# k-sheridan/ekf_vio

Measured on AMD Instinct MI355X. Metric: filter steps/sec (predict+update), higher is better.
Workload: dtype f32

## Files before the change

### ekf_vio_amd/capi.py

```python
import ctypes as C
import os

from . import _build

OK, EINVAL, ENUMERIC, ECAPACITY, EDEVICE, ESTATE, EABORTED = range(7)
_ERR = {EINVAL: "EKFVIO_EINVAL", ENUMERIC: "EKFVIO_ENUMERIC", ECAPACITY: "EKFVIO_ECAPACITY",
        EDEVICE: "EKFVIO_EDEVICE", ESTATE: "EKFVIO_ESTATE", EABORTED: "EKFVIO_EABORTED"}
PREDICT_STRUCTURED, PREDICT_DENSE = 0, 1


class Config(C.Structure):
    _fields_ = [("max_features", C.c_int32), ("default_point_depth", C.c_float),
                ("default_point_depth_variance", C.c_float), ("default_point_homogenous_variance", C.c_float),
                ("predict_mode", C.c_int32), ("klt_window_size", C.c_int32), ("klt_max_pyramid_level", C.c_int32),
                ("klt_max_iterations", C.c_int32), ("klt_epsilon", C.c_float), ("klt_min_eigen", C.c_float),
                ("kill_pad", C.c_int32), ("max_image_width", C.c_int32), ("max_image_height", C.c_int32),
                ("use_principal_point", C.c_int32), ("inverse_image_scale", C.c_int32), ("fast_threshold", C.c_int32),
                ("min_new_feature_dist", C.c_int32), ("fast_blur_sigma", C.c_float), ("replenish", C.c_int32),
                ("sample_based_uncertainty", C.c_int32), ("use_imu", C.c_int32), ("imu_gyro_variance", C.c_float),
                ("imu_accel_variance", C.c_float), ("gravity", C.c_float * 3),
                ("klt_fb_max_px", C.c_float), ("remove_lost", C.c_int32)]


class EkfvioError(RuntimeError):
    def __init__(self, code, msg=""):
        super().__init__("%s %s" % (_ERR.get(code, str(code)), msg))
        self.code = code


SYMBOLS = ["ekfvio_default_config", "ekfvio_create", "ekfvio_destroy", "ekfvio_reset", "ekfvio_last_error",
           "ekfvio_add_features", "ekfvio_process", "ekfvio_linearize", "ekfvio_update", "ekfvio_measurement_map",
           "ekfvio_num_features", "ekfvio_dim", "ekfvio_get_base_mu", "ekfvio_get_features", "ekfvio_get_sigma",
           "ekfvio_get_feature_cov", "ekfvio_get_depth_variance", "ekfvio_set_feature_cov", "ekfvio_metric2pixel_map",
           "ekfvio_pixel2metric_map", "ekfvio_get_odometry", "ekfvio_get_points", "ekfvio_check_sigma", "ekfvio_set_state",
           "ekfvio_remove_features", "ekfvio_klt_push_frame", "ekfvio_klt_track", "ekfvio_klt_track_points", "ekfvio_klt_get_level",
           "ekfvio_klt_uncertainty_points", "ekfvio_step_image", "ekfvio_replenish", "ekfvio_fast_detect", "ekfvio_imu", "ekfvio_imu_update",
           "ekfvio_upload_measurements", "ekfvio_run_uploaded", "ekfvio_synchronize", "ekfvio_profile_enable",
           "ekfvio_profile_reset", "ekfvio_profile_count", "ekfvio_profile_name", "ekfvio_profile_get",
           "ekfvio_profile_update_gemms", "ekfvio_get_counters", "ekfvio_set_gate", "ekfvio_get_gate",
           "ekfvio_set_klt_fb", "ekfvio_get_klt_fb", "ekfvio_klt_track_points_fb", "ekfvio_set_distortion", "ekfvio_rectify_map",
           "ekfvio_set_output_covariance", "ekfvio_get_odometry_covariance", "ekfvio_get_points_covariance", "ekfvio_rotation_error_jacobian",
           "ekfvio_set_mask", "ekfvio_get_mask", "ekfvio_get_mask_hits", "ekfvio_mask_blocked", "ekfvio_set_equalize", "ekfvio_equalize",
           "ekfvio_set_klt_photometric", "ekfvio_klt_project_gradients",
           "ekfvio_get_landmark_ids", "ekfvio_set_ended_export", "ekfvio_get_ended",
           "ekfvio_set_zupt", "ekfvio_zupt_update", "ekfvio_get_zupt", "ekfvio_zupt_decide"]
MASK_RECTIFY_BORDER = 1
HOOK_SYMBOLS = ["ekfvio_test_klt_padded_level", "ekfvio_test_blurred_level0", "ekfvio_test_gemm", "ekfvio_test_gemm_bench", "ekfvio_test_potrf_stamps",
                "ekfvio_test_sweep_stamps", "ekfvio_test_sweep_fault", "ekfvio_test_sweep_delay", "ekfvio_test_cholesky_solve", "ekfvio_test_plan", "ekfvio_test_persist_grid", "ekfvio_test_t2_pair",
                "ekfvio_test_gemm_plan", "ekfvio_test_predict_plan", "ekfvio_test_run_plan", "ekfvio_test_mem", "ekfvio_test_mem_fail",
                "ekfvio_test_fill_update_scratch", "ekfvio_test_zupt_decide"]

_libs = {}


def lib_path():
    return _build.LIB_PATH


def load(build_if_missing=True, hooks=False):
    if hooks in _libs:
        return _libs[hooks]
    path = _build.HOOKS_LIB_PATH if hooks else _build.LIB_PATH
    if build_if_missing:
        _build.build(hooks=hooks)
    elif not os.path.exists(path):
        raise FileNotFoundError(path + " not built; run python -m ekf_vio_amd._build")
    lib = C.CDLL(path)
    vp, i32, f32 = C.c_void_p, C.c_int32, C.c_float
    fp, u8p, ip = C.POINTER(C.c_float), C.POINTER(C.c_uint8), C.POINTER(C.c_int32)
    sig = {
        "ekfvio_default_config": [C.POINTER(Config)],
        "ekfvio_create": [C.POINTER(Config), C.c_int, vp, C.POINTER(vp)],
        "ekfvio_destroy": [vp], "ekfvio_reset": [vp],
        "ekfvio_add_features": [vp, fp, i32], "ekfvio_process": [vp, f32], "ekfvio_linearize": [vp, f32, fp],
        "ekfvio_update": [vp, fp, fp, u8p, i32], "ekfvio_measurement_map": [vp, u8p, i32, ip, ip],
        "ekfvio_num_features": [vp], "ekfvio_dim": [vp], "ekfvio_get_base_mu": [vp, fp],
        "ekfvio_get_features": [vp, fp, fp, u8p], "ekfvio_get_sigma": [vp, fp, i32],
        "ekfvio_get_feature_cov": [vp, i32, fp], "ekfvio_get_depth_variance": [vp, i32, fp],
        "ekfvio_set_feature_cov": [vp, i32, fp], "ekfvio_metric2pixel_map": [fp, fp], "ekfvio_pixel2metric_map": [fp, fp],
        "ekfvio_get_odometry": [vp, fp, fp, fp, fp], "ekfvio_get_points": [vp, fp, fp],
        "ekfvio_check_sigma": [vp, fp, fp], "ekfvio_set_state": [vp, i32, fp, fp, fp, u8p, fp, i32],
        "ekfvio_remove_features": [vp, u8p, i32, ip],
        "ekfvio_klt_push_frame": [vp, u8p, i32, i32, i32, fp], "ekfvio_klt_track": [vp, fp, fp, u8p],
        "ekfvio_klt_track_points": [vp, fp, fp, i32, fp, u8p],
        "ekfvio_klt_uncertainty_points": [vp, fp, fp, i32, fp],
        "ekfvio_klt_get_level": [vp, i32, ip, ip, u8p, C.POINTER(C.c_int16)],
        "ekfvio_step_image": [vp, C.c_double, u8p, i32, i32, i32, fp], "ekfvio_imu": [vp, C.c_double, fp, fp], "ekfvio_imu_update": [vp, fp, fp],
        "ekfvio_replenish": [vp, ip, ip], "ekfvio_fast_detect": [vp, i32, i32, i32, ip, ip, ip],
        "ekfvio_upload_measurements": [vp, i32, fp, fp, u8p], "ekfvio_run_uploaded": [vp, i32, i32, f32],
        "ekfvio_synchronize": [vp], "ekfvio_profile_enable": [vp, i32], "ekfvio_profile_reset": [vp],
        "ekfvio_profile_count": [], "ekfvio_profile_name": [i32],
        "ekfvio_profile_get": [vp, i32, C.POINTER(C.c_double), C.POINTER(C.c_int64), C.POINTER(C.c_double)],
        "ekfvio_profile_update_gemms": [vp, i32, C.POINTER(C.c_double), C.POINTER(C.c_double)],
        "ekfvio_get_counters": [vp, C.POINTER(C.c_int64)],
        "ekfvio_set_gate": [vp, f32], "ekfvio_get_gate": [vp, fp, u8p, ip, ip, C.POINTER(C.c_int64)],
        "ekfvio_set_klt_fb": [vp, f32], "ekfvio_get_klt_fb": [vp, fp, u8p, ip, ip, C.POINTER(C.c_int64)],
        "ekfvio_klt_track_points_fb": [vp, fp, fp, i32, fp, u8p, fp, fp, u8p],
        "ekfvio_set_distortion": [vp, C.POINTER(C.c_double), i32],
        "ekfvio_rectify_map": [fp, C.POINTER(C.c_double), i32, i32, i32, ip, ip],
        "ekfvio_set_output_covariance": [vp, i32], "ekfvio_get_odometry_covariance": [vp, fp, fp], "ekfvio_get_points_covariance": [vp, fp],
        "ekfvio_rotation_error_jacobian": [fp, fp],
        "ekfvio_set_mask": [vp, u8p, i32, i32, i32, i32], "ekfvio_get_mask": [vp, u8p, i32, ip, ip], "ekfvio_get_mask_hits": [vp, u8p, ip, ip],
        "ekfvio_mask_blocked": [fp, C.POINTER(C.c_double), i32, u8p, i32, i32, i32, i32, i32, i32, u8p],
        "ekfvio_set_equalize": [vp, f32, i32, i32],
        "ekfvio_equalize": [u8p, i32, i32, i32, f32, i32, i32, u8p],
        "ekfvio_set_klt_photometric": [vp, i32],
        "ekfvio_klt_project_gradients": [ip, ip, ip, i32, ip, ip],
        "ekfvio_get_landmark_ids": [vp, C.POINTER(C.c_int64), C.POINTER(C.c_double)],
        "ekfvio_set_ended_export": [vp, i32],
        "ekfvio_get_ended": [vp, C.POINTER(C.c_int64), C.POINTER(C.c_double), ip, fp, fp, i32, ip, C.POINTER(C.c_int64)],
        "ekfvio_set_zupt": [vp, f32, i32, f32, f32, f32], "ekfvio_zupt_update": [vp, f32, f32],
        "ekfvio_get_zupt": [vp, fp, ip, ip, ip, ip, C.POINTER(C.c_int64)],
        "ekfvio_zupt_decide": [fp, fp, u8p, i32, f32, i32, f32, fp, ip, ip, ip],
    }
    if hooks:
        sig.update({
            "ekfvio_test_klt_padded_level": [vp, i32, ip, u8p, C.POINTER(C.c_int16)],
            "ekfvio_test_blurred_level0": [vp, u8p],
            "ekfvio_test_gemm": [vp, i32, i32, i32, i32, f32, fp, i32, fp, i32, f32, fp, i32, i32],
            "ekfvio_test_cholesky_solve": [vp, i32, i32, fp, fp, fp, fp, ip],
            "ekfvio_test_potrf_stamps": [vp, C.POINTER(C.c_int64)],
            "ekfvio_test_sweep_stamps": [vp, C.c_int, C.POINTER(C.c_int64)],
            "ekfvio_test_sweep_fault": [vp, i32, i32],
            "ekfvio_test_sweep_delay": [vp, i32, i32, i32],
            "ekfvio_test_gemm_bench": [vp, i32, i32, i32, i32, i32, i32, i32, C.POINTER(C.c_double)],
            "ekfvio_test_plan": [i32] * 8 + [f32, ip],
            "ekfvio_test_persist_grid": [i32] * 8 + [f32, ip, i32, ip],
            "ekfvio_test_t2_pair": [i32, ip],
            "ekfvio_test_gemm_plan": [i32] * 11 + [ip],
            "ekfvio_test_predict_plan": [i32] * 5 + [ip],
            "ekfvio_test_run_plan": [i32] * 4 + [ip, i32, ip],
            "ekfvio_test_mem": [vp, C.POINTER(C.c_int64)],
            "ekfvio_test_mem_fail": [vp, i32],
            "ekfvio_test_fill_update_scratch": [vp, C.c_uint32],
            "ekfvio_test_zupt_decide": [vp, fp, fp, u8p, i32, f32, i32, f32, fp, ip, ip, ip],
        })
    for name, args in sig.items():
        fn = getattr(lib, name)
        fn.argtypes = args
        fn.restype = C.c_int
    lib.ekfvio_last_error.argtypes = [vp]
    lib.ekfvio_last_error.restype = C.c_char_p
    lib.ekfvio_profile_name.restype = C.c_char_p
    _libs[hooks] = lib
    return lib
```

### ekf_vio_amd/csrc/api.hip

```cpp
#include <math.h>
#include <stdio.h>
#include <string.h>

#include <algorithm>
#include <atomic>
#include <chrono>

#include <unistd.h>

#include "common.h"

static_assert((int)hipErrorOutOfMemory == MEM_ERR_OUT_OF_MEMORY && (int)hipSuccess == MEM_OK, "mem.h's codes are the runtime's");
namespace {
struct MemTotal {
    std::atomic<int64_t> live{0}, live_bytes{0}, acquired{0}, released{0};
} g_mem_total[MEM_KINDS];
int hip_mem_allocate(MemKind kind, size_t bytes, void** out) {
    static const unsigned host_flags[MEM_KINDS] = {0, hipHostMallocDefault, hipHostMallocMapped, hipHostMallocMapped | hipHostMallocCoherent};
    void* p = nullptr;
    const hipError_t e = kind == MEM_DEVICE ? hipMalloc(&p, bytes) : hipHostMalloc(&p, bytes, host_flags[kind]);
    if (e != hipSuccess) return (int)e;
    g_mem_total[kind].live++, g_mem_total[kind].live_bytes += (int64_t)bytes, g_mem_total[kind].acquired++;
    *out = p;
    return MEM_OK;
// ... 117 lines not shown
    return EKFVIO_OK;
}

extern "C" {

int ekfvio_default_config(ekfvio_config* c) {
    if (!c) return EKFVIO_EINVAL;
    c->max_features = 100;
    c->default_point_depth = 0.5f;
    c->default_point_depth_variance = 100.f;
    c->default_point_homogenous_variance = 1e-5f;
    c->predict_mode = EKFVIO_PREDICT_STRUCTURED;
    c->klt_window_size = 21;
    c->klt_max_pyramid_level = 3;
    c->klt_max_iterations = 30;
    c->klt_epsilon = 0.01f;
    c->klt_min_eigen = 1e-4f;
    c->kill_pad = 11;
    c->max_image_width = 640;
    c->max_image_height = 480;
    c->use_principal_point = 0;
    c->inverse_image_scale = 1;
    c->fast_threshold = 50;
    c->min_new_feature_dist = 30;
    c->fast_blur_sigma = 0.f;
    c->replenish = 0;
    c->sample_based_uncertainty = 0;
    c->use_imu = 0;
    c->imu_gyro_variance = 1e-4f;
    c->imu_accel_variance = 1e-2f;
    c->gravity[0] = 0.f;
    c->gravity[1] = 9.81f;
    c->gravity[2] = 0.f;
    c->klt_fb_max_px = 0.f;
    c->remove_lost = 0;
    return EKFVIO_OK;
}

static int create_body(ekfvio_filter* f, const ekfvio_config* cfg, int device, void* stream) {
    HIP_TRY(f, hipSetDevice(device));
    if (stream) {
        f->stream = (hipStream_t)stream;
    } else {
        HIP_TRY(f, hipStreamCreateWithFlags(&f->stream, hipStreamNonBlocking));
        f->own_stream = true;
    }
    const int maxf = cfg->max_features;
    const FilterDims dims = filter_dims(maxf);
    f->n_cap = dims.n_cap, f->ldp = dims.ldp, f->m_cap = dims.m_cap, f->ld_aug = dims.ld_aug, f->sweep_sync_words = dims.sweep_sync_words;
    f->tune = tuning_from_env();
    const size_t pp = (size_t)f->ldp * f->ldp, pm = (size_t)f->ldp * f->m_cap;
    HIP_TRY(f, dev_alloc(f, &f->mu, f->ldp));
    HIP_TRY(f, dev_alloc(f, &f->mu_next, f->ldp));
    HIP_TRY(f, dev_alloc(f, &f->last_klt, 2 * (size_t)maxf));
    HIP_TRY(f, dev_alloc(f, &f->del_flag, (size_t)maxf));
    HIP_TRY(f, dev_alloc(f, &f->lm_id, (size_t)maxf));
    HIP_TRY(f, dev_alloc(f, &f->lm_born, (size_t)maxf));
    HIP_TRY(f, dev_alloc(f, &f->P, pp));
    HIP_TRY(f, dev_alloc(f, &f->P2, pp));
    HIP_TRY(f, dev_alloc(f, &f->FA, EKF_BASE * EKF_BASE));
    HIP_TRY(f, dev_alloc(f, &f->FB, 27 * (size_t)maxf));
    HIP_TRY(f, dev_alloc(f, &f->FD, 9 * (size_t)maxf));
    HIP_TRY(f, dev_alloc(f, &f->Fdense, pp));
    HIP_TRY(f, dev_alloc(f, &f->idx, (size_t)f->m_cap));
    HIP_TRY(f, dev_alloc(f, &f->inv_idx, (size_t)f->ldp));
    HIP_TRY(f, dev_alloc(f, &f->zmeas, 2 * (size_t)maxf));
    HIP_TRY(f, dev_alloc(f, &f->Rmeas, 4 * (size_t)maxf));
    HIP_TRY(f, dev_alloc(f, &f->pass, (size_t)maxf));
    HIP_TRY(f, dev_alloc(f, &f->yres, (size_t)f->m_cap));
    HIP_TRY(f, dev_alloc(f, &f->Rm, 2 * (size_t)f->m_cap));
    HIP_TRY(f, dev_alloc(f, &f->Saug, (size_t)f->ld_aug * f->m_cap));
    HIP_TRY(f, dev_alloc(f, &f->Laug, (size_t)f->ld_aug * f->m_cap));
    HIP_TRY(f, dev_alloc(f, &f->Linv, 64 * (size_t)f->m_cap));
    HIP_TRY(f, dev_alloc(f, &f->Lsign, (size_t)(f->m_cap / 64 > 256 ? f->m_cap / 64 : 256)));
    HIP_TRY(f, dev_alloc(f, &f->sweep_sync, f->sweep_sync_words));
    {
        hipDeviceProp_t prop;
        HIP_TRY(f, hipGetDeviceProperties(&prop, device));
        f->num_cus = prop.multiProcessorCount;
    }
    HIP_TRY(f, dev_alloc(f, &f->Km, pm));
    HIP_TRY(f, dev_alloc(f, &f->Wt, pm));
    HIP_TRY(f, dev_alloc(f, &f->Gm, pm));
    HIP_TRY(f, dev_alloc(f, &f->info, 4));
    HIP_TRY(f, dev_alloc(f, &f->remove_words, 4));
    HIP_TRY(f, host_alloc(f, &f->h_info, 16 * sizeof(int), MEM_PINNED_COHERENT));
    memset(f->h_info, 0, 16 * sizeof(int));
    HIP_TRY(f, hipHostGetDevicePointer((void**)&f->d_hinfo, f->h_info, 0));
    {
        const size_t words = out_words(f);
        HIP_TRY(f, host_alloc(f, &f->h_out, words * sizeof(float), MEM_PINNED_COHERENT));
        HIP_TRY(f, hipHostGetDevicePointer((void**)&f->d_out, f->h_out, 0));
    }
    {
        const size_t cap = (size_t)(f->cfg.max_features > 0 ? f->cfg.max_features : 1);
        HIP_TRY(f, host_alloc(f, &f->h_meas, 25 * cap, MEM_PINNED));
        HIP_TRY(f, dev_alloc_bare(f, &f->d_meas, 25 * cap));
    }
    HIP_TRY(f, hipEventCreate(&f->ev0));
    HIP_TRY(f, hipEventCreate(&f->ev1));
    int rc = klt_alloc(f);
    if (rc != EKFVIO_OK) return rc;
    rc = fast_alloc(f);
    if (rc != EKFVIO_OK) return rc;
    return ekfvio_reset(f);
}

}

static std::atomic<int>* live_registry() {
    static std::atomic<int>* reg = [] {
        char name[64], val[32];
        snprintf(name, sizeof(name), "EKFVIO_LIVE_HANDLES_%ld", (long)getpid());
        if (const char* e = getenv(name)) {
            void* p = nullptr;
            if (sscanf(e, "%p", &p) == 1 && p) return static_cast<std::atomic<int>*>(p);
        }
        auto* a = new std::atomic<int>[64];
        for (int i = 0; i < 64; i++) a[i].store(0, std::memory_order_relaxed);
        snprintf(val, sizeof(val), "%p", static_cast<void*>(a));
        setenv(name, val, 1);
        return a;
    }();
    return reg;
}
int live_handles_on(int device) { return (device >= 0 && device < 64) ? live_registry()[device].load(std::memory_order_relaxed) : 2; }

void drop_graph(ekfvio_filter* f) {
    for (GraphCache::Entry& e : f->graphs.g) {
        if (e.exec) (void)hipGraphExecDestroy(e.exec);
        e = GraphCache::Entry();
    }
}
template <class Body>
static int capture_graph(ekfvio_filter* f, hipGraphExec_t* out, Body body) {
    hipGraph_t g = nullptr;
    HIP_TRY(f, hipStreamSynchronize(f->stream));
    HIP_TRY(f, hipStreamBeginCapture(f->stream, hipStreamCaptureModeThreadLocal));
    body();
    const hipError_t ce = hipStreamEndCapture(f->stream, &g);
    if (ce != hipSuccess || !g) {
        f->last_error = std::string("graph capture: ") + hipGetErrorString(ce);
        return EKFVIO_EDEVICE;
    }
    HIP_TRY(f, hipGraphInstantiate(out, g, nullptr, nullptr, 0));
    (void)hipGraphDestroy(g);
    return EKFVIO_OK;
}

extern "C" {

int ekfvio_create(const ekfvio_config* cfg, int device, void* stream, ekfvio_filter** out) {
    if (!out) return EKFVIO_EINVAL;
    *out = nullptr;
    if (!cfg || cfg->max_features < 0) return EKFVIO_EINVAL;
    if (cfg->remove_lost != 0 && cfg->remove_lost != 1) return EKFVIO_EINVAL;
    if (cfg->remove_lost && (size_t)cfg->max_features * 17 > 64 * 1024) return EKFVIO_ECAPACITY;
    if (!(cfg->klt_fb_max_px >= 0.f)) return EKFVIO_EINVAL;
    int ndev = 0;
    if (hipGetDeviceCount(&ndev) != hipSuccess || device < 0 || device >= ndev) return EKFVIO_EDEVICE;
    ekfvio_filter* f = new ekfvio_filter();
#ifdef EKFVIO_TEST_HOOKS
    f->mem.fail_nth(g_next_create_fail.exchange(0));
#endif
    f->cfg = *cfg;
    f->device = device;
// ... 817 lines not shown
    return EKFVIO_OK;
}

int ekfvio_test_plan(int32_t num_cus, int32_t max_features, int32_t N, int32_t m, int32_t m_on_device, int32_t sole_handle,
                     int32_t latched_off, int32_t dense_predict, float next_dt, int32_t plan[12]) {
    if (!plan || max_features < 0 || N < 0 || N > max_features) return EKFVIO_EINVAL;
    const FilterDims d = filter_dims(max_features);
    PlanShape s;
    s.num_cus = num_cus, s.ldp = d.ldp, s.sweep_sync_words = d.sweep_sync_words, s.N = N, s.n = EKF_BASE + 3 * N;
    s.dense_predict = dense_predict != 0, s.sole_handle = sole_handle != 0, s.latched_off = latched_off != 0;
    const UpdatePlan p = plan_update(tuning_from_env(), s, m, m_on_device != 0, next_dt);
    const int32_t out[12] = {p.m, p.m_pad, p.n_pad, p.sweep, p.fused_gather, p.with_wt, p.gain, p.tail, p.t2_skip, p.t2_by_sweep, p.compact, p.lin_blocks};
    std::copy(out, out + 12, plan);
    return EKFVIO_OK;
}

int ekfvio_test_gemm_plan(int32_t num_cus, int32_t M, int32_t N, int32_t K, int32_t transB, int32_t lowerB, int32_t epi, int32_t mean,
                          int32_t lin_blocks, int32_t sym, int32_t variant, int32_t plan[18]) {
    if (!plan || M <= 0 || N <= 0 || K <= 0 || epi < EPI_NONE || epi > EPI_MEAN_PARTIAL) return EKFVIO_EINVAL;
    GemmShape s;
    s.M = M, s.N = N, s.K = K, s.transB = transB != 0, s.lowerB = lowerB != 0, s.epi = epi, s.mean = mean != 0;
    s.lin_blocks = lin_blocks, s.sym = sym != 0, s.variant = variant;
    const GemmPlan p = plan_gemm(tuning_from_env(), num_cus, s);
    const int32_t out[18] = {p.k16, p.bm, p.wps, p.groups, p.threads(), p.tiles_x, p.tiles_y, p.tiles, p.grid_x, p.grid_y, p.mean_wg, p.lin_blocks,
                             p.mean_keep, p.sym, p.sym_w, p.order2d, gemm_throughput_regime(num_cus, M, N, K), gemm_tile_height(num_cus, M, N, K, s.transB)};
    std::copy(out, out + 18, plan);
    return EKFVIO_OK;
}
int ekfvio_test_predict_plan(int32_t num_cus, int32_t N, int32_t dense_predict, int32_t prelinearized, int32_t bookkeeping, int32_t plan[8]) {
    if (!plan || N < 0) return EKFVIO_EINVAL;
    PlanShape s;
    s.num_cus = num_cus, s.N = N, s.n = EKF_BASE + 3 * N, s.dense_predict = dense_predict != 0;
    const PredictPlan p = plan_predict(tuning_from_env(), s, prelinearized != 0);
    const int32_t out[8] = {p.dense, p.pre, p.lin_inside, p.lin_in_front, p.ts, p.chunks, p.book_rides(), p.grid(bookkeeping != 0)};
    std::copy(out, out + 8, plan);
    return EKFVIO_OK;
}
int ekfvio_test_run_plan(int32_t N, int32_t gated, int32_t profiling, int32_t frames, const int32_t* rows, int32_t count, int32_t out[6]) {
    if (!out || !rows || N < 0 || frames <= 0 || count < 0) return EKFVIO_EINVAL;
    const RunPlan p = plan_run(rows, frames, N, gated != 0, profiling != 0, count);
    const int32_t res[6] = {p.graphs, p.m, p.replays[0], p.replays[1], p.replays[2], p.eager};
    std::copy(res, res + 6, out);
    return EKFVIO_OK;
}

int ekfvio_test_persist_grid(int32_t num_cus, int32_t max_features, int32_t N, int32_t m, int32_t m_on_device, int32_t sole_handle,
                             int32_t latched_off, int32_t dense_predict, float next_dt, int32_t* roles, int32_t max_blocks, int32_t out[10]) {
    if (!out || max_features < 0 || N < 0 || N > max_features) return EKFVIO_EINVAL;
    const FilterDims d = filter_dims(max_features);
    PlanShape s;
    s.num_cus = num_cus, s.ldp = d.ldp, s.sweep_sync_words = d.sweep_sync_words, s.N = N, s.n = EKF_BASE + 3 * N;
    s.dense_predict = dense_predict != 0, s.sole_handle = sole_handle != 0, s.latched_off = latched_off != 0;
    const UpdatePlan p = plan_update(tuning_from_env(), s, m, m_on_device != 0, next_dt);
    std::fill(out, out + 10, 0);
    if (!p.persistent()) return EKFVIO_OK;
    const PersistGrid g = persist_grid(p, d.ldp);
    const PersistFlags fl(p.m_pad, p.n_pad);
    const int32_t res[10] = {g.total(), g.kind, g.owners(), fl.ready(), fl.fin(), fl.pan(), fl.abort_word(), (int32_t)fl.words(), fl.zero_words(),
                             (int32_t)d.sweep_sync_words};
    std::copy(res, res + 10, out);
    if (!roles) return EKFVIO_OK;
    if (max_blocks < g.total()) return EKFVIO_ECAPACITY;
    for (int b = 0; b < g.total(); b++) {
        const PersistRole r = g.role(b);
        roles[4 * b] = r.kind, roles[4 * b + 1] = r.a, roles[4 * b + 2] = r.b;
        roles[4 * b + 3] = r.kind == ROLE_OWNER ? g.owner_block(r.n) : -1;
    }
    return EKFVIO_OK;
}
int ekfvio_test_t2_pair(int32_t p, int32_t pair[2]) {
    if (p < 0 || !pair) return EKFVIO_EINVAL;
    int ta, tb;
    t2_pair(p, ta, tb);
    pair[0] = ta, pair[1] = tb;
    return EKFVIO_OK;
}

int ekfvio_test_fill_update_scratch(ekfvio_filter* f, uint32_t word) {
    if (!f) return EKFVIO_EINVAL;
    HIP_TRY(f, hipSetDevice(f->device));
    const size_t maxf = (size_t)(f->cfg.max_features > 0 ? f->cfg.max_features : 0);
    const size_t aug = (size_t)f->ld_aug * f->m_cap, pm = (size_t)f->ldp * f->m_cap;
    const struct { float* p; size_t count; } regions[] = {
        {f->Saug, aug}, {f->Laug, aug}, {f->Linv, 64 * (size_t)f->m_cap}, {f->Km, pm}, {f->Wt, pm}, {f->Gm, pm},
        {f->yres, (size_t)f->m_cap}, {f->Rm, 2 * (size_t)f->m_cap}, {f->Fdense, (size_t)f->ldp * f->ldp},
        {f->FA, (size_t)EKF_BASE * EKF_BASE}, {f->FB, 27 * maxf}, {f->FD, 9 * maxf}, {f->mu_next, (size_t)f->ldp},
    };
    for (const auto& r : regions)
        if (r.p && r.count) HIP_TRY(f, hipMemsetD32Async((hipDeviceptr_t)r.p, (int)word, r.count, f->stream));
    return EKFVIO_OK;
}
#endif

}
```

### ekf_vio_amd/csrc/chol_persist.inc

```

#ifndef PERSIST_POLL_SLEEP_LAZY
#define PERSIST_POLL_SLEEP_LAZY 12
#endif
#ifndef PERSIST_POLL_SLEEP
#define PERSIST_POLL_SLEEP 2
#endif

struct PollBound {
    int spin_limit, wait_ticks;
};
struct PersistArgs {
    float* S;
    int lds;
    float* L;
    int ldl;
    float* Linv;
    int mb, idb0;
    int* info;
    unsigned long long* Lsign;
    int* ready;
    int* fin;
    int* abort_flag;
    long long* dbg;
    PersistGrid grid;
// ... 144 lines not shown
}
__device__ __forceinline__ void persist_publish(int* flag, int tid) {
    wait_vm0();
    __syncthreads();
    if (tid == 0) __hip_atomic_store(flag, 1, __ATOMIC_RELAXED, __HIP_MEMORY_SCOPE_AGENT);
}
__device__ __forceinline__ void persist_publish_wave(int* flag, int lane) {
    wait_vm0();
    if (lane == 0) __hip_atomic_fetch_add(flag, 1, __ATOMIC_RELAXED, __HIP_MEMORY_SCOPE_AGENT);
}
#ifdef EKFVIO_TEST_HOOKS
#define PERSIST_TEST_DELAY(a, point)                                                                                        \
    do {                                                                                                                    \
        if ((int)blockIdx.x == (a).delay_wg && (a).delay_point == (point)) {                                                \
            const unsigned long long t0_ = __builtin_amdgcn_s_memrealtime();                                                \
            while (__builtin_amdgcn_s_memrealtime() - t0_ < (unsigned long long)(unsigned)(a).delay_ticks) __builtin_amdgcn_s_sleep(8); \
        }                                                                                                                   \
    } while (0)
#else
#define PERSIST_TEST_DELAY(a, point) do { } while (0)
#endif
__device__ __forceinline__ unsigned long long ld_sign_sc1(const unsigned long long* p) {
    return __hip_atomic_load(p, __ATOMIC_RELAXED, __HIP_MEMORY_SCOPE_AGENT);
}

__device__ __forceinline__ void gain_tile(const PersistArgs& a, float* Ti, float* Tj, float* Tl, float* Tinv, int ib, int cb, int tid) {
    const int lane = tid & 63, wave = tid >> 6, wr = wave & 1, wc = wave >> 1;
    const int r = wr * 32 + (lane & 31);
    const int mb = a.mb, ldl = a.ldl;
    const __amdgpu_buffer_rsrc_t bL = persist_rsrc(a.L, (unsigned)ldl * (unsigned)(mb * PB));
    float kv[16];
#pragma unroll
    for (int q = 0; q < 16; q++) kv[q] = 0.f;
    const int iy = mb + ib, iz = a.idb0 + cb;
    for (int kb = cb; kb < mb; kb++) {
        bool signed_last = false;
        unsigned long long negl = 0ull;
        if (kb == mb - 1) {
            const __amdgpu_buffer_rsrc_t bS = persist_rsrc(a.S, (unsigned)a.lds * (unsigned)(mb * PB));
            const __amdgpu_buffer_rsrc_t bI = persist_rsrc(a.Linv, (unsigned)(mb * PB * PB));
            const bool zi = a.grid.compact() && cb == kb;
            persist_wait(a, nullptr, a.fin + iy * mb + kb, zi ? nullptr : a.fin + iz * mb + kb, tid, 1, true);
            load_tile_sc1(Ti, bS, (unsigned)(kb * PB) * (unsigned)a.lds + (unsigned)(iy * PB), a.lds, tid);
            if (zi) identity_tile(Tj, tid);
            else load_tile_sc1(Tj, bS, (unsigned)(kb * PB) * (unsigned)a.lds + (unsigned)(iz * PB), a.lds, tid);
            persist_wait(a, a.ready + kb, nullptr, nullptr, tid, 4, false);
            load_tile_sc1(Tl, bL, (unsigned)(kb * PB) * (unsigned)ldl + (unsigned)(kb * PB), ldl, tid);
            load_inv_sc1(Tinv, bI, (unsigned)(kb * PB * PB), tid);
            negl = ld_sign_sc1(a.Lsign + kb);
            __syncthreads();
            tri_solve_fwd2(Ti, Tj, Tl, Tinv, wave, lane);
            if (a.dbg && tid == 0 && ib * mb + cb < 104) a.dbg[400 + ib * mb + cb] = (long long)__builtin_amdgcn_s_memrealtime();
            signed_last = negl != 0ull;
        } else {
            persist_wait(a, nullptr, a.pan + iy * mb + kb, a.pan + iz * mb + kb, tid, 1, true);
            load_tile_sc1(Ti, bL, (unsigned)(kb * PB) * (unsigned)ldl + (unsigned)(iy * PB), ldl, tid);
            load_tile_sc1(Tj, bL, (unsigned)(kb * PB) * (unsigned)ldl + (unsigned)(iz * PB), ldl, tid);
        }
        __syncthreads();
        const f32x16 up = signed_last ? mma64_signed(Ti, 1, PLD, Tj, 1, PLD, wr, wc, lane, negl) : mma64(Ti, 1, PLD, Tj, 1, PLD, wr, wc, lane);
#pragma unroll
        for (int q = 0; q < 16; q++) kv[q] = kv[q] + up[q];
    }
    float* Kt = a.K + (size_t)(cb * PB) * a.ldk + (size_t)ib * PB;
#pragma unroll
    for (int q = 0; q < 16; q++) {
        const int c = mma64_col(wc, lane, q);
        Kt[(size_t)c * a.ldk + r] = (fabsf(kv[q]) > EKF_FLUSH_THRESH) ? kv[q] : 0.f;
    }
}

__device__ __forceinline__ void sign_cols(float* dst, const float* src, unsigned long long neg, int tid) {
#pragma unroll
    for (int it = 0; it < 4; it++) {
        const int e = tid + it * 256;
        const int c = e >> 4, r4 = (e & 15) * 4;
        const float sg = ((neg >> c) & 1ull) ? -1.f : 1.f;
        const float4 v = *reinterpret_cast<const float4*>(src + c * PLD + r4);
        *reinterpret_cast<float4*>(dst + c * PLD + r4) = make_float4(sg * v.x, sg * v.y, sg * v.z, sg * v.w);
    }
}

template <bool WAIT>
__device__ __forceinline__ void gain_tile2(const PersistArgs& a, const GatherArgs& ga, float* Ti, float* Tj, float* Tl, float* Tinv, float* Th, float* tab,
                                           int ib, int cb, int tid) {
    const int lane = tid & 63, wave = tid >> 6, wr = wave & 1, wc = wave >> 1;
    const int r = wr * 32 + (lane & 31);
    const int mb = a.mb, ldl = a.ldl;
    const int m = ga.m_dev ? *ga.m_dev : ga.m;
    const __amdgpu_buffer_rsrc_t bL = persist_rsrc(a.L, (unsigned)ldl * (unsigned)(mb * PB));
    const __amdgpu_buffer_rsrc_t bS = persist_rsrc(a.S, (unsigned)a.lds * (unsigned)(mb * PB));
    const int iy = mb + ib, iz = a.idb0 + cb;
    const int cq = cb * PB + lane;
    const int sq = (cq < m) ? ga.idx[cq] : -1;
    const unsigned sqc = (unsigned)max(sq, 0);
    int alo = 0, ahi = -1;
    if (cb * PB < m) {
        alo = ga.idx[cb * PB] / PB;
        ahi = ga.idx[min(cb * PB + PB - 1, m - 1)] / PB;
    }
    if (tid < 64) {
        float yq = 0.f, rd = 0.f, ro = 0.f;
        if (sq >= 0) {
            yq = ga.zrow[cq] - ga.mu[sq];
            rd = ga.Rm[2 * cq];
            ro = ga.Rm[2 * (cq ^ 1) + 1];
        }
        tab[tid] = yq, tab[64 + tid] = rd, tab[128 + tid] = ro;
    }
    auto column_flags = [&](int kb, const int* zflag) -> PollLane {
        const int ax = alo + tid - 2;
        return {tid == 0 ? a.pan + iy * mb + kb : tid == 1 ? zflag : (tid >= 2 && ax <= ahi) ? a.pan + (mb + ax) * mb + kb : nullptr, 1};
    };
    float kv[16], w2[16];
    {
        float wv[16];
        const int scl = max(sq, 0);
#pragma unroll
        for (int ps = 0; ps < 16; ps++) wv[ps] = ga.P[(size_t)min(ib * PB + wave + 4 * ps, ga.n - 1) * ga.ld + scl];
#pragma unroll
        for (int ps = 0; ps < 16; ps++) asm volatile("" : "+v"(wv[ps]));
#pragma unroll
        for (int ps = 0; ps < 16; ps++) Th[(wave + 4 * ps) * 65 + lane] = (sq >= 0 && ib * PB + wave + 4 * ps < ga.n) ? wv[ps] : 0.f;
        __syncthreads();
#pragma unroll
        for (int q = 0; q < 16; q++) {
            kv[q] = 0.f;
            w2[q] = Th[r * 65 + mma64_col(wc, lane, q)];
        }
    }
    auto fetch = [&](int kb) -> unsigned long long {
        const bool gk = kb >= cb;
        float hv[16];
        unsigned long long neg;
        if constexpr (WAIT) {
            persist_wait(a, column_flags(kb, gk ? a.pan + iz * mb + kb : nullptr), tid, kb < mb - 2);
            load_tile_sc1(Ti, bL, (unsigned)(kb * PB) * (unsigned)ldl + (unsigned)(iy * PB), ldl, tid);
            if (gk) load_tile_sc1(Tj, bL, (unsigned)(kb * PB) * (unsigned)ldl + (unsigned)(iz * PB), ldl, tid);
#pragma unroll
            for (int ps = 0; ps < 16; ps++)
                hv[ps] = __builtin_bit_cast(float, __builtin_amdgcn_raw_buffer_load_b32(bL, ((unsigned)(kb * PB + wave + 4 * ps) * (unsigned)ldl + (unsigned)(mb * PB) + sqc) * 4u, 0, 16));
#pragma unroll
            for (int ps = 0; ps < 16; ps++) hv[ps] = (sq >= 0) ? hv[ps] : 0.f;
#pragma unroll
            for (int ps = 0; ps < 16; ps++) Th[(wave + 4 * ps) * PLD + lane] = hv[ps];
            neg = ld_sign_sc1(a.Lsign + kb);
        } else {
            load_tile(Ti, a.L + (size_t)kb * PB * ldl + (size_t)iy * PB, ldl, tid);
            if (gk) load_tile(Tj, a.L + (size_t)kb * PB * ldl + (size_t)iz * PB, ldl, tid);
#pragma unroll
            for (int ps = 0; ps < 16; ps++) hv[ps] = a.L[(size_t)(kb * PB + wave + 4 * ps) * ldl + (size_t)(mb * PB) + sqc];
#pragma unroll
            for (int ps = 0; ps < 16; ps++) hv[ps] = (sq >= 0) ? hv[ps] : 0.f;
#pragma unroll
            for (int ps = 0; ps < 16; ps++) Th[(wave + 4 * ps) * PLD + lane] = hv[ps];
            neg = a.Lsign[kb];
        }
        return neg;
    };
    auto products = [&](int kb, unsigned long long neg, bool z_unsigned) {
        if (kb >= cb) {
            const f32x16 up = (z_unsigned && neg != 0ull) ? mma64_signed(Ti, 1, PLD, Tj, 1, PLD, wr, wc, lane, neg) : mma64(Ti, 1, PLD, Tj, 1, PLD, wr, wc, lane);
#pragma unroll
            for (int q = 0; q < 16; q++) kv[q] = kv[q] + up[q];
        }
        if (alo <= ahi) {
            f32x16 up;
            if constexpr (WAIT) {
                up = (neg == 0ull) ? mma64(Ti, 1, PLD, Th, 1, PLD, wr, wc, lane) : mma64_signed(Ti, 1, PLD, Th, 1, PLD, wr, wc, lane, neg);
            } else {
                if (__builtin_amdgcn_readfirstlane((int)(neg != 0ull))) {
                    __syncthreads();
                    sign_cols(Ti, Ti, neg, tid);
                    __syncthreads();
                }
                up = mma64(Ti, 1, PLD, Th, 1, PLD, wr, wc, lane);
            }
#pragma unroll
            for (int q = 0; q < 16; q++) w2[q] = w2[q] - up[q];
        }
        if (WAIT && a.dbg && tid == 0 && mb <= 8 && (ib == 0 || ib == 6) && (cb == 0 || cb == 3 || cb == 7))
            a.dbg[100 + 8 * ((ib ? 3 : 0) + (cb == 0 ? 0 : cb == 3 ? 1 : 2)) + kb] = (long long)__builtin_amdgcn_s_memrealtime();
    };
    if constexpr (WAIT) {
        for (int kb = 0; kb < mb - 2; kb++) {
            __syncthreads();
            const unsigned long long neg = fetch(kb);
            __syncthreads();
            products(kb, neg, false);
        }
    } else {
        for (int kb = 0; kb < mb; kb++) {
            __syncthreads();
            const unsigned long long neg = fetch(kb);
            __syncthreads();
            products(kb, neg, false);
        }
    }
    if constexpr (WAIT) {
        const int kl = mb - 1, k6 = mb - 2;
        const bool gk6 = k6 >= cb;
        const __amdgpu_buffer_rsrc_t bI = persist_rsrc(a.Linv, (unsigned)(mb * PB * PB));
        const bool zi = a.grid.compact() && cb == kl;
        __syncthreads();
        persist_wait(a, column_flags(k6, gk6 ? a.pan + iz * mb + k6 : (zi ? nullptr : a.fin + iz * mb + kl)), tid, false);
        RegTile ql, qi, qj;
        float hq[16];
        unsigned long long neg6;
        {
            RegTile pi6, pj6;
            float h6[16];
            pi6.request(bL, (unsigned)(k6 * PB) * (unsigned)ldl + (unsigned)(iy * PB), ldl, tid);
            if (gk6) pj6.request(bL, (unsigned)(k6 * PB) * (unsigned)ldl + (unsigned)(iz * PB), ldl, tid);
#pragma unroll
            for (int ps = 0; ps < 16; ps++)
                h6[ps] = __builtin_bit_cast(float, __builtin_amdgcn_raw_buffer_load_b32(bL, ((unsigned)(k6 * PB + wave + 4 * ps) * (unsigned)ldl + (unsigned)(mb * PB) + sqc) * 4u, 0, 16));
            neg6 = ld_sign_sc1(a.Lsign + k6);
            pi6.put(Ti, tid);
            if (gk6) pj6.put(Tj, tid);
#pragma unroll
            for (int ps = 0; ps < 16; ps++) Th[(wave + 4 * ps) * PLD + lane] = (sq >= 0) ? h6[ps] : 0.f;
        }
        persist_wait(a, a.ready + kl, nullptr, nullptr, tid, 4, false);
        ql.request(bL, (unsigned)(kl * PB) * (unsigned)ldl + (unsigned)(kl * PB), ldl, tid);
        qi.request(bS, (unsigned)(kl * PB) * (unsigned)a.lds + (unsigned)(iy * PB), a.lds, tid);
        if (!zi) qj.request(bS, (unsigned)(kl * PB) * (unsigned)a.lds + (unsigned)(iz * PB), a.lds, tid);
        const float4 qv = ld_sc1(bI, (unsigned)(kl * PB * PB) + tid * 4);
        const unsigned long long neg7 = ld_sign_sc1(a.Lsign + kl);
#pragma unroll
        for (int ps = 0; ps < 16; ps++)
            hq[ps] = __builtin_bit_cast(float, __builtin_amdgcn_raw_buffer_load_b32(bS, ((unsigned)(kl * PB + wave + 4 * ps) * (unsigned)a.lds + (unsigned)(mb * PB) + sqc) * 4u, 0, 16));
        products(mb - 2, neg6, false);
        __syncthreads();
        ql.put(Tl, tid);
        qi.put(Ti, tid);
        if (zi) identity_tile(Tj, tid);
        else qj.put(Tj, tid);
        inv_put(qv, Tinv, tid);
#pragma unroll
        for (int ps = 0; ps < 16; ps++) Th[(wave + 4 * ps) * PLD + lane] = (sq >= 0) ? hq[ps] : 0.f;
        __syncthreads();
        float* const t3[3] = {Ti, Tj, Th};
        tri_solve_fwd_n<3>(t3, Tl, Tinv, wave, lane);
        __syncthreads();
        products(kl, neg7, true);
    }
#pragma unroll
    for (int q = 0; q < 16; q++) kv[q] = (fabsf(kv[q]) > EKF_FLUSH_THRESH) ? kv[q] : 0.f;
    float* Kt = a.K + (size_t)(cb * PB) * a.ldk + (size_t)ib * PB;
    float* Gt = ga.G + (size_t)(cb * PB) * ga.ld + (size_t)ib * PB;
    float acc = 0.f;
#pragma unroll
    for (int q = 0; q < 16; q++) {
        const int c = mma64_col(wc, lane, q), cg = cb * PB + c;
        Kt[(size_t)c * a.ldk + r] = kv[q];
        float g = 0.f;
        if (cg < m) {
            const float x = kv[q] * tab[64 + c], y = kv[q ^ 1] * tab[128 + c];
            const float kr = ((cg ^ 1) < cg) ? (y + x) : (x + y);
            g = kr - w2[q];
            acc = acc + kv[q] * tab[c];
        }
        Gt[(size_t)c * ga.ld + r] = g;
    }
    __syncthreads();
    float* part = Th;
    part[(wc * 2 + (lane >> 5)) * 64 + r] = acc;
    __syncthreads();
    if (tid < 64) ga.Wt[(size_t)cb * ga.ld + (size_t)ib * PB + tid] = ((part[tid] + part[64 + tid]) + part[128 + tid]) + part[192 + tid];
}

template <bool WAIT>
__device__ __forceinline__ void t2_tile(const PersistArgs& a, float* Ti, float* Tj, float* Tl, float* Tinv, int ta, int tb, int tid, long long* dbg = nullptr) {
    const int lane = tid & 63, wave = tid >> 6, wr = wave & 1, wc = wave >> 1;
    const int r = wr * 32 + (lane & 31);
    const int mb = a.mb, ldl = a.ldl;
    const bool diag = ta == tb;
    const __amdgpu_buffer_rsrc_t bL = persist_rsrc(a.L, (unsigned)ldl * (unsigned)(mb * PB));
    float tab[16], tba[16];
    {
        const float* sab = a.Sg + (size_t)tb * PB * a.ldsg + (size_t)ta * PB;
        const float* sba = a.Sg + (size_t)ta * PB * a.ldsg + (size_t)tb * PB;
#pragma unroll
        for (int q = 0; q < 16; q++) {
            const int c = mma64_col(wc, lane, q);
            tab[q] = sab[(size_t)c * a.ldsg + r];
            tba[q] = diag ? 0.f : sba[(size_t)c * a.ldsg + r];
        }
    }
    const int ia = mb + ta, ib = mb + tb;
    auto apply = [&](int kb, unsigned long long neg) {
        const float* Bj = diag ? Ti : Tj;
        f32x16 up;
        if constexpr (WAIT) {
            up = (neg == 0ull) ? mma64(Ti, 1, PLD, Bj, 1, PLD, wr, wc, lane) : mma64_signed(Ti, 1, PLD, Bj, 1, PLD, wr, wc, lane, neg);
        } else if (__builtin_amdgcn_readfirstlane((int)(neg != 0ull))) {
            sign_cols(Tl, Ti, neg, tid);
            __syncthreads();
            up = mma64(Tl, 1, PLD, Bj, 1, PLD, wr, wc, lane);
            __syncthreads();
        } else {
            up = mma64(Ti, 1, PLD, Bj, 1, PLD, wr, wc, lane);
        }
#pragma unroll
        for (int q = 0; q < 16; q++) tab[q] = tab[q] - up[q];
        if (!diag) {
#pragma unroll
            for (int q = 0; q < 16; q++) Tl[r * PLD + mma64_col(wc, lane, q)] = up[q];
            __syncthreads();
#pragma unroll
            for (int q = 0; q < 16; q++) tba[q] = tba[q] - Tl[mma64_col(wc, lane, q) * PLD + r];
        }
        if (dbg && tid == 0) dbg[kb] = (long long)__builtin_amdgcn_s_memrealtime();
    };
    if constexpr (WAIT) {
        for (int kb = 0; kb < mb - 2; kb++) {
            __syncthreads();
            persist_wait(a, nullptr, a.pan + ia * mb + kb, diag ? nullptr : a.pan + ib * mb + kb, tid, 1, true);
            load_tile_sc1(Ti, bL, (unsigned)(kb * PB) * (unsigned)ldl + (unsigned)(ia * PB), ldl, tid);
            if (!diag) load_tile_sc1(Tj, bL, (unsigned)(kb * PB) * (unsigned)ldl + (unsigned)(ib * PB), ldl, tid);
            const unsigned long long neg = ld_sign_sc1(a.Lsign + kb);
            __syncthreads();
            apply(kb, neg);
        }
    } else {
        for (int kb = 0; kb < mb; kb++) {
            __syncthreads();
            load_tile(Ti, a.L + (size_t)kb * PB * ldl + (size_t)ia * PB, ldl, tid);
            if (!diag) load_tile(Tj, a.L + (size_t)kb * PB * ldl + (size_t)ib * PB, ldl, tid);
            const unsigned long long neg = a.Lsign[kb];
            __syncthreads();
            apply(kb, neg);
        }
    }
    if constexpr (WAIT) {
        const int kl = mb - 1, k6 = mb - 2;
        const __amdgpu_buffer_rsrc_t bS = persist_rsrc(a.S, (unsigned)a.lds * (unsigned)(mb * PB));
        const __amdgpu_buffer_rsrc_t bI = persist_rsrc(a.Linv, (unsigned)(mb * PB * PB));
        __syncthreads();
        persist_wait(a, a.ready + kl, a.pan + ia * mb + k6, diag ? nullptr : a.pan + ib * mb + k6, tid, 4, false);
        RegTile pi6, pj6, ql, qi, qj;
        pi6.request(bL, (unsigned)(k6 * PB) * (unsigned)ldl + (unsigned)(ia * PB), ldl, tid);
        if (!diag) pj6.request(bL, (unsigned)(k6 * PB) * (unsigned)ldl + (unsigned)(ib * PB), ldl, tid);
        const unsigned long long neg6 = ld_sign_sc1(a.Lsign + k6);
        ql.request(bL, (unsigned)(kl * PB) * (unsigned)ldl + (unsigned)(kl * PB), ldl, tid);
        qi.request(bS, (unsigned)(kl * PB) * (unsigned)a.lds + (unsigned)(ia * PB), a.lds, tid);
        if (!diag) qj.request(bS, (unsigned)(kl * PB) * (unsigned)a.lds + (unsigned)(ib * PB), a.lds, tid);
        const float4 qv = ld_sc1(bI, (unsigned)(kl * PB * PB) + tid * 4);
        const unsigned long long neg7 = ld_sign_sc1(a.Lsign + kl);
        pi6.put(Ti, tid);
        if (!diag) pj6.put(Tj, tid);
        __syncthreads();
        apply(k6, neg6);
        __syncthreads();
        ql.put(Tl, tid);
        qi.put(Ti, tid);
        if (!diag) qj.put(Tj, tid);
        inv_put(qv, Tinv, tid);
        __syncthreads();
        if (diag) tri_solve_fwd(Ti, Tl, Tinv, wave, lane);
        else tri_solve_fwd2(Ti, Tj, Tl, Tinv, wave, lane);
        __syncthreads();
        apply(kl, neg7);
    }
    __syncthreads();
#pragma unroll
    for (int q = 0; q < 16; q++) {
        const int c = mma64_col(wc, lane, q);
        Ti[c * PLD + r] = (ta * PB + r < a.nstate && tb * PB + c < a.nstate) ? tab[q] : 0.f;
        if (!diag) Tj[c * PLD + r] = (tb * PB + r < a.nstate && ta * PB + c < a.nstate) ? tba[q] : 0.f;
    }
    __syncthreads();
    store_tile(Ti, a.T2 + (size_t)tb * PB * a.ldt + (size_t)ta * PB, a.ldt, tid);
    if (!diag) store_tile(Tj, a.T2 + (size_t)ta * PB * a.ldt + (size_t)tb * PB, a.ldt, tid);
    if (dbg && tid == 0) dbg[15] = (long long)__builtin_amdgcn_s_memrealtime();
}

template <bool SC1>
__device__ __forceinline__ float persist_ldf(const float* p) {
    if constexpr (SC1) return __hip_atomic_load(p, __ATOMIC_RELAXED, __HIP_MEMORY_SCOPE_AGENT);
    else return *p;
}
template <bool SC1>
__device__ __forceinline__ void persist_tile_x(f32x4 (&x)[4], const float* G, int ld, int wave, int lane) {
    const int li = lane & 15, g = lane >> 4;
#pragma unroll
    for (int b = 0; b < 4; b++)
#pragma unroll
        for (int v = 0; v < 4; v++) x[b][v] = persist_ldf<SC1>(G + (size_t)(16 * b + 4 * g + v) * ld + 16 * wave + li);
}
__device__ __forceinline__ void persist_diag_block(float* D, const float* P, int tr, int tc, int lane, unsigned long long neg) {
    const int li = lane & 15, lk = lane >> 4;
    const int rb = 16 * tr, cb = 16 * tc;
    const float* ap = P + rb + li + lk * PLD;
    const float* bp = P + cb + li + lk * PLD;
    f32x4 u = {0.f, 0.f, 0.f, 0.f};
    if (neg == 0ull) {
#pragma unroll
        for (int q = 0; q < PB; q += 4) u = __builtin_amdgcn_mfma_f32_16x16x4f32(bp[q * PLD], ap[q * PLD], u, 0, 0, 0);
    } else {
#pragma unroll 4
        for (int q = 0; q < PB; q += 4) {
            float av = ap[q * PLD];
            if ((neg >> (q + lk)) & 1ull) av = -av;
            u = __builtin_amdgcn_mfma_f32_16x16x4f32(bp[q * PLD], av, u, 0, 0, 0);
        }
    }
    float t[4];
#pragma unroll
    for (int gq = 0; gq < 4; gq++) t[gq] = D[(cb + 4 * lk + gq) * PLD + rb + li];
#pragma unroll
    for (int gq = 0; gq < 4; gq++) D[(cb + 4 * lk + gq) * PLD + rb + li] = t[gq] - u[gq];
}


struct GTile {
    int ia[16];
    int ib;
    float v[16], rd[16], ro[16];
};
__device__ __forceinline__ void gtile_idx(GTile& t, const GatherArgs& ga, int m, int rb, int cb, int mb, int idb0, int tid) {
    if (rb < mb) {
        const int c = cb * PB + (tid & 63);
        t.ib = (c < m) ? ga.idx[c] : 0;
#pragma unroll
        for (int ps = 0; ps < 16; ps++) {
            const int rc = max(min(rb * PB + (tid >> 6) + 4 * ps, m - 1), 0);
            t.ia[ps] = max(ga.idx[rc], 0);
            t.rd[ps] = ga.Rm[2 * rc];
            t.ro[ps] = ga.Rm[2 * rc + 1];
        }
    } else if (rb < idb0) {
#pragma unroll
        for (int ps = 0; ps < 16; ps++) {
            const int c = cb * PB + (tid >> 6) + 4 * ps;
            t.ia[ps] = (c < m) ? ga.idx[c] : 0;
        }
    }
}
__device__ __forceinline__ void gtile_val(GTile& t, const GatherArgs& ga, int m, int rb, int cb, int mb, int idb0, int tid) {
    if (rb < mb) {
#pragma unroll
        for (int ps = 0; ps < 16; ps++) t.v[ps] = ga.P[(size_t)t.ia[ps] * ga.ld + t.ib];
    } else if (rb < idb0) {
        const int x = min((rb - mb) * PB + (tid & 63), ga.ld - 1);
#pragma unroll
        for (int ps = 0; ps < 16; ps++) t.v[ps] = ga.P[(size_t)t.ia[ps] * ga.ld + x];
    }
}
__device__ __forceinline__ void gtile_put(const GTile& t, float* T, const GatherArgs& ga, int m, int rb, int cb, int mb, int idb0, int tid) {
    if (rb < mb) {
        const int cl = tid & 63, c = cb * PB + cl;
#pragma unroll
        for (int ps = 0; ps < 16; ps++) {
            const int rl = (tid >> 6) + 4 * ps;
            T[cl * PLD + rl] = gather_a_elem(t.v[ps], rb * PB + rl, c, m, t.rd[ps], t.ro[ps]);
        }
// ... 193 lines not shown
#pragma unroll
                    for (int v = 0; v < 4; v++) Pdst[(size_t)(16 * bq + 4 * g + v) * ldl] = x[0][bq][v];
            }
            __syncthreads();
            PSTAMP(32 + 8 * k + 3);
            persist_diag_block(Dn, Ti, wave, 0, lane, neg);
            __syncthreads();
            PSTAMP(32 + 8 * k + 4);
            float* Dn_c = Dn;
            const float* Ti_c = Ti;
            const unsigned long long neg_c = neg;
            auto idle = [&](auto pc, int wv) {
                constexpr int p = decltype(pc)::value;
                if constexpr (p == 0) {
                    if (wv == 1) {
                        persist_diag_block(Dn_c, Ti_c, 1, 1, lane, neg_c);
                        persist_diag_block(Dn_c, Ti_c, 2, 1, lane, neg_c);
                    } else if (wv == 2) {
                        persist_diag_block(Dn_c, Ti_c, 3, 1, lane, neg_c);
                        persist_diag_block(Dn_c, Ti_c, 2, 2, lane, neg_c);
                    } else {
                        persist_diag_block(Dn_c, Ti_c, 3, 2, lane, neg_c);
                        persist_diag_block(Dn_c, Ti_c, 3, 3, lane, neg_c);
                    }
                }
            };
            const bool bad = potrf64_lds<EKF_POTRF_FV>(Dn, Tinv, tid, nullptr, idle);
            unsigned long long neg1 = 0ull;
            PSTAMP(32 + 8 * k + 5);
            if (a.dbg && tid == 0) a.dbg[700 + k] = (long long)__builtin_amdgcn_s_memrealtime();
            seen = 1;
            if (k + 2 < mb && lane < 2)
                seen = __hip_atomic_load(lane == 0 ? a.fin + (i + 1) * mb + i : a.fin + (i + 1) * mb + (i + 1), __ATOMIC_RELAXED, __HIP_MEMORY_SCOPE_AGENT);
            if (bad) {
                __syncthreads();
                if (k >= kf) load_tile_sc1(Dn, bS, oii, lds, tid);
                else load_tile(Dn, S + oii, lds, tid);
                __syncthreads();
                const f32x16 up = (neg == 0ull) ? mma64(Ti, 1, PLD, Ti, 1, PLD, wr, wc, lane) : mma64_signed(Ti, 1, PLD, Ti, 1, PLD, wr, wc, lane, neg);
#pragma unroll
                for (int q = 0; q < 16; q++) {
                    const int c = mma64_col(wc, lane, q);
                    Dn[c * PLD + r] = Dn[c * PLD + r] - up[q];
                }
                neg1 = potrf64_signed(Dn, Tinv, tid);
            }
            store_tile_sc1<true>(Dn, bL, (unsigned)(i * PB) * (unsigned)ldl + (unsigned)(i * PB), ldl, tid);
            store_inv_sc1(Tinv, bI, (unsigned)(i * PB * PB), tid);
            if (tid == 0) {
                __hip_atomic_store(a.Lsign + i, neg1, __ATOMIC_RELAXED, __HIP_MEMORY_SCOPE_AGENT);
                if (bad) atomicOr(a.info, 1);
            }
            asm volatile("" ::: "memory");
            neg = neg1;
            float* t = Lk;
            Lk = Dn;
            Dn = t;
        }
        persist_publish_wave(a.ready + (mb - 1), lane);
        PSTAMP(32 + 8 * (mb - 1));
        if (a.dbg && tid == 0) a.dbg[897] = (long long)__builtin_amdgcn_s_memrealtime();
        PEXIT();
    }

    if (role.kind == ROLE_LEAD || role.kind == ROLE_LEAD_GATHER0) {
        if (!compact) gather_body<false>(ga, ga.nb1 + role.n, persist_dyn_lds);
        else if (role.kind == ROLE_LEAD_GATHER0) {
            const int cb = role.a;
            const int m = ga.m_dev ? *ga.m_dev : ga.m;
            GTile t;
            gtile_idx(t, ga, m, 1, cb, mb, a.idb0, tid);
            gtile_pin(t);
            gtile_val(t, ga, m, 1, cb, mb, a.idb0, tid);
            gtile_pinv(t);
            gtile_put(t, Tl, ga, m, 1, cb, mb, a.idb0, tid);
            __syncthreads();
            store_tile_sc1<false>(Tl, bS, (unsigned)(cb * PB) * (unsigned)lds + (unsigned)PB, lds, tid);
            persist_publish(a.fin + 1 * mb + cb, tid);
        }
        if (a.gain) {
            const int tb = role.n;
            __syncthreads();
            if (role.a < a.idb0 - mb) {
                if (a.t2) gain_tile2<true>(a, ga, Ti, Tj, Tl, Tinv, persist_dyn_lds, persist_dyn_lds + PB * PLD, role.a, role.b, tid);
                else gain_tile(a, Ti, Tj, Tl, Tinv, role.a, role.b, tid);
                if (a.dbg && tid == 0 && tb < 104) a.dbg[200 + tb] = (long long)__builtin_amdgcn_s_memrealtime();
            }
        }
        PEXIT();
    }
    const int idb0 = a.idb0;
    if (role.kind == ROLE_GATHER0) {
        const int cb = role.a;
        const int m = ga.m_dev ? *ga.m_dev : ga.m;
        GTile t;
        gtile_idx(t, ga, m, 1, cb, mb, idb0, tid);
        gtile_pin(t);
        gtile_val(t, ga, m, 1, cb, mb, idb0, tid);
        gtile_pinv(t);
        gtile_put(t, Tl, ga, m, 1, cb, mb, idb0, tid);
        __syncthreads();
        store_tile_sc1<false>(Tl, bS, (unsigned)(cb * PB) * (unsigned)lds + (unsigned)PB, lds, tid);
        persist_publish(a.fin + 1 * mb + cb, tid);
        PEXIT();
    }
    const int i = role.a, j = role.b, hidx = role.n;
    const int k0 = (i >= idb0) ? (i - idb0) : 0;
    const int klast = (i == j) ? j - 2 : j - 1;
    const unsigned oij = (unsigned)(j * PB) * (unsigned)lds + (unsigned)(i * PB);
    float tv[16];
    if (fused) {
        const int m = ga.m_dev ? *ga.m_dev : ga.m;
        const bool step0 = k0 == 0 && klast >= 0;
        GTile tn, ti_, tj_;
        gtile_idx(tn, ga, m, i, j, mb, idb0, tid);
        if (step0) {
            gtile_idx(ti_, ga, m, i, 0, mb, idb0, tid);
            if (i != j) gtile_idx(tj_, ga, m, j, 0, mb, idb0, tid);
        }
        gtile_pin(tn);
        if (step0) gtile_pin(ti_);
        gtile_val(tn, ga, m, i, j, mb, idb0, tid);
        if (step0) {
            gtile_val(ti_, ga, m, i, 0, mb, idb0, tid);
            if (i != j) gtile_val(tj_, ga, m, j, 0, mb, idb0, tid);
        }
        gtile_pinv(tn);
        gtile_put(tn, Tl, ga, m, i, j, mb, idb0, tid);
        if (step0) {
            gtile_put(ti_, Ti, ga, m, i, 0, mb, idb0, tid);
            if (i != j) gtile_put(tj_, Tj, ga, m, j, 0, mb, idb0, tid);
        }
        __syncthreads();
#pragma unroll
        for (int q = 0; q < 16; q++) tv[q] = Tl[mma64_col(wc, lane, q) * PLD + r];
        __syncthreads();
    } else {
#pragma unroll
        for (int q = 0; q < 16; q++) tv[q] = S[oij + (size_t)mma64_col(wc, lane, q) * lds + r];
    }
#define HSTAMP(n)                                                                                                       \
    do {                                                                                                                \
        if (a.dbg && i == j + 1 && i < mb && k == klast && tid == 0) a.dbg[600 + 8 * j + (n)] = (long long)__builtin_amdgcn_s_memtime(); \
    } while (0)
    unsigned long long neg = 0ull;
    int k = k0;
    for (; k <= klast; k++) {
        HSTAMP(0);
        const bool lazy = !(k == klast && i <= j + 1);
        const bool early = a.early_sources && k >= 1;
        const bool src_ident = compact && k >= 1 && i >= idb0 && i - idb0 == k;
        const int* fin_ik = src_ident ? nullptr : a.fin + i * mb + k;
        if (early) {
            persist_wait(a, nullptr, fin_ik, (i != j) ? a.fin + j * mb + k : nullptr, tid, 1, lazy);
            if (src_ident) identity_tile(Ti, tid);
            else load_tile_sc1(Ti, bS, (unsigned)(k * PB) * (unsigned)lds + (unsigned)(i * PB), lds, tid);
            if (i != j) load_tile_sc1(Tj, bS, (unsigned)(k * PB) * (unsigned)lds + (unsigned)(j * PB), lds, tid);
            persist_wait(a, a.ready + k, nullptr, nullptr, tid, 4, lazy);
        } else if (k >= 1) persist_wait(a, a.ready + k, fin_ik, (i != j) ? a.fin + j * mb + k : nullptr, tid, 4, lazy);
        else if (fused) persist_wait(a, a.ready, nullptr, nullptr, tid, 4, lazy);
        else __syncthreads();
        HSTAMP(1);
        if (k >= 1 || fused) {
            load_tile_sc1(Tl, bL, (unsigned)(k * PB) * (unsigned)ldl + (unsigned)(k * PB), ldl, tid);
            load_inv_sc1(Tinv, bI, (unsigned)(k * PB * PB), tid);
            if (k >= 1 && !early) {
                if (src_ident) identity_tile(Ti, tid);
                else load_tile_sc1(Ti, bS, (unsigned)(k * PB) * (unsigned)lds + (unsigned)(i * PB), lds, tid);
                if (i != j) load_tile_sc1(Tj, bS, (unsigned)(k * PB) * (unsigned)lds + (unsigned)(j * PB), lds, tid);
            }
            neg = ld_sign_sc1(a.Lsign + k);
        } else {
            load_tile(Tl, L, ldl, tid);
            load_inv(Tinv, a.Linv, tid);
            load_tile(Ti, S + (size_t)i * PB, lds, tid);
            if (i != j) load_tile(Tj, S + (size_t)j * PB, lds, tid);
            neg = a.Lsign[0];
        }
        __syncthreads();
        HSTAMP(2);
        if (i != j)
            tri_solve_fwd2(Ti, Tj, Tl, Tinv, wave, lane);
        else
            tri_solve_fwd(Ti, Tl, Tinv, wave, lane);
        __syncthreads();
        HSTAMP(3);
        const float* Bj = (i != j) ? Tj : Ti;
        const f32x16 up = (neg == 0ull) ? mma64(Ti, 1, PLD, Bj, 1, PLD, wr, wc, lane) : mma64_signed(Ti, 1, PLD, Bj, 1, PLD, wr, wc, lane, neg);
#pragma unroll
        for (int q = 0; q < 16; q++) tv[q] = tv[q] - up[q];
        HSTAMP(4);
    }
    k = klast;
    if (klast >= k0 || fused) {
        if (klast < k0) __syncthreads();
#pragma unroll
        for (int q = 0; q < 16; q++) Tl[mma64_col(wc, lane, q) * PLD + r] = tv[q];
        __syncthreads();
        PERSIST_TEST_DELAY(a, 0);
        store_tile_sc1<false>(Tl, bS, oij, lds, tid);
    }
    if ((int)blockIdx.x != a.stall_wg) persist_publish(a.fin + i * mb + j, tid);
    else __syncthreads();
    HSTAMP(5);
    if (a.dbg && tid == 0 && i < mb && (i == j + 1 || i == j)) a.dbg[(i == j ? 740 : 720) + j] = (long long)__builtin_amdgcn_s_memrealtime();
    if (klast >= k0 && i != j) {
        if (a.gain && i >= mb) {
            const unsigned od = (unsigned)(klast * PB) * (unsigned)ldl + (unsigned)(i * PB);
            PERSIST_TEST_DELAY(a, 1);
            if (neg != 0ull && i >= idb0) store_tile_signed_sc1(Ti, bL, od, ldl, tid, neg);
            else store_tile_sc1<false>(Ti, bL, od, ldl, tid);
            persist_publish(a.pan + i * mb + klast, tid);
        } else {
            float* dst = L + (size_t)klast * PB * ldl + (size_t)i * PB;
            if (neg != 0ull && i >= idb0) store_tile_signed(Ti, dst, ldl, tid, neg);
            else store_tile(Ti, dst, ldl, tid);
        }
    }
    if (a.t2) {
        const int p = a.grid.t2_pair_of(hidx);
        if (a.dbg && tid == 0 && hidx < 8) {
            a.dbg[192 + hidx] = (long long)__builtin_amdgcn_s_memrealtime();
        }
        if (p >= 0) {
            int ta, tb;
            t2_pair(p, ta, tb);
            long long* td = nullptr;
            const int np_ = t2_pairs(a.grid.nX);
            if (a.dbg && (p == 0 || p == np_ / 2 || p == np_ - 1)) {
                td = a.dbg + 840 + 16 * (p == 0 ? 0 : p == np_ - 1 ? 2 : 1);
                if (tid == 0) td[14] = (long long)__builtin_amdgcn_s_memrealtime();
            }
            t2_tile<true>(a, Ti, Tj, Tl, Tinv, ta, tb, tid, td);
            if (a.dbg && tid == 0 && p < 91) a.dbg[304 + p] = (long long)__builtin_amdgcn_s_memrealtime();
        }
        PEXIT();
    }
    if (j == mb - 1 && i >= mb) {
        if (i >= idb0 && i - idb0 > j) PEXIT();
        if (a.gain) PEXIT();
        persist_wait(a, a.ready + j, nullptr, nullptr, tid, 4, false);
        load_tile_sc1(Tj, bL, (unsigned)(j * PB) * (unsigned)ldl + (unsigned)(j * PB), ldl, tid);
        load_inv_sc1(Tinv, bI, (unsigned)(j * PB * PB), tid);
        const unsigned long long negl = ld_sign_sc1(a.Lsign + j);
        if (klast < k0) {
#pragma unroll
            for (int q = 0; q < 16; q++) Tl[mma64_col(wc, lane, q) * PLD + r] = tv[q];
        }
        __syncthreads();
        tri_solve_fwd(Tl, Tj, Tinv, wave, lane);
        __syncthreads();
        if (a.gain) {
            const unsigned od = (unsigned)(j * PB) * (unsigned)ldl + (unsigned)(i * PB);
            if (negl != 0ull && i >= idb0) store_tile_signed_sc1(Tl, bL, od, ldl, tid, negl);
            else store_tile_sc1<false>(Tl, bL, od, ldl, tid);
            persist_publish(a.pan + i * mb + j, tid);
        } else {
            float* dst = L + (size_t)j * PB * ldl + (size_t)i * PB;
            if (negl != 0ull && i >= idb0) store_tile_signed(Tl, dst, ldl, tid, negl);
            else store_tile(Tl, dst, ldl, tid);
        }
    }
    PEXIT();
#undef PEXIT
#undef HSTAMP
#undef PSTAMP
}

__global__ __launch_bounds__(256) void gain_tiles_kernel(PersistArgs a) {
    __shared__ __attribute__((aligned(16))) float Ti[PB * PLD];
    __shared__ __attribute__((aligned(16))) float Tj[PB * PLD];
    const int tid = threadIdx.x, lane = tid & 63, wave = tid >> 6, wr = wave & 1, wc = wave >> 1;
    const int r = wr * 32 + (lane & 31);
    const int mb = a.mb, ldl = a.ldl;
    const int ib = (int)blockIdx.x / mb, cb = (int)blockIdx.x % mb;
    const int iy = mb + ib, iz = a.idb0 + cb;
    float kv[16];
#pragma unroll
    for (int q = 0; q < 16; q++) kv[q] = 0.f;
#define GT_DECL(S) float4 ya##S##0, ya##S##1, ya##S##2, ya##S##3, za##S##0, za##S##1, za##S##2, za##S##3;
#define GT_REQ1(S, IT, KB)                                                                                                                    \
    ya##S##IT = *reinterpret_cast<const float4*>(a.L + (size_t)(KB) * PB * ldl + (size_t)iy * PB + (size_t)((tid + IT * 256) >> 4) * ldl + ((tid + IT * 256) & 15) * 4); \
    za##S##IT = *reinterpret_cast<const float4*>(a.L + (size_t)(KB) * PB * ldl + (size_t)iz * PB + (size_t)((tid + IT * 256) >> 4) * ldl + ((tid + IT * 256) & 15) * 4);
#define GT_REQ(S, KB) GT_REQ1(S, 0, KB) GT_REQ1(S, 1, KB) GT_REQ1(S, 2, KB) GT_REQ1(S, 3, KB)
#define GT_PUT1(S, IT)                                                                                        \
    *reinterpret_cast<float4*>(Ti + ((tid + IT * 256) >> 4) * PLD + ((tid + IT * 256) & 15) * 4) = ya##S##IT; \
    *reinterpret_cast<float4*>(Tj + ((tid + IT * 256) >> 4) * PLD + ((tid + IT * 256) & 15) * 4) = za##S##IT;
#define GT_STEP(S, KB)                                                      \
    do {                                                                    \
        __syncthreads();                                                    \
        GT_PUT1(S, 0) GT_PUT1(S, 1) GT_PUT1(S, 2) GT_PUT1(S, 3)             \
        __syncthreads();                                                    \
        if ((KB) + 2 < mb) { GT_REQ(S, (KB) + 2) }                          \
        const f32x16 up = mma64(Ti, 1, PLD, Tj, 1, PLD, wr, wc, lane);      \
        _Pragma("unroll") for (int q = 0; q < 16; q++) kv[q] = kv[q] + up[q]; \
    } while (0)
    GT_DECL(0)
    GT_DECL(1)
    GT_REQ(0, cb)
    if (cb + 1 < mb) { GT_REQ(1, cb + 1) }
    else { ya10 = ya11 = ya12 = ya13 = za10 = za11 = za12 = za13 = make_float4(0.f, 0.f, 0.f, 0.f); }
    for (int kb = cb; kb < mb; kb += 2) {
        GT_STEP(0, kb);
        if (kb + 1 < mb) GT_STEP(1, kb + 1);
    }
#undef GT_DECL
#undef GT_REQ1
#undef GT_REQ
#undef GT_PUT1
#undef GT_STEP
    float* Kt = a.K + (size_t)(cb * PB) * a.ldk + (size_t)ib * PB;
#pragma unroll
    for (int q = 0; q < 16; q++) {
        const int c = mma64_col(wc, lane, q);
        Kt[(size_t)c * a.ldk + r] = (fabsf(kv[q]) > EKF_FLUSH_THRESH) ? kv[q] : 0.f;
    }
}

__global__ __launch_bounds__(256) void gain2_t2_tiles_kernel(PersistArgs a, GatherArgs ga, int gain_wgs) {
    extern __shared__ float g2_dyn_lds[];
    __shared__ __attribute__((aligned(16))) float Ti[PB * PLD];
    __shared__ __attribute__((aligned(16))) float Tj[PB * PLD];
    __shared__ __attribute__((aligned(16))) float Th[PB * PLD];
    __shared__ float tab[192];
    if ((int)blockIdx.x < gain_wgs) {
        gain_tile2<false>(a, ga, Ti, Tj, nullptr, nullptr, Th, tab, (int)blockIdx.x / a.mb, (int)blockIdx.x % a.mb, threadIdx.x);
    } else {
        int ta, tb;
        t2_pair((int)blockIdx.x - gain_wgs, ta, tb);
        t2_tile<false>(a, Ti, Tj, Th, nullptr, ta, tb, threadIdx.x);
    }
}
```

### ekf_vio_amd/csrc/common.h

```cpp
#pragma once
#include <hip/hip_runtime.h>
#include <stdint.h>

#include <chrono>
#include <string>
#include <vector>

#include "../../include/ekfvio.h"
#include "mem.h"
#include "plan.h"
#ifdef EKFVIO_TEST_HOOKS
#include "../../include/ekfvio_test_hooks.h"
#endif

#ifndef EKF_POTRF_FV
#define EKF_POTRF_FV 12
#endif
#define EKF_FLUSH_THRESH (1e-8f * 1e-5f)

#define HIP_TRY(f, expr)                                                           \
    do {                                                                           \
        hipError_t e__ = (expr);                                                   \
        if (e__ != hipSuccess) {                                                   \
            (f)->last_error = std::string(#expr) + ": " + hipGetErrorString(e__);  \
// ... 67 lines not shown
    }
};
struct GraphCache {
    struct Entry {
        hipGraphExec_t exec = nullptr;
        int steps = 0;
        int pre = 0;
    };
    GraphKey key;
    Entry g[RUN_GRAPHS];
    bool leaves_flags_clean = false;
};

const MemBackend& hip_mem_backend();

struct ekfvio_filter {
    ekfvio_config cfg;
    int device = 0;
    hipStream_t stream = nullptr;
    bool own_stream = false;
    std::string last_error;
    MemLedger mem{hip_mem_backend()};

    int N = 0;
    int n = EKF_BASE;
    int n_cap = 0, ldp = 0, m_cap = 0;
    Tuning tune;

    float* mu = nullptr;
    float* mu_next = nullptr;
    float* last_klt = nullptr;
    uint8_t* del_flag = nullptr;
    int64_t* lm_id = nullptr;
    double* lm_born = nullptr;
    int64_t next_id = 0;
    float* P = nullptr;
    float* P2 = nullptr;
    float* FA = nullptr;
    float* FB = nullptr;
    float* FD = nullptr;
    float* Fdense = nullptr;
    int* idx = nullptr;
    int* inv_idx = nullptr;
    float* zmeas = nullptr;
    float* Rmeas = nullptr;
    uint8_t* pass = nullptr;
    float* yres = nullptr;
    float* Rm = nullptr;
    float* Saug = nullptr;
    float* Laug = nullptr;
    int ld_aug = 0;
    float* Linv = nullptr;
    unsigned long long* Lsign = nullptr;
    int* sweep_sync = nullptr;
    size_t sweep_sync_words = 0;
    bool sweep_latched_off = false;
    long long persistent_sweeps = 0;
    long long schur_sweeps = 0;
    long long sweep_recoveries = 0;
    long long early_output_frames = 0;
    int sweep_spin_limit = 0;
    int sweep_stall_wg = -1;
#ifdef EKFVIO_TEST_HOOKS
    int sweep_delay_wg = -1, sweep_delay_point = 0, sweep_delay_ticks = 0;
#endif
    bool sweep_retry_armed = false;
    double sweep_retry_pause_s = 0.0;
    int sweep_probation = 0;
    std::chrono::steady_clock::time_point sweep_retry_at;
    bool sweep_flags_clean = false;
    bool persist_attr_set = false;
    bool gain2_attr_set = false;
    bool gather_attr_set = false;
    long long t2_updates = 0;
    long long graph_steps = 0;
    long long prelinearized_steps = 0;
    int num_cus = 0;
    int last_m = 0;
    long long* sweep_dbg = nullptr;
    long long* gemm_stamps = nullptr;
    float* Km = nullptr;
    float* Wt = nullptr;
    float* Gm = nullptr;
    int* info = nullptr;
    float gate_chi2 = 0.f;
    float* gate_d2 = nullptr;
    uint8_t* gate_flag = nullptr;
    uint8_t* gate_pass = nullptr;
    int* gate_words = nullptr;
    int* fb_words = nullptr;
    float* fb_err2 = nullptr;
    uint8_t* fb_flag = nullptr;
    float* fb_pt_err2 = nullptr;
    float* fb_pt_back = nullptr;
    uint8_t* fb_pt_flag = nullptr;
    bool ended_on = false;
    unsigned char* h_ended = nullptr;
    int64_t* ended_id = nullptr;
    double* ended_born = nullptr;
    float* ended_xyz = nullptr;
    float* ended_cov = nullptr;
    int* ended_index = nullptr;
    int ended_count = 0;
    int64_t ended_total = 0;
    float zupt_max_flow_px = 0.f;
    int zupt_min_tracks = 0;
    float zupt_min_ratio = 0.f, zupt_vel_var = 0.f, zupt_omega_var = 0.f;
    int* zupt_words = nullptr;
    int* h_zupt = nullptr;
    int* d_hzupt = nullptr;
    int zupt_n = 0, zupt_pass = 0, zupt_still = 0, zupt_applied_last = 0;
    int64_t zupt_applied_total = 0;
    int* remove_words = nullptr;
    int* h_info = nullptr;
    int* d_hinfo = nullptr;
    int status_seq = 0;
    float* h_out = nullptr;
    float* d_out = nullptr;
    bool out_fresh = false;
    bool output_cov = false;
    bool out_cov_fresh = false;
    unsigned char* h_meas = nullptr;
    unsigned char* d_meas = nullptr;
    float* seq_z = nullptr;
    float* seq_R = nullptr;
    uint8_t* seq_pass = nullptr;
    int seq_frames = 0;
    int seq_N = 0;
    std::vector<int> seq_m;
    std::vector<std::vector<uint8_t>> seq_pass_host;

    KltFrame frames[2];
    int cur = 0;
    int klt_border = 0;
    float* klt_prev_px = nullptr;
    float* klt_next_px = nullptr;
    uint8_t* klt_status = nullptr;
    float* klt_cov_px = nullptr;
    bool klt_photo = false;
    uint8_t* staging = nullptr;
    uint8_t* h_image = nullptr;
    size_t src_cap = 0;
    double dist[5] = {0, 0, 0, 0, 0};
    bool rect_on = false;
    int* rect_sx = nullptr;
    int* rect_sy = nullptr;
    uint8_t* rect_img = nullptr;
    size_t rect_cap = 0;
    RectifyKey rect_key;
    bool rect_key_valid = false;
    bool mask_on = false;
    int mask_flags = 0;
    uint8_t* mask_user = nullptr;
    int mask_uw = 0, mask_uh = 0;
    unsigned mask_user_gen = 0;
    unsigned* mask_nodata = nullptr;
    unsigned* mask_blocked = nullptr;
    size_t mask_cap_words = 0;
    MaskKey mask_key;
    bool mask_key_valid = false;
    int mask_bw = 0, mask_bh = 0;
    uint8_t* mask_hit = nullptr;
    int mask_hits_n = 0;
    bool eq_on = false;
    float eq_clip = 0.f;
    int eq_tx = 0, eq_ty = 0;
    uint8_t* eq_lut = nullptr;
    size_t eq_lut_cap = 0;
    uint8_t* blurred = nullptr;
    unsigned* fast_row_kp = nullptr;
    int* fast_kp_xy = nullptr;
    short* fast_kp_score = nullptr;
    int fast_kp_cap = 0;
    uint8_t* occ_mask = nullptr;
    int* fast_row_cnt = nullptr;
    int* new_xy = nullptr;
    int* fast_counts = nullptr;
    int fast_cap_w = 0, fast_cap_h = 0;
    double t_stamp = 0;
    bool have_stamp = false;

    GraphCache graphs;

    bool prof_on = false;
    float prof_overhead_ms = 0.f;
    ProfSlot prof[PC_COUNT];
    hipEvent_t ev0 = nullptr, ev1 = nullptr;
};

inline hipError_t mem_error(int rc) { return rc == MEM_ERR_FOREIGN ? hipErrorInvalidDevicePointer : (hipError_t)rc; }
template <class T>
hipError_t dev_alloc(MemLedger& mem, hipStream_t s, T** p, size_t count) {
    const size_t bytes = sizeof(T) * (count ? count : 1);
    hipError_t e = mem_error(mem.acquire(p, bytes, MEM_DEVICE));
    if (e == hipSuccess) e = hipMemsetAsync(*p, 0, bytes, s);
    return e;
}
template <class T>
hipError_t dev_alloc(ekfvio_filter* f, T** p, size_t count) { return dev_alloc(f->mem, f->stream, p, count); }
template <class T>
hipError_t dev_alloc_bare(ekfvio_filter* f, T** p, size_t bytes) { return mem_error(f->mem.acquire(p, bytes, MEM_DEVICE)); }
template <class T>
hipError_t host_alloc(ekfvio_filter* f, T** p, size_t bytes, MemKind kind) { return mem_error(f->mem.acquire(p, bytes, kind)); }

struct GemmEpi {
    int mode = 0;
    const int* inv_idx = nullptr;
    const float* Rm = nullptr;
    float* G = nullptr;
    int ldg = 0;
    float* mu = nullptr;
    float* Pcol = nullptr;
    const float* Kyp = nullptr;
    int kyp_blocks = 0, kyp_ld = 0;
    int n = 0;
    int* frame_counter = nullptr;
    int frames = 0;
    long long* stamps = nullptr;
    int* zero_words = nullptr;
    int n_zero = 0;
    int order2d = 0;
    int lin_blocks = 0;
    int lin_N = 0;
    float lin_dt = 0.f;
    float* lin_FA = nullptr;
    float* lin_FB = nullptr;
    float* lin_FD = nullptr;
    float* lin_mu_next = nullptr;
    int mean_keep = 0;
    int sym_w = 1;
    int sym = 0;
    const int* abort = nullptr;
};
struct GemmCall {
    int M = 0, N = 0, K = 0;
    bool transB = false;
    bool flush = false, lowerB = false;
    float alpha = 1.f, beta = 0.f;
    const float *A = nullptr, *B = nullptr, *Cin = nullptr;
    float* C = nullptr;
    int lda = 0, ldb = 0, ldcin = 0, ldc = 0;
    GemmEpi epi;
    int variant = 0;
};
inline GemmShape gemm_shape(const GemmCall& c) {
    GemmShape s;
    s.M = c.M, s.N = c.N, s.K = c.K, s.transB = c.transB, s.lowerB = c.lowerB;
    s.epi = c.epi.mode, s.mean = c.epi.n > 0, s.lin_blocks = c.epi.lin_blocks, s.sym = c.epi.sym != 0, s.variant = c.variant;
    return s;
}
void launch_gemm(ekfvio_filter* f, const GemmCall& c);

struct BookArgs {
    int enabled = 0;
    int N = 0, m_pad = 0;
    const float* z = nullptr;
    const float* R = nullptr;
    const uint8_t* pass = nullptr;
    float* last_klt = nullptr;
    uint8_t* del_flag = nullptr;
    int* idx = nullptr;
    int* inv_idx = nullptr;
    float* zrow = nullptr;
    float* Rm = nullptr;
    const int* frame_counter = nullptr;
    int* m_out = nullptr;
    uint8_t* pass_eff = nullptr;
    const float* mu = nullptr;
    const float* P = nullptr;
    int ldp = 0;
    float chi2 = 0.f;
    float* d2 = nullptr;
    uint8_t* gated = nullptr;
    int* gate_words = nullptr;
    int count_total = 0;
};
BookArgs make_book_args(ekfvio_filter* f, int m, const float* d_z, const float* d_R, const uint8_t* d_pass, const int* d_frame_counter);
void launch_linearize(ekfvio_filter* f, float dt, const BookArgs* book = nullptr);
void launch_build_dense_F(ekfvio_filter* f, float* Fdense);
bool launch_predict(ekfvio_filter* f, float dt, const BookArgs* book = nullptr, bool prelinearized = false);
struct UpdateInputs {
    int m = 0;
    const float *z = nullptr, *R = nullptr;
    const uint8_t* pass = nullptr;
    int* frame_counter = nullptr;
    int frames = 0;
    bool bookkeeping_done = false;
    bool m_on_device = false;
    bool gate_counted = false;
    float next_dt = -1.f;
    int publish_seq = 0;
    int (*between)(ekfvio_filter*, int kyp_blocks) = nullptr;
    bool recoverable = true;
};
struct UpdateResult {
    bool published = false;
    int between_seq = 0;
    bool linearised_next = false;
};
UpdateResult launch_update(ekfvio_filter* f, const UpdateInputs& in);
void launch_check_sigma(ekfvio_filter* f, float* d_out);
int klt_level_pitch(int w);
int klt_border();
void klt_intrinsics(const ekfvio_filter* f, const float* K, float* fx, float* fy, float* cx, float* cy);
struct Level0View {
    const uint8_t* img = nullptr;
    int pitch = 0, w = 0, h = 0;
    float fx = 0.f, fy = 0.f, cx = 0.f, cy = 0.f;
};
Level0View klt_level0(const ekfvio_filter* f);
inline size_t out_cov_offset(const ekfvio_filter* f) { return EKF_BASE + 4 * (size_t)(f->cfg.max_features > 0 ? f->cfg.max_features : 1); }
inline size_t out_ids_offset(const ekfvio_filter* f) {
    return (out_cov_offset(f) + 72 + 9 * (size_t)(f->cfg.max_features > 0 ? f->cfg.max_features : 1) + 1) & ~(size_t)1;
}
// ... 86 lines not shown
```

### ekf_vio_amd/csrc/ekf_kernels.hip

```cpp
#include <algorithm>
#include <utility>

#include "common.h"

namespace {

#include "motion_model.inc"

template <int NT, bool EFF = false>
__device__ __forceinline__ void bookkeeping_body(const BookArgs& a) {
    __shared__ int s_cnt[32];
    __shared__ int s_total;
    const int tid = threadIdx.x;
    const int N = a.N, m_pad = a.m_pad;
    const float* z = a.z;
    const float* R = a.R;
    const uint8_t* pass = a.pass;
    if (a.frame_counter) {
        const int fi = *a.frame_counter;
        z += (size_t)fi * 2 * N;
        R += (size_t)fi * 4 * N;
        pass += (size_t)fi * N;
    }
    if (EFF) pass = a.pass_eff;
// ... 667 lines not shown
};
static TailGemms update_tail_gemms(ekfvio_filter* f, const UpdatePlan& p, const float* from, float* to) {
    const int n = f->n, ld = f->ldp;
    TailGemms t;
    GemmCall c;
    c.M = c.N = n, c.K = p.m_pad, c.transB = true, c.lda = c.ldb = c.ldcin = c.ldc = ld, c.beta = 1.f, c.Cin = from, c.C = to;
    t.g[0] = t.g[1] = c;
    GemmCall& g2 = t.g[1];
    if (p.tail != TAIL_JOSEPH) {
        t.count = 1;
        GemmCall& g = t.g[0];
        g.A = f->Km, g.B = f->Gm, g.flush = true, g.epi.mode = EPI_MEAN;
        return t;
    }
    t.count = 2;
    GemmCall& g1 = t.g[0];
    g1.N = n + 1, g1.alpha = -1.f, g1.A = f->Km, g1.B = f->Wt;
    g1.epi.mode = EPI_JOSEPH1, g1.epi.inv_idx = f->inv_idx, g1.epi.Rm = f->Rm, g1.epi.G = f->Gm, g1.epi.ldg = ld;
    g2.A = f->Gm, g2.B = f->Km, g2.Cin = to, g2.flush = true, g2.epi.mode = EPI_MEAN, g2.epi.sym = 1;
    return t;
}

UpdateResult launch_update(ekfvio_filter* f, const UpdateInputs& in) {
    const bool gate = f->gate_chi2 > 0.f && f->N > 0;
    const UpdatePlan p = plan_update(f, in.m, in.m_on_device || (gate && in.m > 0), in.next_dt, in.recoverable);
    const int m = p.m, m_pad = p.m_pad, n_pad = p.n_pad, n = f->n, ld = f->ldp;
    UpdateResult out;
    f->last_m = m;
    {
        ProfScope ps(f, PC_GATHER);
        if (!in.bookkeeping_done) {
            BookArgs bk = make_book_args(f, m, in.z, in.R, in.pass, in.frame_counter);
            if (p.m_on_device) bk.m_out = f->info + 2;
            if (gate) {
                bk.pass_eff = f->gate_pass, bk.mu = f->mu, bk.P = f->P, bk.ldp = ld, bk.chi2 = f->gate_chi2;
                bk.d2 = f->gate_d2, bk.gated = f->gate_flag, bk.gate_words = f->gate_words, bk.count_total = in.gate_counted ? 0 : 1;
                hipLaunchKernelGGL(gate_bookkeeping_kernel, dim3(1), dim3(1024), 0, f->stream, bk);
            } else
                hipLaunchKernelGGL(update_bookkeeping_kernel, dim3(1), dim3(1024), 0, f->stream, bk);
        }
        if (p.fused_gather) {
            launch_gather_potrf(f, p);
        } else if (m > 0 && p.sweep != SWEEP_PERSIST_FUSED) {
            const GatherArgs ga = make_gather_args(f, p);
            const int nb2 = p.with_wt ? (m_pad / 64) * (ld / 64) : 0;
            hipLaunchKernelGGL(gather_kernel, dim3(ga.nb1 + nb2), dim3(256), 0, f->stream, ga);
        }
    }
    if (m <= 0) {
        ProfScope ps(f, PC_UPDATE_MISC);
        hipLaunchKernelGGL(mean_update_kernel, dim3((n + 63) / 64), dim3(256), 0, f->stream, f->Km, ld, n, 0, f->yres, f->mu,
                           in.frame_counter, in.frames);
        return out;
    }
    const bool zero_flags = p.persistent() && !p.fused_gather && !f->sweep_flags_clean;
    const int* abort = p.sweep == SWEEP_PERSIST_FUSED ? launch_persist_fused(f, p, zero_flags)
                                                      : launch_chol_sweep(f, p, f->Saug, f->Laug, f->Linv, f->ld_aug, zero_flags);
    if (in.publish_seq) launch_publish_status(f, in.publish_seq), out.published = true;
    TailGemms tail = update_tail_gemms(f, p, p.tail == TAIL_T2 ? t2_buffer(f) : f->P, f->P);
    GemmEpi& e2 = tail.last().epi;
    e2.mu = f->mu, e2.Pcol = f->P + (size_t)n * ld, e2.n = n;
    e2.frame_counter = in.frame_counter, e2.frames = in.frames;
    e2.abort = abort;
    if (p.persistent()) {
        e2.zero_words = f->sweep_sync, e2.n_zero = persist_zero_words(m_pad, n_pad);
        f->sweep_flags_clean = true;
    }
    if (p.tail == TAIL_T2) f->t2_updates++;
    if (p.gain == GAIN_SCHUR) launch_joseph_g(f, m, m_pad, n_pad, p.m_on_device);
    else if (p.gain == GAIN2_T2_TILES) launch_gain2_tiles(f, p);
    else if (p.gain != GAIN_SWEEP) launch_gain_from_sweep(f, p, f->Laug, f->ld_aug, n, f->Km, f->Gm, ld, 0);
    if (p.tail == TAIL_JOSEPH) {
        tail.g[0].epi.abort = abort;
        ProfScope ps(f, PC_GEMM_UPDATE, 2.0 * n * (double)(n + 1) * m_pad + 2.0 * n * (double)n * m_pad, 2);
        launch_gemm(f, tail.g[0]);
        if (in.between) out.between_seq = in.between(f, 0);
        launch_gemm(f, tail.g[1]);
        return out;
    }
    if (p.tail == TAIL_T2 && in.between) out.between_seq = in.between(f, m_pad / 64);
    ProfScope ps(f, PC_GEMM_UPDATE, 2.0 * n * (double)n * m_pad, 1);
    e2.mode = EPI_MEAN_PARTIAL;
    e2.Kyp = f->Wt, e2.kyp_blocks = m_pad / 64, e2.kyp_ld = ld;
    if (p.lin_blocks) {
        e2.lin_blocks = p.lin_blocks, e2.lin_N = f->N, e2.lin_dt = in.next_dt;
        e2.lin_FA = f->FA, e2.lin_FB = f->FB, e2.lin_FD = f->FD, e2.lin_mu_next = f->mu_next;
        out.linearised_next = true;
    }
    launch_gemm(f, tail.last());
    return out;
}

int launch_update_gemms_scratch(ekfvio_filter* f, const UpdatePlan& p, int reps, double* last_flops) {
    TailGemms tail = update_tail_gemms(f, p, f->P, f->P2);
    for (int r = 0; r < reps; r++)
        for (int k = 0; k < tail.count; k++) launch_gemm(f, tail.g[k]);
    const GemmShape sh = gemm_shape(tail.last());
    *last_flops = gemm_executed_flops(sh, plan_gemm(f->tune, f->num_cus, sh));
    return tail.count;
}

void launch_check_sigma(ekfvio_filter* f, float* d_out) {
    hipLaunchKernelGGL(check_sigma_kernel, dim3(1), dim3(256), 0, f->stream, f->P, f->ldp, f->n, d_out);
}
```

### ekf_vio_amd/csrc/gather_body.inc

```
struct GatherArgs {
    const float* P;
    int ld, n;
    const int* idx;
    const float* Rm;
    int m, m_pad, n_pad;
    const int* m_dev;
    float* Saug;
    int lda;
    float* Wt;
    const float* zrow;
    const float* mu;
    float* G;
    int gx, nb1;
    int* zero_words;
    int n_zero;
};

__device__ __forceinline__ float gather_a_elem(float sigma_cr, int r, int c, int m, float rd, float ro) {
    if (r < m && c < m) {
        float v = sigma_cr;
        if (r == c)
            v = v + rd;
        else if ((r ^ 1) == c)
            v = v + ro;
        return v;
    }
    return (r == c) ? 1.f : 0.f;
}

template <bool WT>
__device__ __forceinline__ void gather_st(float* p, float v) {
    if constexpr (WT) __hip_atomic_store(p, v, __ATOMIC_RELAXED, __HIP_MEMORY_SCOPE_AGENT);
    else *p = v;
}
template <bool WT = false>
__device__ __forceinline__ void gather_body(const GatherArgs& a, int block, float* tile ) {
    const float* __restrict__ P = a.P;
    const int* __restrict__ idx = a.idx;
    const int ld = a.ld, n = a.n, m = a.m_dev ? *a.m_dev : a.m, m_pad = a.m_pad, n_pad = a.n_pad, lda = a.lda;
    float* Saug = a.Saug;
    if (block >= a.nb1) {
        const int tb = block - a.nb1, tiles_c = m_pad / 64;
        const int c0 = (tb % tiles_c) * 64, i0 = (tb / tiles_c) * 64;
        const int l64 = threadIdx.x & 63, q4 = threadIdx.x >> 6;
        const int c = c0 + l64;
        const int sc = (c < m) ? idx[c] : -1;
        float wv[16];
        const int scl = max(sc, 0);
#pragma unroll
        for (int ps = 0; ps < 16; ps++) {
            const int i = min(i0 + q4 + 4 * ps, n - 1);
            wv[ps] = P[(size_t)i * ld + scl];
        }
#pragma unroll
        for (int ps = 0; ps < 16; ps++) asm volatile("" : "+v"(wv[ps]));
        const bool has_n = (n >= i0 && n < i0 + 64);
        const float ny = (has_n && sc >= 0) ? -(a.zrow[c] - a.mu[sc]) : 0.f;
#pragma unroll
        for (int ps = 0; ps < 16; ps++) {
            const int ii = q4 + 4 * ps;
            float w = (sc >= 0 && i0 + ii < n) ? wv[ps] : 0.f;
            if (i0 + ii == n) w = ny;
            tile[ii * 65 + l64] = w;
        }
        __syncthreads();
        const int i = i0 + l64;
#pragma unroll
        for (int ps = 0; ps < 16; ps++) {
            const int cc = q4 + 4 * ps, cw = c0 + cc;
            if (i < ld) {
                a.Wt[(size_t)cw * ld + i] = tile[l64 * 65 + cc];
                if (cw >= m) a.G[(size_t)cw * ld + i] = 0.f;
            }
        }
        return;
    }
    const int x = (block % a.gx) * blockDim.x + threadIdx.x;
    const int r = x;
    const int ir = (r < m) ? idx[r] : 0;
    const float rd = (r < m) ? a.Rm[2 * r] : 0.f, ro = (r < m) ? a.Rm[2 * r + 1] : 0.f;
    constexpr int GCT = GC * GCI;
    const int cbase = (block / a.gx) * GCT;
    int scv[GCT];
    float sv[GCT], cv[GCT];
#pragma unroll
    for (int q = 0; q < GCT; q++) scv[q] = (cbase + q < m) ? idx[cbase + q] : 0;
#pragma unroll
    for (int q = 0; q < GCT; q++) {
        const int c = cbase + q;
        sv[q] = (x < m_pad && r < m && c < m) ? P[(size_t)ir * ld + scv[q]] : 0.f;
        cv[q] = (x < ld && c < m && x < n) ? P[(size_t)scv[q] * ld + x] : 0.f;
    }
#pragma unroll
    for (int q = 0; q < GCT; q++) {
        asm volatile("" : "+v"(sv[q]));
        asm volatile("" : "+v"(cv[q]));
    }
#pragma unroll
    for (int q = 0; q < GCT; q++) {
        const int c = cbase + q;
        if (x < m_pad) {
            gather_st<WT>(Saug + (size_t)c * lda + r, gather_a_elem(sv[q], r, c, m, rd, ro));
            gather_st<WT>(Saug + (size_t)c * lda + m_pad + n_pad + r, (r == c) ? 1.f : 0.f);
        }
        if (x < ld) {
            if (x < n_pad) gather_st<WT>(Saug + (size_t)c * lda + m_pad + x, cv[q]);
            if (c >= m) a.G[(size_t)c * ld + x] = 0.f;
        }
    }
}

static GatherArgs make_gather_args(ekfvio_filter* f, const UpdatePlan& p) {
    const int m_pad = p.m_pad;
    GatherArgs a;
    a.P = f->P;
    a.ld = f->ldp;
    a.n = f->n;
    a.idx = f->idx;
    a.Rm = f->Rm;
    a.m = p.m;
    a.m_dev = p.m_on_device ? f->info + 2 : nullptr;
    a.m_pad = m_pad;
    a.n_pad = p.n_pad;
    a.Saug = f->Saug;
    a.lda = f->ld_aug;
    a.Wt = f->Wt;
    a.zrow = f->yres;
    a.mu = f->mu;
    a.G = f->Gm;
    a.gx = gather_gx(f->ldp, m_pad);
    a.nb1 = gather_element_wgs(f->ldp, m_pad);
    a.zero_words = nullptr;
    a.n_zero = 0;
    return a;
}
```

### ekf_vio_amd/csrc/gemm.hip

```cpp
#include "common.h"

#include <algorithm>

typedef float f32x16 __attribute__((ext_vector_type(16)));
typedef float f32x4 __attribute__((ext_vector_type(4)));

namespace {
#include "motion_model.inc"
}

#ifdef EKF_GEMM_STAMPS
#define GSTAMP(i)                                                                                  \
    do {                                                                                           \
        if (stamps_ && (i) < 40) stamps_[i] = (long long)__builtin_amdgcn_s_memtime();             \
    } while (0)
#else
#define GSTAMP(i) do { } while (0)
#endif

#define BM 64
#define BN 64
#define BK 32
#define LDS_A (BM)
#define LDS_BT (BN)
#define LDS_BN (BN + 1)

template <bool TRANSB, int GROUPS, int EPI>
__global__ __launch_bounds__(256 * GROUPS) void gemm_f32_mfma_kernel(int M, int N, int K, float alpha, const float* __restrict__ A,
                                                            int lda, const float* __restrict__ B, int ldb, float beta,
                                                            const float* Cin, int ldcin, float* C, int ldc, int flush,
                                                            int lowerB, GemmEpi epi) {
    __shared__ __attribute__((aligned(16))) float AsG[GROUPS][2][BK * LDS_A];
    __shared__ __attribute__((aligned(16))) float BsG[GROUPS][2][BK * LDS_BN];
    constexpr int LDB_S = TRANSB ? LDS_BT : LDS_BN;

#ifdef EKF_GEMM_STAMPS
    long long* stamps_ = (blockIdx.x == 1 && blockIdx.y == 1 && threadIdx.x == 0) ? epi.stamps : nullptr;
#endif
    GSTAMP(0);
    const int grp = (GROUPS > 1) ? (threadIdx.x >> 8) : 0;
    float (*As)[BK * LDS_A] = AsG[grp];
    float (*Bs)[BK * LDS_BN] = BsG[grp];
    const int tid = threadIdx.x & 255;
    const int lane = tid & 63;
    const int wave = tid >> 6;
    const int wr = wave & 1;
    const int wc = wave >> 1;
    int bx = blockIdx.x, by = blockIdx.y;
    if (EPI == 2 && epi.sym) {
        const int T = gridDim.x, L = (int)blockIdx.x;
        const int bq = T >> 3, br = T & 7, xcd = L & 7;
        int t = xcd * bq + min(xcd, br) + (L >> 3);
        const int tn = (N + BN - 1) / BN;
        int c0 = 0, w = 1;
        for (;;) {
            w = min(epi.sym_w, tn - c0);
            const int cnt = w * (w - 1) / 2 + w * (tn - c0 - (w - 1));
            if (t < cnt || c0 + w >= tn) break;
            t -= cnt;
            c0 += w;
        }
        const int head = w * (w - 1) / 2;
        if (t < head) {
            int r = 0;
            while (t >= r + 1) {
                t -= r + 1;
                r++;
            }
            bx = c0 + r;
            by = c0 + t;
        } else {
            t -= head;
            const int r = t / w;
            bx = c0 + (w - 1) + r;
            by = c0 + (t - r * w);
        }
    } else if (epi.order2d) {
        const int tm = gridDim.x, tn = gridDim.y, T = tm * tn;
        const int L = (int)blockIdx.x + (int)blockIdx.y * tm;
        const int bq = T >> 3, br = T & 7, xcd = L & 7;
        const int swz = xcd * bq + min(xcd, br) + (L >> 3);
        const int W = (tn + 7) >> 3, per = tm * W;
        const int st = swz / per, within = swz - st * per;
        const int wcs = min(W, tn - st * W);
        bx = within / wcs;
        by = st * W + within - bx * wcs;
    }
    const int i0 = bx * BM;
    const int j0 = by * BN;

    const int a_k = tid >> 4;
    const int a_i = (tid & 15) * 4;
    const int b_j = tid >> 2;
    const int b_k = (tid & 3) * 4;

    const int kbeg0 = lowerB ? min(j0, K) : 0;
    const int KTall = (K - kbeg0) / BK;
    const int KTm = (KTall + GROUPS - 1) / GROUPS;
    const int KT = max(0, min(KTm, KTall - grp * KTm));
    const int kbeg = kbeg0 + grp * KTm * BK;
    const float* Ap = A + (size_t)(kbeg + a_k) * lda + i0 + a_i;
    const float* Bp = TRANSB ? (B + (size_t)(kbeg + a_k) * ldb + j0 + a_i) : (B + (size_t)(j0 + b_j) * ldb + kbeg + b_k);
    const size_t a_step = (size_t)BK * lda, b_step = TRANSB ? (size_t)BK * ldb : (size_t)BK;
    const size_t a_half = (size_t)16 * lda, b_half = TRANSB ? (size_t)16 * ldb : (size_t)16;

    f32x16 acc;
#pragma unroll
    for (int r = 0; r < 16; r++) acc[r] = 0.f;
    const int li = lane & 31;
    const int lk = lane >> 5;
    int sweep_aborted = 0;
    if (EPI != 0 && epi.abort) sweep_aborted = *epi.abort;

    float4 xa0, xa1, xb0, xb1;
    xa0 = xa1 = xb0 = xb1 = make_float4(0.f, 0.f, 0.f, 0.f);
    float Fa[BK / 2], Fb[BK / 2], Ga[BK / 2], Gb[BK / 2];
#pragma unroll
    for (int kk = 0; kk < BK / 2; kk++) Fa[kk] = Fb[kk] = Ga[kk] = Gb[kk] = 0.f;

#define GEMM_LOAD(kt)                                                      \
    do {                                                                   \
        const float* ap_ = Ap + (size_t)(kt) * a_step;                     \
        const float* bp_ = Bp + (size_t)(kt) * b_step;                     \
        xa0 = *reinterpret_cast<const float4*>(ap_);                       \
        xa1 = *reinterpret_cast<const float4*>(ap_ + a_half);              \
        xb0 = *reinterpret_cast<const float4*>(bp_);                       \
        xb1 = *reinterpret_cast<const float4*>(bp_ + b_half);              \
    } while (0)
#define GEMM_STAGE_A0(buf) *reinterpret_cast<float4*>(&As[buf][a_k * LDS_A + a_i]) = xa0
#define GEMM_STAGE_A1(buf) *reinterpret_cast<float4*>(&As[buf][(a_k + 16) * LDS_A + a_i]) = xa1
#define GEMM_STAGE_B0(buf)                                                                          \
    do {                                                                                            \
        if (TRANSB) {                                                                               \
            *reinterpret_cast<float4*>(&Bs[buf][a_k * LDS_BT + a_i]) = xb0;                         \
        } else {                                                                                    \
            float* b_ = &Bs[buf][b_k * LDS_BN + b_j];                                               \
            b_[0] = xb0.x; b_[LDS_BN] = xb0.y; b_[2 * LDS_BN] = xb0.z; b_[3 * LDS_BN] = xb0.w;      \
        }                                                                                           \
    } while (0)
#define GEMM_STAGE_B1(buf)                                                                          \
    do {                                                                                            \
        if (TRANSB) {                                                                               \
            *reinterpret_cast<float4*>(&Bs[buf][(a_k + 16) * LDS_BT + a_i]) = xb1;                  \
        } else {                                                                                    \
            float* b_ = &Bs[buf][(b_k + 16) * LDS_BN + b_j];                                        \
            b_[0] = xb1.x; b_[LDS_BN] = xb1.y; b_[2 * LDS_BN] = xb1.z; b_[3 * LDS_BN] = xb1.w;      \
        }                                                                                           \
    } while (0)
#define GEMM_STAGE(buf)    \
    do {                   \
        GEMM_STAGE_A0(buf); \
        GEMM_STAGE_A1(buf); \
        GEMM_STAGE_B0(buf); \
        GEMM_STAGE_B1(buf); \
    } while (0)
#define GEMM_FRAGS(S, buf)                                                         \
    do {                                                                           \
        const float* as_ = &As[buf][lk * LDS_A + wr * 32 + li];                    \
        const float* bs_ = &Bs[buf][lk * LDB_S + wc * 32 + li];                    \
        _Pragma("unroll") for (int kk = 0; kk < BK / 2; kk++) {                    \
            S##a[kk] = as_[2 * kk * LDS_A];                                        \
            S##b[kk] = bs_[2 * kk * LDB_S];                                        \
        }                                                                          \
    } while (0)
#define GEMM_MFMA1(S, kk) acc = __builtin_amdgcn_mfma_f32_32x32x2f32(S##b[kk], S##a[kk], acc, 0, 0, 0)
#define GEMM_TILE(C, Nx, nb, sb, act, fr, stg, ld, lt)                                         \
    do {                                                                                       \
        const float* as_ = &As[nb][lk * LDS_A + wr * 32 + li];                                 \
        const float* bs_ = &Bs[nb][lk * LDB_S + wc * 32 + li];                                 \
        const float* ap_ = Ap + (size_t)(lt) * a_step;                                         \
        const float* bp_ = Bp + (size_t)(lt) * b_step;                                         \
        _Pragma("unroll") for (int sl = 0; sl < 16; sl++) {                                    \
            if (act) GEMM_MFMA1(C, sl);                                                        \
            if (sl < 8 && (fr)) {                                                              \
                Nx##a[2 * sl] = as_[(4 * sl) * LDS_A];                                         \
                Nx##a[2 * sl + 1] = as_[(4 * sl + 2) * LDS_A];                                 \
                Nx##b[2 * sl] = bs_[(4 * sl) * LDB_S];                                         \
                Nx##b[2 * sl + 1] = bs_[(4 * sl + 2) * LDB_S];                                 \
            }                                                                                  \
            if (stg) {                                                                         \
                if (sl == 8) GEMM_STAGE_A0(sb);                                                \
                if (sl == 9) GEMM_STAGE_A1(sb);                                                \
                if (sl == 10) GEMM_STAGE_B0(sb);                                               \
                if (sl == 11) GEMM_STAGE_B1(sb);                                               \
            }                                                                                  \
            if (ld) {                                                                          \
                if (sl == 12) xa0 = *reinterpret_cast<const float4*>(ap_);                     \
                if (sl == 13) xa1 = *reinterpret_cast<const float4*>(ap_ + a_half);            \
                if (sl == 14) xb0 = *reinterpret_cast<const float4*>(bp_);                     \
                if (sl == 15) xb1 = *reinterpret_cast<const float4*>(bp_ + b_half);            \
            }                                                                                  \
            __builtin_amdgcn_sched_barrier(0);                                                 \
        }                                                                                      \
    } while (0)

    const int ci_ = i0 + wr * 32 + li;
    float cpre[16];
#pragma unroll
    for (int r = 0; r < 16; r++) {
        const int j = j0 + wc * 32 + (r & 3) + 8 * (r >> 2) + 4 * lk;
        cpre[r] = (beta != 0.f && ci_ < M && j < N) ? Cin[(size_t)j * ldcin + ci_] : 0.f;
    }
    {
        float4 ya0, ya1, yb0, yb1;
        ya0 = ya1 = yb0 = yb1 = make_float4(0.f, 0.f, 0.f, 0.f);
        if (KT > 0) GEMM_LOAD(0);
        if (KT > 1) {
            const float* ap_ = Ap + a_step;
            const float* bp_ = Bp + b_step;
            ya0 = *reinterpret_cast<const float4*>(ap_);
            ya1 = *reinterpret_cast<const float4*>(ap_ + a_half);
            yb0 = *reinterpret_cast<const float4*>(bp_);
            yb1 = *reinterpret_cast<const float4*>(bp_ + b_half);
        }
        if (KT > 0) GEMM_STAGE(0);
        __syncthreads();
        if (KT > 0) GEMM_FRAGS(F, 0);
        xa0 = ya0; xa1 = ya1; xb0 = yb0; xb1 = yb1;
        if (KT > 1) GEMM_STAGE(1);
        if (KT > 2) GEMM_LOAD(2);
        __syncthreads();
    }
    GSTAMP(1);
    const int klast = KT > 0 ? KT - 1 : 0;
    const bool any = KT > 0;
    int kt = 0;
    for (; kt + 1 < KTm; kt += 2) {
        GEMM_TILE(F, G, 1, 0, kt < KT, any, any, any, min(kt + 3, klast));
        __syncthreads();
        GSTAMP(2 + kt);
        GEMM_TILE(G, F, 0, 1, kt + 1 < KT, any, any, any, min(kt + 4, klast));
        __syncthreads();
        GSTAMP(3 + kt);
    }
    if (kt < KTm) {
        GEMM_TILE(F, G, 1, 0, kt < KT, false, false, false, klast);
        __syncthreads();
    }
    GSTAMP(36);
    if (GROUPS > 1) {
        float* red = &AsG[0][0][0];
        if (grp == 1) {
#pragma unroll
            for (int r = 0; r < 16; r++) red[r * 256 + tid] = acc[r];
        }
        __syncthreads();
        if (grp == 1) return;
#pragma unroll
        for (int r = 0; r < 16; r++) acc[r] += red[r * 256 + tid];
    }
#undef GEMM_LOAD
#undef GEMM_STAGE
#undef GEMM_STAGE_A0
#undef GEMM_STAGE_A1
#undef GEMM_STAGE_B0
#undef GEMM_STAGE_B1
#undef GEMM_FRAGS
#undef GEMM_MFMA1
#undef GEMM_TILE

    GSTAMP(37);
    if (EPI != 0 && sweep_aborted) return;
    const int i = i0 + wr * 32 + li;
    float vout[16];
#pragma unroll
    for (int r = 0; r < 16; r++) {
        float v = alpha * acc[r];
        v = v + beta * cpre[r];
        if (flush) v = (fabsf(v) > EKF_FLUSH_THRESH) ? v : 0.f;
        vout[r] = v;
    }
    if (EPI == 1) {
        const int ic = min(i, M - 1);
        int qv[16];
#pragma unroll
        for (int r = 0; r < 16; r++) {
            const int j = j0 + wc * 32 + 4 * lk + (r & 3) + 8 * (r >> 2);
            qv[r] = epi.inv_idx[min(j, N - 1)];
        }
        float kq[16], kp[16];
#pragma unroll
        for (int r = 0; r < 16; r++) {
            const int q = max(qv[r], 0);
            kq[r] = A[(size_t)q * lda + ic] * epi.Rm[2 * q];
            kp[r] = A[(size_t)(q ^ 1) * lda + ic] * epi.Rm[2 * q + 1];
        }
#pragma unroll
        for (int r = 0; r < 16; r++) {
            const int j = j0 + wc * 32 + 4 * lk + (r & 3) + 8 * (r >> 2);
            const int q = qv[r];
            const float kr = ((q ^ 1) < q) ? (kp[r] + kq[r]) : (kq[r] + kp[r]);
            if (q >= 0 && j < N && i < M) epi.G[(size_t)q * epi.ldg + i] = kr - vout[r];
        }
    }
    if ((EPI == 2 || EPI == 3) && bx == 0 && by == 0 && epi.n > 0) {
        __shared__ float s_q[4];
        for (int e = threadIdx.x; e < epi.n; e += 256 * GROUPS) {
            float v;
            if (EPI == 3) {
                float ky = epi.Kyp[e];
                for (int cb = 1; cb < epi.kyp_blocks; cb++) ky = ky + epi.Kyp[(size_t)cb * epi.kyp_ld + e];
                v = epi.mu[e] + ky;
            } else {
                v = epi.mu[e] + epi.Pcol[e];
                epi.Pcol[e] = 0.f;
            }
            if (e >= 3 && e <= 6) s_q[e - 3] = v;
            else epi.mu[e] = v;
        }
        __syncthreads();
        if (threadIdx.x < 4) {
            const float qn = sqrtf(s_q[0] * s_q[0] + s_q[1] * s_q[1] + s_q[2] * s_q[2] + s_q[3] * s_q[3]);
            epi.mu[3 + threadIdx.x] = s_q[threadIdx.x] / qn;
        }
        if (threadIdx.x == 0 && epi.frame_counter) {
            const int fi = *epi.frame_counter + 1;
            *epi.frame_counter = (fi >= epi.frames) ? 0 : fi;
        }
        for (int e = threadIdx.x; e < epi.n_zero; e += 256 * GROUPS) epi.zero_words[e] = 0;
    }
    float* cp = C + (size_t)(j0 + wc * 32 + 4 * lk) * ldc + i;
    if (i0 + BM <= M && j0 + BN <= N) {
#pragma unroll
        for (int r = 0; r < 16; r++) cp[(size_t)((r & 3) + 8 * (r >> 2)) * ldc] = vout[r];
    } else if (i < M) {
#pragma unroll
        for (int r = 0; r < 16; r++) {
            const int jo = (r & 3) + 8 * (r >> 2);
            if (j0 + wc * 32 + 4 * lk + jo < N) cp[(size_t)jo * ldc] = vout[r];
        }
    }
    if (EPI == 2 && epi.sym && bx != by) {
        static_assert(!TRANSB || 2 * BK * LDS_BN >= 64 * 65, "turning tile");
        float* tr = &BsG[0][0][0];
        __syncthreads();
        const int il = wr * 32 + li;
#pragma unroll
        for (int r = 0; r < 16; r++) tr[il * 65 + wc * 32 + 4 * lk + (r & 3) + 8 * (r >> 2)] = vout[r];
        __syncthreads();
        const int jm = j0 + il;
#pragma unroll
        for (int r = 0; r < 16; r++) {
            const int io = wc * 32 + 4 * lk + (r & 3) + 8 * (r >> 2);
            if (jm < N && i0 + io < M) C[(size_t)(i0 + io) * ldc + jm] = tr[io * 65 + il];
        }
    }
    GSTAMP(38);
}


template <int EPI>
__device__ __forceinline__ void gemm16_finish_mean(const GemmEpi& epi) {
    __shared__ float s_q[4];
    int aborted = 0;
    if (epi.abort) aborted = *epi.abort;
    const bool keep = EPI == 3 && epi.mean_keep;
    float v4[4] = {0.f, 0.f, 0.f, 0.f};
#pragma unroll
    for (int u = 0; u < 4; u++) {
        if (keep) break;
        const int e = min((int)threadIdx.x + 256 * u, epi.n - 1);
        if (EPI == 3) {
            float pk[16];
#pragma unroll
            for (int cb = 0; cb < 16; cb++) pk[cb] = epi.Kyp[(size_t)min(cb, epi.kyp_blocks - 1) * epi.kyp_ld + e];
            const float m0 = epi.mu[e];
            float ky = pk[0];
#pragma unroll
            for (int cb = 1; cb < 16; cb++) ky = (cb < epi.kyp_blocks) ? ky + pk[cb] : ky;
            for (int cb = 16; cb < epi.kyp_blocks; cb++) ky = ky + epi.Kyp[(size_t)cb * epi.kyp_ld + e];
            v4[u] = m0 + ky;
        } else {
            v4[u] = epi.mu[e] + epi.Pcol[e];
        }
    }
    if (aborted) return;
#pragma unroll
    for (int u = 0; u < 4; u++) {
        const int e = (int)threadIdx.x + 256 * u;
        if (e < epi.n && !keep) {
            if (EPI != 3) epi.Pcol[e] = 0.f;
            if (e >= 3 && e <= 6) s_q[e - 3] = v4[u];
            else epi.mu[e] = v4[u];
        }
    }
    for (int e = threadIdx.x + 1024; e < (keep ? 0 : epi.n); e += 256) {
        float v;
        if (EPI == 3) {
            float ky = epi.Kyp[e];
            for (int cb = 1; cb < epi.kyp_blocks; cb++) ky = ky + epi.Kyp[(size_t)cb * epi.kyp_ld + e];
            v = epi.mu[e] + ky;
        } else {
            v = epi.mu[e] + epi.Pcol[e];
            epi.Pcol[e] = 0.f;
        }
        epi.mu[e] = v;
    }
    __builtin_amdgcn_s_waitcnt(0xc07f);
    __builtin_amdgcn_s_barrier();
    if (threadIdx.x < 4 && !keep) {
        const float qn = sqrtf(s_q[0] * s_q[0] + s_q[1] * s_q[1] + s_q[2] * s_q[2] + s_q[3] * s_q[3]);
        epi.mu[3 + threadIdx.x] = s_q[threadIdx.x] / qn;
    }
    if (threadIdx.x == 0 && epi.frame_counter) {
        const int fi = *epi.frame_counter + 1;
        *epi.frame_counter = (fi >= epi.frames) ? 0 : fi;
    }
    for (int e = threadIdx.x; e < epi.n_zero; e += 256) epi.zero_words[e] = 0;
}

template <int BMt, int WPS, int EPI>
__global__ __launch_bounds__(256 * WPS) void gemm16_kernel(int M, int N, int K, float alpha, const float* __restrict__ A, int lda,
                                                     const float* __restrict__ B, int ldb, float beta, const float* Cin,
                                                     int ldcin, float* C, int ldc, int flush, int lowerB, GemmEpi epi,
                                                     int tiles_x, int tiles_y) {
    constexpr int RB = BMt / 16;
    constexpr int SA = (BMt % 32 == 16) ? BMt : BMt + 16;
    constexpr int SB = 80;
    constexpr int BKK = 64;
    constexpr int NT = 256 * WPS;
    constexpr int AVT = BKK * BMt / 4;
    constexpr int AV = (AVT + NT - 1) / NT;
    constexpr int BV = BKK * 64 / 4 / NT;
    constexpr int BKS = NT / 16;
    constexpr int NS = BKK / 4 / WPS;
    __shared__ __attribute__((aligned(16))) float As[3][BKK * SA];
    __shared__ __attribute__((aligned(16))) float Bs[3][BKK * SB];

    if ((EPI == 2 || EPI == 3) && (int)blockIdx.x == tiles_x * tiles_y) {
        if (threadIdx.x >= 256) return;
        if (epi.n > 0) gemm16_finish_mean<EPI>(epi);
        return;
    }
    if (EPI == 3 && (int)blockIdx.x > tiles_x * tiles_y) {
        if (threadIdx.x >= 256) return;
        const int tid = threadIdx.x;
        const int lb = (int)blockIdx.x - tiles_x * tiles_y - 1;
        LinLds& l = *reinterpret_cast<LinLds*>(&As[0][0]);
        static_assert(sizeof(LinLds) <= sizeof(As), "linearisation scratch");
        float* s_mu = &Bs[0][0];
        int aborted = 0;
        if (epi.abort) aborted = *epi.abort;
        constexpr int NE = EKF_BASE + 3 * LIN_LM;
        if (tid < NE) {
            const int e = (tid < EKF_BASE) ? tid : min(EKF_BASE + 3 * LIN_LM * lb + (tid - EKF_BASE), epi.n - 1);
            float pk[16];
#pragma unroll
            for (int cb = 0; cb < 16; cb++) pk[cb] = epi.Kyp[(size_t)min(cb, epi.kyp_blocks - 1) * epi.kyp_ld + e];
            const float m0 = epi.mu[e];
            float ky = pk[0];
#pragma unroll
            for (int cb = 1; cb < 16; cb++) ky = (cb < epi.kyp_blocks) ? ky + pk[cb] : ky;
            for (int cb = 16; cb < epi.kyp_blocks; cb++) ky = ky + epi.Kyp[(size_t)cb * epi.kyp_ld + e];
            s_mu[tid] = aborted ? m0 : m0 + ky;
        }
        __syncthreads();
        if (tid < 4 && !aborted) {
            const float qn = sqrtf(s_mu[3] * s_mu[3] + s_mu[4] * s_mu[4] + s_mu[5] * s_mu[5] + s_mu[6] * s_mu[6]);
            const float qv = s_mu[3 + tid] / qn;
            s_mu[3 + tid] = qv;
        }
        __syncthreads();
        const int e0 = EKF_BASE + 3 * LIN_LM * lb;
        auto mean = [s_mu, e0](int e) { return (e < EKF_BASE) ? s_mu[e] : s_mu[EKF_BASE + (e - e0)]; };
        linearize_block(mean, epi.lin_N, epi.lin_dt, epi.lin_FA, epi.lin_FB, epi.lin_FD, epi.lin_mu_next, lb, epi.lin_blocks - 1, l, tid);
        return;
    }
    const int nwg = tiles_x * tiles_y;
    const int bq = nwg >> 3, br = nwg & 7, xcd = blockIdx.x & 7;
    const int swz = xcd * bq + min(xcd, br) + (blockIdx.x >> 3);
    const int ti = swz % tiles_x, tj = swz / tiles_x;
    const int i0 = ti * BMt;
    const int j0 = tj * 64;

#ifdef EKF_GEMM_STAMPS
    long long* stamps_ = (blockIdx.x == 9 && threadIdx.x == 0) ? epi.stamps : nullptr;
#endif
    GSTAMP(0);
    const int tid = threadIdx.x, lane = tid & 63;
    const int wave = (tid >> 6) & 3;
    const int kg = tid >> 8;
    const int li = lane & 15, g = lane >> 4;
    const int Mread = (M + 63) & ~63;

    const int kbeg = lowerB ? min(j0, K) : 0;
    const int KT = (K - kbeg) / BKK;

#define G16_ACOORD(u)                                                                       \
    const int ea##u = min(tid + NT * u, AVT - 1);                                           \
    const int ao##u = ((ea##u / (BMt / 4)) * lda + min(i0 + (ea##u % (BMt / 4)) * 4, Mread - 4)) * 4;  \
    const int al##u = (ea##u / (BMt / 4)) * SA + (ea##u % (BMt / 4)) * 4;
    G16_ACOORD(0) G16_ACOORD(1) G16_ACOORD(2) G16_ACOORD(3)
#undef G16_ACOORD
    const __amdgpu_buffer_rsrc_t rsA = __builtin_amdgcn_make_buffer_rsrc(const_cast<float*>(A), 0, K * lda * 4, 0x00020000);
    const __amdgpu_buffer_rsrc_t rsB = __builtin_amdgcn_make_buffer_rsrc(const_cast<float*>(B), 0, K * ldb * 4, 0x00020000);
    const int bo = ((tid >> 4) * ldb + j0 + (tid & 15) * 4) * 4;
    const int bl = (tid >> 4) * SB + (tid & 15) * 4;
    const int a_step = BKK * lda * 4, b_step = BKK * ldb * 4, b_rows = BKS * ldb * 4;
    const int a_base = kbeg * lda * 4, b_base = kbeg * ldb * 4;
    static_assert((BV == 4 || BV == 2) && AV >= 1 && AV <= 4, "staging is written for 1..4 float4 of A and 2 or 4 of B per thread");

    f32x4 acc[RB];
#pragma unroll
    for (int a = 0; a < RB; a++) acc[a] = f32x4{0.f, 0.f, 0.f, 0.f};
    int sweep_aborted = 0;
    if (EPI != 0 && epi.abort) sweep_aborted = *epi.abort;

    float cpre[RB][4];
#pragma unroll
    for (int a = 0; a < RB; a++)
#pragma unroll
        for (int v = 0; v < 4; v++) {
            const int i = i0 + 16 * a + li, j = j0 + 16 * wave + 4 * g + v;
            cpre[a][v] = (beta != 0.f && i < M && j < N) ? Cin[(size_t)j * ldcin + i] : 0.f;
        }

    int qv[4] = {-1, -1, -1, -1};
    float kq[RB][4], kp[RB][4];
    if (EPI == 1 && kg == 0) {
        const int jbq = j0 + 16 * wave + 4 * g;
#pragma unroll
        for (int v = 0; v < 4; v++) qv[v] = epi.inv_idx[min(jbq + v, N - 1)];
#pragma unroll
        for (int a = 0; a < RB; a++) {
            const int ic = min(i0 + 16 * a + li, M - 1);
#pragma unroll
            for (int v = 0; v < 4; v++) {
                const int q = max(qv[v], 0);
                kq[a][v] = A[(size_t)q * lda + ic] * epi.Rm[2 * q];
                kp[a][v] = A[(size_t)(q ^ 1) * lda + ic] * epi.Rm[2 * q + 1];
            }
        }
    }
    float4 Xa0, Xa1, Xa2, Xa3, Xb0, Xb1, Xb2, Xb3, Ya0, Ya1, Ya2, Ya3, Yb0, Yb1, Yb2, Yb3;
    float4 Za0, Za1, Za2, Za3, Zb0, Zb1, Zb2, Zb3;
    Xa0 = Xa1 = Xa2 = Xa3 = Xb0 = Xb1 = Xb2 = Xb3 = make_float4(0.f, 0.f, 0.f, 0.f);
    Ya0 = Ya1 = Ya2 = Ya3 = Yb0 = Yb1 = Yb2 = Yb3 = make_float4(0.f, 0.f, 0.f, 0.f);
    Za0 = Za1 = Za2 = Za3 = Zb0 = Zb1 = Zb2 = Zb3 = make_float4(0.f, 0.f, 0.f, 0.f);
#define G16_LOAD(S, kt)                                                                                \
    do {                                                                                               \
        const int sa_ = a_base + (kt) * a_step, sb_ = b_base + (kt) * b_step;                          \
        S##a0 = __builtin_bit_cast(float4, __builtin_amdgcn_raw_buffer_load_b128(rsA, ao0, sa_, 0));                                                               \
        if constexpr (AV > 1) S##a1 = __builtin_bit_cast(float4, __builtin_amdgcn_raw_buffer_load_b128(rsA, ao1, sa_, 0));                                         \
        if constexpr (AV > 2) S##a2 = __builtin_bit_cast(float4, __builtin_amdgcn_raw_buffer_load_b128(rsA, ao2, sa_, 0));                                         \
        if constexpr (AV > 3) S##a3 = __builtin_bit_cast(float4, __builtin_amdgcn_raw_buffer_load_b128(rsA, ao3, sa_, 0));                                         \
        S##b0 = __builtin_bit_cast(float4, __builtin_amdgcn_raw_buffer_load_b128(rsB, bo, sb_, 0));                                                                \
        S##b1 = __builtin_bit_cast(float4, __builtin_amdgcn_raw_buffer_load_b128(rsB, bo + b_rows, sb_, 0));                                                       \
        if constexpr (BV > 2) S##b2 = __builtin_bit_cast(float4, __builtin_amdgcn_raw_buffer_load_b128(rsB, bo + 2 * b_rows, sb_, 0));                             \
        if constexpr (BV > 2) S##b3 = __builtin_bit_cast(float4, __builtin_amdgcn_raw_buffer_load_b128(rsB, bo + 3 * b_rows, sb_, 0));                             \
    } while (0)
#define G16_LOADI(S, j, kt)                                                                            \
    do {                                                                                               \
        const int sa_ = a_base + (kt) * a_step, sb_ = b_base + (kt) * b_step;                          \
        if ((j) == 0) S##a0 = __builtin_bit_cast(float4, __builtin_amdgcn_raw_buffer_load_b128(rsA, ao0, sa_, 0));                                                 \
        if ((j) == 1 && AV > 1) S##a1 = __builtin_bit_cast(float4, __builtin_amdgcn_raw_buffer_load_b128(rsA, ao1, sa_, 0));                                       \
        if ((j) == 2 && AV > 2) S##a2 = __builtin_bit_cast(float4, __builtin_amdgcn_raw_buffer_load_b128(rsA, ao2, sa_, 0));                                       \
        if ((j) == 3 && AV > 3) S##a3 = __builtin_bit_cast(float4, __builtin_amdgcn_raw_buffer_load_b128(rsA, ao3, sa_, 0));                                       \
        if ((j) == AV) S##b0 = __builtin_bit_cast(float4, __builtin_amdgcn_raw_buffer_load_b128(rsB, bo, sb_, 0));                                                 \
        if ((j) == AV + 1) S##b1 = __builtin_bit_cast(float4, __builtin_amdgcn_raw_buffer_load_b128(rsB, bo + b_rows, sb_, 0));                                    \
        if ((j) == AV + 2 && BV > 2) S##b2 = __builtin_bit_cast(float4, __builtin_amdgcn_raw_buffer_load_b128(rsB, bo + 2 * b_rows, sb_, 0));                      \
        if ((j) == AV + 3 && BV > 2) S##b3 = __builtin_bit_cast(float4, __builtin_amdgcn_raw_buffer_load_b128(rsB, bo + 3 * b_rows, sb_, 0));                      \
    } while (0)
#define G16_STAGEI(S, j, buf)                                                                          \
    do {                                                                                               \
        if ((j) == 0) *reinterpret_cast<float4*>(&As[buf][al0]) = S##a0;                               \
        if ((j) == 1 && AV > 1) *reinterpret_cast<float4*>(&As[buf][al1]) = S##a1;                     \
        if ((j) == 2 && AV > 2) *reinterpret_cast<float4*>(&As[buf][al2]) = S##a2;                     \
        if ((j) == 3 && AV > 3) *reinterpret_cast<float4*>(&As[buf][al3]) = S##a3;                     \
        if ((j) == AV) *reinterpret_cast<float4*>(&Bs[buf][bl]) = S##b0;                               \
        if ((j) == AV + 1) *reinterpret_cast<float4*>(&Bs[buf][bl + BKS * SB]) = S##b1;                \
        if ((j) == AV + 2 && BV > 2) *reinterpret_cast<float4*>(&Bs[buf][bl + 2 * BKS * SB]) = S##b2;  \
        if ((j) == AV + 3 && BV > 2) *reinterpret_cast<float4*>(&Bs[buf][bl + 3 * BKS * SB]) = S##b3;  \
    } while (0)
#define G16_STAGE_A(S, buf)                                                                            \
    do {                                                                                               \
        *reinterpret_cast<float4*>(&As[buf][al0]) = S##a0;  \
        if constexpr (AV > 1) *reinterpret_cast<float4*>(&As[buf][al1]) = S##a1;                       \
        if constexpr (AV > 2) *reinterpret_cast<float4*>(&As[buf][al2]) = S##a2;                       \
        if constexpr (AV > 3) *reinterpret_cast<float4*>(&As[buf][al3]) = S##a3;                       \
    } while (0)
#define G16_STAGE_B(S, buf)                                                                            \
    do {                                                                                               \
        *reinterpret_cast<float4*>(&Bs[buf][bl]) = S##b0;                                              \
        *reinterpret_cast<float4*>(&Bs[buf][bl + BKS * SB]) = S##b1;                                   \
        if constexpr (BV > 2) *reinterpret_cast<float4*>(&Bs[buf][bl + 2 * BKS * SB]) = S##b2;         \
        if constexpr (BV > 2) *reinterpret_cast<float4*>(&Bs[buf][bl + 3 * BKS * SB]) = S##b3;         \
    } while (0)
#define G16_MFMA(c, b, a) c = __builtin_amdgcn_mfma_f32_16x16x4f32(b, a, c, 0, 0, 0)
#ifndef G16X_NOLOAD
#define G16X_NOLOAD 0
#endif
#ifndef G16X_NOSTAGE
#define G16X_NOSTAGE 0
#endif
#ifndef G16X_NOBAR
#define G16X_NOBAR 0
#endif
#ifndef G16X_NOFR
#define G16X_NOFR 0
#endif
#define G16_FR(P, st, slot)                                                               \
    do {                                                                                  \
        if (G16X_NOFR) break;                                                             \
        fb[slot] = P##b[(4 * WPS * (st)) * SB];                                           \
        _Pragma("unroll") for (int a = 0; a < RB; a++) fa[slot][a] = P##a[(4 * WPS * (st)) * SA + 16 * a]; \
    } while (0)
#define G16_TILE(S1, S2, tcur)                                                            \
    do {                                                                                  \
        const int nxt = (cb == 2) ? 0 : cb + 1;                                           \
        na = &As[nxt][(g + 4 * kg) * SA + li];                                            \
        nb = &Bs[nxt][(g + 4 * kg) * SB + 16 * wave + li];                                \
        _Pragma("unroll") for (int st = 0; st < NS; st++) {                               \
            if (st + 2 < NS) G16_FR(p, st + 2, (st + 2) % 4);                             \
            _Pragma("unroll") for (int a = 0; a < RB; a++)                                \
                G16_MFMA(acc[a], fb[st % 4], fa[st % 4][a]);                              \
               \
                   \
            if (!G16X_NOLOAD) G16_LOADI(S2, st, (tcur) + 3);                              \
            if (!G16X_NOSTAGE) G16_STAGEI(S1, st, nxt);                                   \
            if (st == BAR && !G16X_NOBAR) __syncthreads();                                \
            if (st == NS - 2) G16_FR(n, 0, 0);                                            \
            if (st == NS - 1) G16_FR(n, 1, 1);                                            \
            __builtin_amdgcn_sched_barrier(0);                                            \
        }                                                                                 \
        cb = nxt;                                                                         \
        pa = na;                                                                          \
        pb = nb;                                                                          \
    } while (0)

    if (KT > 0) {
        constexpr int BAR = AV + BV;
        static_assert(BAR <= NS - 3 && NS % 4 == 0, "step schedule");
        G16_LOAD(Z, 0);
        G16_LOAD(X, 1);
        G16_LOAD(Y, 2);
        G16_STAGE_A(Z, 0);
        G16_STAGE_B(Z, 0);
        __syncthreads();
        float fa[4][RB], fb[4];
        int cb = 0;
        const float* pa = &As[0][(g + 4 * kg) * SA + li];
        const float* pb = &Bs[0][(g + 4 * kg) * SB + 16 * wave + li];
        const float* na = pa;
        const float* nb = pb;
        G16_FR(n, 0, 0);
        G16_FR(n, 1, 1);
        GSTAMP(1);
        int t = 0;
        for (; t + 2 < KT; t += 3) {
            G16_TILE(X, Z, t);
            GSTAMP(2 + t);
            G16_TILE(Y, X, t + 1);
            GSTAMP(3 + t);
            G16_TILE(Z, Y, t + 2);
            GSTAMP(4 + t);
        }
        if (t < KT) {
            G16_TILE(X, Z, t);
            t++;
        }
        if (t < KT) G16_TILE(Y, X, t);
        GSTAMP(36);
        __syncthreads();
    }
#undef G16_TILE
#undef G16_FR
#undef G16_LOAD
#undef G16_LOADI
#undef G16_STAGEI
#undef G16_STAGE_A
#undef G16_STAGE_B
    if constexpr (WPS > 1) {
        float* red = &As[0][0];
        static_assert(3 * BKK * SA >= RB * 4 * 256, "reduction scratch");
        if (kg == 1) {
#pragma unroll
            for (int a = 0; a < RB; a++)
#pragma unroll
                for (int v = 0; v < 4; v++) red[(a * 4 + v) * 256 + (tid & 255)] = acc[a][v];
        }
        __syncthreads();
        if (kg == 1) return;
#pragma unroll
        for (int a = 0; a < RB; a++)
#pragma unroll
            for (int v = 0; v < 4; v++) acc[a][v] += red[(a * 4 + v) * 256 + tid];
    }

    GSTAMP(37);
    if (EPI != 0 && sweep_aborted) return;
    float vout[RB][4];
#pragma unroll
    for (int a = 0; a < RB; a++)
#pragma unroll
        for (int v = 0; v < 4; v++) {
            float x = alpha * acc[a][v];
            x = x + beta * cpre[a][v];
            if (flush) x = (fabsf(x) > EKF_FLUSH_THRESH) ? x : 0.f;
            vout[a][v] = x;
        }
    const int jb = j0 + 16 * wave + 4 * g;
    if (EPI == 1) {
#pragma unroll
        for (int a = 0; a < RB; a++) {
            const int i = i0 + 16 * a + li;
#pragma unroll
            for (int v = 0; v < 4; v++) {
                const int q = qv[v];
                const float kr = ((q ^ 1) < q) ? (kp[a][v] + kq[a][v]) : (kq[a][v] + kp[a][v]);
                if (q >= 0 && jb + v < N && i < M) epi.G[(size_t)q * epi.ldg + i] = kr - vout[a][v];
            }
        }
    }
    float* cp = C + (size_t)jb * ldc + i0 + li;
    if (i0 + BMt <= M && j0 + 64 <= N) {
#pragma unroll
        for (int a = 0; a < RB; a++)
#pragma unroll
            for (int v = 0; v < 4; v++) cp[(size_t)v * ldc + 16 * a] = vout[a][v];
    } else {
#pragma unroll
        for (int a = 0; a < RB; a++) {
            if (i0 + 16 * a + li < M) {
#pragma unroll
                for (int v = 0; v < 4; v++)
                    if (jb + v < N) cp[(size_t)v * ldc + 16 * a] = vout[a][v];
            }
        }
    }
    GSTAMP(38);
}

void launch_gemm(ekfvio_filter* f, const GemmCall& c) {
    const int M = c.M, N = c.N, K = c.K;
    if (M <= 0 || N <= 0 || K <= 0) return;
    GemmEpi e = c.epi;
    const GemmPlan p = plan_gemm(f->tune, f->num_cus, gemm_shape(c));
    hipStream_t s = f->stream;
    e.stamps = f->gemm_stamps;
    e.lin_blocks = p.lin_blocks, e.mean_keep = p.mean_keep;
    const dim3 grid(p.grid_x, p.grid_y), block(p.threads());
    const int flush = c.flush, lowerB = c.lowerB;
    if (p.k16) {
#define GEMM16_GO(BMv, W, EP)                                                                                                     \
    hipLaunchKernelGGL((gemm16_kernel<BMv, W, EP>), grid, block, 0, s, M, N, K, c.alpha, c.A, c.lda, c.B, c.ldb, c.beta, c.Cin, c.ldcin, \
                       c.C, c.ldc, flush, lowerB, e, p.tiles_x, p.tiles_y)
#define GEMM16_BM(W, EP)                            \
    do {                                            \
        if (p.bm == 32) GEMM16_GO(32, W, EP);       \
        else if (p.bm == 48) GEMM16_GO(48, W, EP);  \
        else GEMM16_GO(64, W, EP);                  \
    } while (0)
        if (e.mode == EPI_JOSEPH1) GEMM16_BM(2, 1);
        else if (e.mode == EPI_MEAN) GEMM16_BM(2, 2);
        else if (e.mode == EPI_MEAN_PARTIAL) GEMM16_BM(2, 3);
        else if (p.wps == 2) GEMM16_BM(2, 0);
        else GEMM16_BM(1, 0);
#undef GEMM16_BM
#undef GEMM16_GO
        return;
    }
    e.sym = p.sym, e.sym_w = p.sym_w, e.order2d = p.order2d;
#define GEMM_GO(TB, G, EP)                                                                                                        \
    hipLaunchKernelGGL((gemm_f32_mfma_kernel<TB, G, EP>), grid, block, 0, s, M, N, K, c.alpha, c.A, c.lda, c.B, c.ldb, c.beta, c.Cin, \
                       c.ldcin, c.C, c.ldc, flush, lowerB, e)
    if (e.mode == EPI_JOSEPH1) {
        GEMM_GO(true, 1, 1);
    } else if (e.mode == EPI_MEAN) {
        GEMM_GO(true, 1, 2);
    } else if (e.mode == EPI_MEAN_PARTIAL) {
        GEMM_GO(true, 1, 3);
    } else if (p.groups == 2) {
        if (c.transB) GEMM_GO(true, 2, 0);
        else GEMM_GO(false, 2, 0);
    } else {
        if (c.transB) GEMM_GO(true, 1, 0);
        else GEMM_GO(false, 1, 0);
    }
#undef GEMM_GO
}
```

### ekf_vio_amd/filter.py

```python
import ctypes as C

import numpy as np

from . import capi

BASE_STATE_SIZE = 22


def _fp(a):
    return a.ctypes.data_as(C.POINTER(C.c_float))


def _u8(a):
    return a.ctypes.data_as(C.POINTER(C.c_uint8))


class TightlyCoupledEKF:
    def __init__(self, max_features=100, device=0, stream=None, predict_mode=capi.PREDICT_STRUCTURED,
                 default_point_depth=0.5, default_point_depth_variance=100.0,
                 default_point_homogenous_variance=1e-5, hooks=False, gate_chi2=0.0, klt_fb_max_px=0.0, distortion=None, output_covariance=False,
                 mask=None, mask_rectify_border=False, equalize=None, klt_photometric=False, ended_export=False, zupt=None,
                 **cfg_overrides):
        self.hooks = bool(hooks)
        self.lib = capi.load(hooks=self.hooks)
# ... 267 lines not shown

    def set_state(self, st):
        base = np.ascontiguousarray(st["base_mu"], dtype=np.float32)
        feat = np.ascontiguousarray(st["feat_mu"], dtype=np.float32).reshape(-1, 3)
        N = feat.shape[0]
        klt = np.ascontiguousarray(st["last_klt"], dtype=np.float32).reshape(N, 2)
        dele = np.ascontiguousarray(st["del_flag"], dtype=np.uint8).reshape(N)
        sig = np.ascontiguousarray(np.asarray(st["Sigma"], dtype=np.float32).T)
        n = BASE_STATE_SIZE + 3 * N
        self._chk(self.lib.ekfvio_set_state(self.h, N, _fp(base), _fp(feat), _fp(klt), _u8(dele), _fp(sig), n))

    def upload_measurements(self, z, R, passed):
        z = np.ascontiguousarray(z, dtype=np.float32)
        R = np.ascontiguousarray(R, dtype=np.float32)
        p = np.ascontiguousarray(passed, dtype=np.uint8)
        frames = p.shape[0]
        self._chk(self.lib.ekfvio_upload_measurements(self.h, frames, _fp(z), _fp(R), _u8(p)))

    def run_uploaded(self, first, count, dt):
        self._chk(self.lib.ekfvio_run_uploaded(self.h, first, count, float(dt)))

    def synchronize(self):
        return self._chk(self.lib.ekfvio_synchronize(self.h), allow=(capi.ENUMERIC,))

    def profile(self, on):
        self._chk(self.lib.ekfvio_profile_enable(self.h, int(on)))
        if on:
            self._chk(self.lib.ekfvio_profile_reset(self.h))

    def profile_report(self):
        out = {}
        for c in range(self.lib.ekfvio_profile_count()):
            ms, n, fl = C.c_double(0), C.c_int64(0), C.c_double(0)
            self._chk(self.lib.ekfvio_profile_get(self.h, c, C.byref(ms), C.byref(n), C.byref(fl)))
            out[self.lib.ekfvio_profile_name(c).decode()] = dict(ms=ms.value, launches=n.value, flops=fl.value)
        return out

    def profile_update_gemms(self, reps=50):
        us, fl = C.c_double(0), C.c_double(0)
        self._chk(self.lib.ekfvio_profile_update_gemms(self.h, int(reps), C.byref(us), C.byref(fl)))
        return us.value, fl.value

    def test_gemm(self, A, B, C0, alpha=1.0, beta=0.0, transB=True, variant=0):
        self._need_hooks()
        A = np.asarray(A, np.float32)
        B = np.asarray(B, np.float32)
        M, K = A.shape
        N = B.shape[0] if transB else B.shape[1]
        Ac, Bc = np.array(A.T, order="C", copy=True), np.array(B.T, order="C", copy=True)
        Cc = np.array(np.asarray(C0, np.float32).T, order="C", copy=True)
        self._chk(self.lib.ekfvio_test_gemm(self.h, int(transB), M, N, K, alpha, _fp(Ac), M, _fp(Bc), B.shape[0], beta,
                                            _fp(Cc), M, int(variant)))
        return Cc.T.copy()

    def counters(self):
        c = (C.c_int64 * 8)()
        self._chk(self.lib.ekfvio_get_counters(self.h, c))
        return dict(persistent=int(c[0]), schur=int(c[1]), recoveries=int(c[2]), mode=int(c[3]), early_output_frames=int(c[4]), t2_updates=int(c[5]),
                    graph_steps=int(c[6]), prelinearized_steps=int(c[7]))

    def _need_hooks(self):
        if not self.hooks:
            raise RuntimeError("this entry point exists only in the hooks build: construct the filter with hooks=True")

    def persistent_sweeps(self):
        return self.counters()["persistent"]

    def sweep_counts(self):
        c = self.counters()
        return {k: c[k] for k in ("persistent", "schur", "recoveries", "mode")}

    def sweep_fault(self, spin_limit=0, stall_workgroup=-1):
        self._need_hooks()
        self._chk(self.lib.ekfvio_test_sweep_fault(self.h, int(spin_limit), int(stall_workgroup)))

    def sweep_delay(self, workgroup=-1, point=0, ticks=0):
        self._need_hooks()
        self._chk(self.lib.ekfvio_test_sweep_delay(self.h, int(workgroup), int(point), int(ticks)))

    def fill_update_scratch(self, word):
        self._need_hooks()
        self._chk(self.lib.ekfvio_test_fill_update_scratch(self.h, int(word) & 0xFFFFFFFF))

    def test_cholesky_solve(self, S, Crhs):
        self._need_hooks()
        S = np.asarray(S, np.float32)
        Crhs = np.asarray(Crhs, np.float32)
        m, nr = S.shape[0], Crhs.shape[0]
        Sc, Cc = np.array(S.T, order="C", copy=True), np.array(Crhs.T, order="C", copy=True)
        L = np.zeros((m, m), np.float32)
        X = np.zeros((m, nr), np.float32)
        info = C.c_int32(0)
        self._chk(self.lib.ekfvio_test_cholesky_solve(self.h, m, nr, _fp(Sc), _fp(Cc), _fp(L), _fp(X), C.byref(info)))
        return L.T.copy(), X.T.copy(), info.value


class KLTTracker:

    def __init__(self, ekf):
        self.ekf = ekf
        self.lib = ekf.lib

    def push_frame(self, img, K):
        img = np.ascontiguousarray(img, dtype=np.uint8)
        h, w = img.shape
        K = np.ascontiguousarray(K, dtype=np.float32).reshape(9)
        self.ekf._chk(self.lib.ekfvio_klt_push_frame(self.ekf.h, _u8(img), w, h, w, _fp(K)))

    def findNewFeaturePositions(self):
        N = self.ekf.num_features
        z = np.zeros((N, 2), np.float32)
        R = np.zeros((N, 4), np.float32)
        p = np.zeros(N, np.uint8)
        self.ekf._chk(self.lib.ekfvio_klt_track(self.ekf.h, _fp(z), _fp(R), _u8(p)))
        return z, R, p

    def track_points(self, prev_px, init_px):
        pp = np.ascontiguousarray(prev_px, dtype=np.float32).reshape(-1, 2)
        ii = np.ascontiguousarray(init_px, dtype=np.float32).reshape(-1, 2)
        out = np.zeros_like(pp)
        st = np.zeros(pp.shape[0], np.uint8)
        self.ekf._chk(self.lib.ekfvio_klt_track_points(self.ekf.h, _fp(pp), _fp(ii), pp.shape[0], _fp(out), _u8(st)))
        return out, st

    def track_points_fb(self, prev_px, init_px):
        pp = np.ascontiguousarray(prev_px, dtype=np.float32).reshape(-1, 2)
        ii = np.ascontiguousarray(init_px, dtype=np.float32).reshape(-1, 2)
        out, back = np.zeros_like(pp), np.zeros_like(pp)
        st, ok = np.zeros(pp.shape[0], np.uint8), np.zeros(pp.shape[0], np.uint8)
        e2 = np.zeros(pp.shape[0], np.float32)
        self.ekf._chk(self.lib.ekfvio_klt_track_points_fb(self.ekf.h, _fp(pp), _fp(ii), pp.shape[0], _fp(out), _u8(st), _fp(back), _fp(e2),
                                                          _u8(ok)))
        return out, st, back, e2, ok

    def uncertainty_points(self, ref_px, cur_px):
        rp = np.ascontiguousarray(ref_px, dtype=np.float32).reshape(-1, 2)
        cp = np.ascontiguousarray(cur_px, dtype=np.float32).reshape(-1, 2)
        cov = np.zeros((rp.shape[0], 4), np.float32)
        self.ekf._chk(self.lib.ekfvio_klt_uncertainty_points(self.ekf.h, _fp(rp), _fp(cp), rp.shape[0], _fp(cov)))
        return cov.reshape(-1, 2, 2)

    def level(self, l):
        w, h = C.c_int32(0), C.c_int32(0)
        self.ekf._chk(self.lib.ekfvio_klt_get_level(self.ekf.h, l, C.byref(w), C.byref(h), None, None))
        img = np.zeros((h.value, w.value), np.uint8)
        der = np.zeros((h.value, w.value, 2), np.int16)
        self.ekf._chk(self.lib.ekfvio_klt_get_level(self.ekf.h, l, C.byref(w), C.byref(h), _u8(img),
                                                    der.ctypes.data_as(C.POINTER(C.c_int16))))
        return img, der

    def padded_level(self, l):
        w, h, b = C.c_int32(0), C.c_int32(0), C.c_int32(0)
        self.ekf._chk(self.lib.ekfvio_klt_get_level(self.ekf.h, l, C.byref(w), C.byref(h), None, None))
        self.ekf._chk(self.lib.ekfvio_test_klt_padded_level(self.ekf.h, l, C.byref(b), None, None))
        img = np.zeros((h.value + 2 * b.value, w.value + 2 * b.value), np.uint8)
        der = np.zeros((h.value + 2 * b.value, w.value + 2 * b.value, 2), np.int16)
        self.ekf._chk(self.lib.ekfvio_test_klt_padded_level(self.ekf.h, l, C.byref(b), _u8(img), der.ctypes.data_as(C.POINTER(C.c_int16))))
        return img, der, b.value


def _ip(a):
    return a.ctypes.data_as(C.POINTER(C.c_int32))


def rotation_error_jacobian(q_wxyz):
    lib = capi.load()
# ... 206 lines not shown
```

### include/ekfvio_test_hooks.h

```cpp
#ifndef EKFVIO_TEST_HOOKS_H_
#define EKFVIO_TEST_HOOKS_H_
#include "ekfvio.h"
#ifdef __cplusplus
extern "C" {
#endif

EKFVIO_API int ekfvio_test_klt_padded_level(ekfvio_filter* f, int32_t level, int32_t* border, uint8_t* img, int16_t* deriv);
EKFVIO_API int ekfvio_test_blurred_level0(ekfvio_filter* f, uint8_t* out);
EKFVIO_API int ekfvio_test_gemm(ekfvio_filter* f, int32_t transB, int32_t M, int32_t N, int32_t K, float alpha, const float* A,
                     int32_t lda, const float* B, int32_t ldb, float beta, float* C, int32_t ldc, int32_t variant);
EKFVIO_API int ekfvio_test_gemm_bench(ekfvio_filter* f, int32_t transB, int32_t lowerB, int32_t M, int32_t N, int32_t K,
                           int32_t reps, int32_t variant, double* mean_us);
EKFVIO_API int ekfvio_test_potrf_stamps(ekfvio_filter* f, int64_t stamps[80]);
EKFVIO_API int ekfvio_test_sweep_stamps(ekfvio_filter* f, int enable, int64_t stamps[1024]);
EKFVIO_API int ekfvio_test_sweep_fault(ekfvio_filter* f, int32_t spin_limit, int32_t stall_workgroup);
#define EKFVIO_TEST_SWEEP_DELAY_MAX_TICKS 100000
EKFVIO_API int ekfvio_test_sweep_delay(ekfvio_filter* f, int32_t workgroup, int32_t point, int32_t ticks);
EKFVIO_API int ekfvio_test_cholesky_solve(ekfvio_filter* f, int32_t m, int32_t nrhs, const float* S, const float* Crhs,
                               float* L_out, float* X_out, int32_t* info);
EKFVIO_API int ekfvio_test_plan(int32_t num_cus, int32_t max_features, int32_t N, int32_t m, int32_t m_on_device, int32_t sole_handle,
                                int32_t latched_off, int32_t dense_predict, float next_dt, int32_t plan[12]);
EKFVIO_API int ekfvio_test_gemm_plan(int32_t num_cus, int32_t M, int32_t N, int32_t K, int32_t transB, int32_t lowerB, int32_t epi, int32_t mean,
                                     int32_t lin_blocks, int32_t sym, int32_t variant, int32_t plan[18]);
EKFVIO_API int ekfvio_test_predict_plan(int32_t num_cus, int32_t N, int32_t dense_predict, int32_t prelinearized, int32_t bookkeeping,
                                        int32_t plan[8]);
EKFVIO_API int ekfvio_test_run_plan(int32_t N, int32_t gated, int32_t profiling, int32_t frames, const int32_t* rows, int32_t count, int32_t out[6]);
EKFVIO_API int ekfvio_test_persist_grid(int32_t num_cus, int32_t max_features, int32_t N, int32_t m, int32_t m_on_device, int32_t sole_handle,
                                        int32_t latched_off, int32_t dense_predict, float next_dt, int32_t* roles, int32_t max_blocks,
                                        int32_t out[10]);
EKFVIO_API int ekfvio_test_t2_pair(int32_t p, int32_t pair[2]);
EKFVIO_API int ekfvio_test_mem(ekfvio_filter* f, int64_t out[8]);
EKFVIO_API int ekfvio_test_mem_fail(ekfvio_filter* f, int32_t nth);
EKFVIO_API int ekfvio_test_fill_update_scratch(ekfvio_filter* f, uint32_t word);
EKFVIO_API int ekfvio_test_zupt_decide(ekfvio_filter* f, const float* prev_px, const float* cur_px, const uint8_t* pass, int32_t count,
                                       float max_flow_px, int32_t min_tracks, float min_ratio, float* flow2, int32_t* n_pass, int32_t* n_still,
                                       int32_t* stationary);

#ifdef __cplusplus
}
#endif
#endif
```

Measured before the change: 11030.

## Export T2 rows to gather buffer and subtract in GEMM instead of gain tile

The persistent gain tile no longer computes the W2 correction term, which it used to do from gathered P columns, extra L/S column loads and a third triangular-solve right-hand side. Instead, the T2 tile writes its rows into a new T2m buffer indexed by measurement. The downstream mean-partial GEMM subtracts T2m from its B operand on the fly through a new SUBB template variant. This cuts per-k-block work in the gain tile and starts its k loop at cb, at the cost of an extra buffer, an extra B-sized load stream in the GEMM, and new scattered float4 writes in t2_tile.

```diff
diff --git a/ekf_vio_amd/capi.py b/ekf_vio_amd/capi.py
--- a/ekf_vio_amd/capi.py
+++ b/ekf_vio_amd/capi.py
@@ -48,7 +48,7 @@
 HOOK_SYMBOLS = ["ekfvio_test_klt_padded_level", "ekfvio_test_blurred_level0", "ekfvio_test_gemm", "ekfvio_test_gemm_bench", "ekfvio_test_potrf_stamps",
                 "ekfvio_test_sweep_stamps", "ekfvio_test_sweep_fault", "ekfvio_test_sweep_delay", "ekfvio_test_cholesky_solve", "ekfvio_test_plan", "ekfvio_test_persist_grid", "ekfvio_test_t2_pair",
                 "ekfvio_test_gemm_plan", "ekfvio_test_predict_plan", "ekfvio_test_run_plan", "ekfvio_test_mem", "ekfvio_test_mem_fail",
-                "ekfvio_test_fill_update_scratch", "ekfvio_test_zupt_decide"]
+                "ekfvio_test_fill_update_scratch", "ekfvio_test_update_buffer", "ekfvio_test_zupt_decide"]
 
 _libs = {}
 
@@ -133,6 +133,7 @@
             "ekfvio_test_mem": [vp, C.POINTER(C.c_int64)],
             "ekfvio_test_mem_fail": [vp, i32],
             "ekfvio_test_fill_update_scratch": [vp, C.c_uint32],
+            "ekfvio_test_update_buffer": [vp, i32, fp, C.c_int64],
             "ekfvio_test_zupt_decide": [vp, fp, fp, u8p, i32, f32, i32, f32, fp, ip, ip, ip],
         })
     for name, args in sig.items():
diff --git a/ekf_vio_amd/csrc/api.hip b/ekf_vio_amd/csrc/api.hip
--- a/ekf_vio_amd/csrc/api.hip
+++ b/ekf_vio_amd/csrc/api.hip
@@ -223,6 +223,7 @@
     HIP_TRY(f, dev_alloc(f, &f->Km, pm));
     HIP_TRY(f, dev_alloc(f, &f->Wt, pm));
     HIP_TRY(f, dev_alloc(f, &f->Gm, pm));
+    HIP_TRY(f, dev_alloc(f, &f->T2m, pm));
     HIP_TRY(f, dev_alloc(f, &f->info, 4));
     HIP_TRY(f, dev_alloc(f, &f->remove_words, 4));
     HIP_TRY(f, host_alloc(f, &f->h_info, 16 * sizeof(int), MEM_PINNED_COHERENT));
@@ -1206,7 +1207,7 @@
     const size_t maxf = (size_t)(f->cfg.max_features > 0 ? f->cfg.max_features : 0);
     const size_t aug = (size_t)f->ld_aug * f->m_cap, pm = (size_t)f->ldp * f->m_cap;
     const struct { float* p; size_t count; } regions[] = {
-        {f->Saug, aug}, {f->Laug, aug}, {f->Linv, 64 * (size_t)f->m_cap}, {f->Km, pm}, {f->Wt, pm}, {f->Gm, pm},
+        {f->Saug, aug}, {f->Laug, aug}, {f->Linv, 64 * (size_t)f->m_cap}, {f->Km, pm}, {f->Wt, pm}, {f->Gm, pm}, {f->T2m, pm},
         {f->yres, (size_t)f->m_cap}, {f->Rm, 2 * (size_t)f->m_cap}, {f->Fdense, (size_t)f->ldp * f->ldp},
         {f->FA, (size_t)EKF_BASE * EKF_BASE}, {f->FB, 27 * maxf}, {f->FD, 9 * maxf}, {f->mu_next, (size_t)f->ldp},
     };
@@ -1214,6 +1215,16 @@
         if (r.p && r.count) HIP_TRY(f, hipMemsetD32Async((hipDeviceptr_t)r.p, (int)word, r.count, f->stream));
     return EKFVIO_OK;
 }
+int ekfvio_test_update_buffer(ekfvio_filter* f, int32_t which, float* out, int64_t count) {
+    if (!f || !out || count < 0) return EKFVIO_EINVAL;
+    HIP_TRY(f, hipSetDevice(f->device));
+    const size_t pm = (size_t)f->ldp * f->m_cap;
+    const struct { const float* p; size_t count; } buffers[] = {{f->Km, pm}, {f->Gm, pm}, {f->T2m, pm}, {t2_buffer(f), (size_t)f->ldp * f->ldp}};
+    if (which < 0 || which >= (int32_t)(sizeof(buffers) / sizeof(buffers[0])) || (size_t)count > buffers[which].count) return EKFVIO_EINVAL;
+    HIP_TRY(f, hipStreamSynchronize(f->stream));
+    if (count) HIP_TRY(f, hipMemcpy(out, buffers[which].p, (size_t)count * sizeof(float), hipMemcpyDeviceToHost));
+    return EKFVIO_OK;
+}
 #endif
 
 }
diff --git a/ekf_vio_amd/csrc/chol_persist.inc b/ekf_vio_amd/csrc/chol_persist.inc
--- a/ekf_vio_amd/csrc/chol_persist.inc
+++ b/ekf_vio_amd/csrc/chol_persist.inc
@@ -250,24 +250,17 @@
 }
 
 template <bool WAIT>
-__device__ __forceinline__ void gain_tile2(const PersistArgs& a, const GatherArgs& ga, float* Ti, float* Tj, float* Tl, float* Tinv, float* Th, float* tab,
+__device__ __forceinline__ void gain_tile2(const PersistArgs& a, const GatherArgs& ga, float* Ti, float* Tj, float* Tl, float* Tinv, float* part, float* tab,
                                            int ib, int cb, int tid) {
     const int lane = tid & 63, wave = tid >> 6, wr = wave & 1, wc = wave >> 1;
     const int r = wr * 32 + (lane & 31);
     const int mb = a.mb, ldl = a.ldl;
     const int m = ga.m_dev ? *ga.m_dev : ga.m;
     const __amdgpu_buffer_rsrc_t bL = persist_rsrc(a.L, (unsigned)ldl * (unsigned)(mb * PB));
-    const __amdgpu_buffer_rsrc_t bS = persist_rsrc(a.S, (unsigned)a.lds * (unsigned)(mb * PB));
     const int iy = mb + ib, iz = a.idb0 + cb;
-    const int cq = cb * PB + lane;
-    const int sq = (cq < m) ? ga.idx[cq] : -1;
-    const unsigned sqc = (unsigned)max(sq, 0);
-    int alo = 0, ahi = -1;
-    if (cb * PB < m) {
-        alo = ga.idx[cb * PB] / PB;
-        ahi = ga.idx[min(cb * PB + PB - 1, m - 1)] / PB;
-    }
     if (tid < 64) {
+        const int cq = cb * PB + lane;
+        const int sq = (cq < m) ? ga.idx[cq] : -1;
         float yq = 0.f, rd = 0.f, ro = 0.f;
         if (sq >= 0) {
             yq = ga.zrow[cq] - ga.mu[sq];
@@ -276,118 +269,40 @@
         }
         tab[tid] = yq, tab[64 + tid] = rd, tab[128 + tid] = ro;
     }
-    auto column_flags = [&](int kb, const int* zflag) -> PollLane {
-        const int ax = alo + tid - 2;
-        return {tid == 0 ? a.pan + iy * mb + kb : tid == 1 ? zflag : (tid >= 2 && ax <= ahi) ? a.pan + (mb + ax) * mb + kb : nullptr, 1};
-    };
-    float kv[16], w2[16];
-    {
-        float wv[16];
-        const int scl = max(sq, 0);
-#pragma unroll
-        for (int ps = 0; ps < 16; ps++) wv[ps] = ga.P[(size_t)min(ib * PB + wave + 4 * ps, ga.n - 1) * ga.ld + scl];
-#pragma unroll
-        for (int ps = 0; ps < 16; ps++) asm volatile("" : "+v"(wv[ps]));
-#pragma unroll
-        for (int ps = 0; ps < 16; ps++) Th[(wave + 4 * ps) * 65 + lane] = (sq >= 0 && ib * PB + wave + 4 * ps < ga.n) ? wv[ps] : 0.f;
-        __syncthreads();
-#pragma unroll
-        for (int q = 0; q < 16; q++) {
-            kv[q] = 0.f;
-            w2[q] = Th[r * 65 + mma64_col(wc, lane, q)];
-        }
-    }
-    auto fetch = [&](int kb) -> unsigned long long {
-        const bool gk = kb >= cb;
-        float hv[16];
-        unsigned long long neg;
-        if constexpr (WAIT) {
-            persist_wait(a, column_flags(kb, gk ? a.pan + iz * mb + kb : nullptr), tid, kb < mb - 2);
-            load_tile_sc1(Ti, bL, (unsigned)(kb * PB) * (unsigned)ldl + (unsigned)(iy * PB), ldl, tid);
-            if (gk) load_tile_sc1(Tj, bL, (unsigned)(kb * PB) * (unsigned)ldl + (unsigned)(iz * PB), ldl, tid);
-#pragma unroll
-            for (int ps = 0; ps < 16; ps++)
-                hv[ps] = __builtin_bit_cast(float, __builtin_amdgcn_raw_buffer_load_b32(bL, ((unsigned)(kb * PB + wave + 4 * ps) * (unsigned)ldl + (unsigned)(mb * PB) + sqc) * 4u, 0, 16));
-#pragma unroll
-            for (int ps = 0; ps < 16; ps++) hv[ps] = (sq >= 0) ? hv[ps] : 0.f;
-#pragma unroll
-            for (int ps = 0; ps < 16; ps++) Th[(wave + 4 * ps) * PLD + lane] = hv[ps];
-            neg = ld_sign_sc1(a.Lsign + kb);
-        } else {
-            load_tile(Ti, a.L + (size_t)kb * PB * ldl + (size_t)iy * PB, ldl, tid);
-            if (gk) load_tile(Tj, a.L + (size_t)kb * PB * ldl + (size_t)iz * PB, ldl, tid);
-#pragma unroll
-            for (int ps = 0; ps < 16; ps++) hv[ps] = a.L[(size_t)(kb * PB + wave + 4 * ps) * ldl + (size_t)(mb * PB) + sqc];
-#pragma unroll
-            for (int ps = 0; ps < 16; ps++) hv[ps] = (sq >= 0) ? hv[ps] : 0.f;
-#pragma unroll
-            for (int ps = 0; ps < 16; ps++) Th[(wave + 4 * ps) * PLD + lane] = hv[ps];
-            neg = a.Lsign[kb];
-        }
-        return neg;
-    };
-    auto products = [&](int kb, unsigned long long neg, bool z_unsigned) {
-        if (kb >= cb) {
-            const f32x16 up = (z_unsigned && neg != 0ull) ? mma64_signed(Ti, 1, PLD, Tj, 1, PLD, wr, wc, lane, neg) : mma64(Ti, 1, PLD, Tj, 1, PLD, wr, wc, lane);
-#pragma unroll
-            for (int q = 0; q < 16; q++) kv[q] = kv[q] + up[q];
-        }
-        if (alo <= ahi) {
-            f32x16 up;
-            if constexpr (WAIT) {
-                up = (neg == 0ull) ? mma64(Ti, 1, PLD, Th, 1, PLD, wr, wc, lane) : mma64_signed(Ti, 1, PLD, Th, 1, PLD, wr, wc, lane, neg);
-            } else {
-                if (__builtin_amdgcn_readfirstlane((int)(neg != 0ull))) {
-                    __syncthreads();
-                    sign_cols(Ti, Ti, neg, tid);
-                    __syncthreads();
-                }
-                up = mma64(Ti, 1, PLD, Th, 1, PLD, wr, wc, lane);
-            }
-#pragma unroll
-            for (int q = 0; q < 16; q++) w2[q] = w2[q] - up[q];
-        }
+    float kv[16];
+#pragma unroll
+    for (int q = 0; q < 16; q++) kv[q] = 0.f;
+    auto product = [&](int kb, unsigned long long neg, bool z_unsigned) {
+        const f32x16 up = (z_unsigned && neg != 0ull) ? mma64_signed(Ti, 1, PLD, Tj, 1, PLD, wr, wc, lane, neg) : mma64(Ti, 1, PLD, Tj, 1, PLD, wr, wc, lane);
+#pragma unroll
+        for (int q = 0; q < 16; q++) kv[q] = kv[q] + up[q];
         if (WAIT && a.dbg && tid == 0 && mb <= 8 && (ib == 0 || ib == 6) && (cb == 0 || cb == 3 || cb == 7))
             a.dbg[100 + 8 * ((ib ? 3 : 0) + (cb == 0 ? 0 : cb == 3 ? 1 : 2)) + kb] = (long long)__builtin_amdgcn_s_memrealtime();
     };
     if constexpr (WAIT) {
-        for (int kb = 0; kb < mb - 2; kb++) {
-            __syncthreads();
-            const unsigned long long neg = fetch(kb);
-            __syncthreads();
-            products(kb, neg, false);
-        }
-    } else {
-        for (int kb = 0; kb < mb; kb++) {
-            __syncthreads();
-            const unsigned long long neg = fetch(kb);
-            __syncthreads();
-            products(kb, neg, false);
-        }
-    }
-    if constexpr (WAIT) {
+        for (int kb = cb; kb < mb - 2; kb++) {
+            __syncthreads();
+            persist_wait(a, nullptr, a.pan + iy * mb + kb, a.pan + iz * mb + kb, tid, 1, true);
+            load_tile_sc1(Ti, bL, (unsigned)(kb * PB) * (unsigned)ldl + (unsigned)(iy * PB), ldl, tid);
+            load_tile_sc1(Tj, bL, (unsigned)(kb * PB) * (unsigned)ldl + (unsigned)(iz * PB), ldl, tid);
+            __syncthreads();
+            product(kb, 0ull, false);
+        }
         const int kl = mb - 1, k6 = mb - 2;
         const bool gk6 = k6 >= cb;
+        const __amdgpu_buffer_rsrc_t bS = persist_rsrc(a.S, (unsigned)a.lds * (unsigned)(mb * PB));
         const __amdgpu_buffer_rsrc_t bI = persist_rsrc(a.Linv, (unsigned)(mb * PB * PB));
         const bool zi = a.grid.compact() && cb == kl;
         __syncthreads();
-        persist_wait(a, column_flags(k6, gk6 ? a.pan + iz * mb + k6 : (zi ? nullptr : a.fin + iz * mb + kl)), tid, false);
+        if (cb > mb - 3) persist_wait(a, nullptr, a.pan + iy * mb + (mb - 3), nullptr, tid, 1, true);
+        persist_wait(a, nullptr, a.pan + iy * mb + k6, gk6 ? a.pan + iz * mb + k6 : (zi ? nullptr : a.fin + iz * mb + kl), tid, 1, false);
         RegTile ql, qi, qj;
-        float hq[16];
-        unsigned long long neg6;
-        {
+        if (gk6) {
             RegTile pi6, pj6;
-            float h6[16];
             pi6.request(bL, (unsigned)(k6 * PB) * (unsigned)ldl + (unsigned)(iy * PB), ldl, tid);
-            if (gk6) pj6.request(bL, (unsigned)(k6 * PB) * (unsigned)ldl + (unsigned)(iz * PB), ldl, tid);
-#pragma unroll
-            for (int ps = 0; ps < 16; ps++)
-                h6[ps] = __builtin_bit_cast(float, __builtin_amdgcn_raw_buffer_load_b32(bL, ((unsigned)(k6 * PB + wave + 4 * ps) * (unsigned)ldl + (unsigned)(mb * PB) + sqc) * 4u, 0, 16));
-            neg6 = ld_sign_sc1(a.Lsign + k6);
+            pj6.request(bL, (unsigned)(k6 * PB) * (unsigned)ldl + (unsigned)(iz * PB), ldl, tid);
             pi6.put(Ti, tid);
-            if (gk6) pj6.put(Tj, tid);
-#pragma unroll
-            for (int ps = 0; ps < 16; ps++) Th[(wave + 4 * ps) * PLD + lane] = (sq >= 0) ? h6[ps] : 0.f;
+            pj6.put(Tj, tid);
         }
         persist_wait(a, a.ready + kl, nullptr, nullptr, tid, 4, false);
         ql.request(bL, (unsigned)(kl * PB) * (unsigned)ldl + (unsigned)(kl * PB), ldl, tid);
@@ -395,28 +310,31 @@
         if (!zi) qj.request(bS, (unsigned)(kl * PB) * (unsigned)a.lds + (unsigned)(iz * PB), a.lds, tid);
         const float4 qv = ld_sc1(bI, (unsigned)(kl * PB * PB) + tid * 4);
         const unsigned long long neg7 = ld_sign_sc1(a.Lsign + kl);
-#pragma unroll
-        for (int ps = 0; ps < 16; ps++)
-            hq[ps] = __builtin_bit_cast(float, __builtin_amdgcn_raw_buffer_load_b32(bS, ((unsigned)(kl * PB + wave + 4 * ps) * (unsigned)a.lds + (unsigned)(mb * PB) + sqc) * 4u, 0, 16));
-        products(mb - 2, neg6, false);
+        if (gk6) product(k6, 0ull, false);
         __syncthreads();
         ql.put(Tl, tid);
         qi.put(Ti, tid);
         if (zi) identity_tile(Tj, tid);
         else qj.put(Tj, tid);
         inv_put(qv, Tinv, tid);
-#pragma unroll
-        for (int ps = 0; ps < 16; ps++) Th[(wave + 4 * ps) * PLD + lane] = (sq >= 0) ? hq[ps] : 0.f;
-        __syncthreads();
-        float* const t3[3] = {Ti, Tj, Th};
-        tri_solve_fwd_n<3>(t3, Tl, Tinv, wave, lane);
-        __syncthreads();
-        products(kl, neg7, true);
+        __syncthreads();
+        tri_solve_fwd2(Ti, Tj, Tl, Tinv, wave, lane);
+        __syncthreads();
+        product(kl, neg7, true);
+    } else {
+        for (int kb = cb; kb < mb; kb++) {
+            __syncthreads();
+            load_tile(Ti, a.L + (size_t)kb * PB * ldl + (size_t)iy * PB, ldl, tid);
+            load_tile(Tj, a.L + (size_t)kb * PB * ldl + (size_t)iz * PB, ldl, tid);
+            __syncthreads();
+            product(kb, 0ull, false);
+        }
     }
 #pragma unroll
     for (int q = 0; q < 16; q++) kv[q] = (fabsf(kv[q]) > EKF_FLUSH_THRESH) ? kv[q] : 0.f;
     float* Kt = a.K + (size_t)(cb * PB) * a.ldk + (size_t)ib * PB;
     float* Gt = ga.G + (size_t)(cb * PB) * ga.ld + (size_t)ib * PB;
+    float* Et = ga.T2m + (size_t)(cb * PB) * ga.ld + (size_t)ib * PB;
     float acc = 0.f;
 #pragma unroll
     for (int q = 0; q < 16; q++) {
@@ -426,20 +344,22 @@
         if (cg < m) {
             const float x = kv[q] * tab[64 + c], y = kv[q ^ 1] * tab[128 + c];
             const float kr = ((cg ^ 1) < cg) ? (y + x) : (x + y);
-            g = kr - w2[q];
+            g = kr;
             acc = acc + kv[q] * tab[c];
+        } else {
+            Et[(size_t)c * ga.ld + r] = 0.f;
         }
         Gt[(size_t)c * ga.ld + r] = g;
     }
     __syncthreads();
-    float* part = Th;
     part[(wc * 2 + (lane >> 5)) * 64 + r] = acc;
     __syncthreads();
     if (tid < 64) ga.Wt[(size_t)cb * ga.ld + (size_t)ib * PB + tid] = ((part[tid] + part[64 + tid]) + part[128 + tid]) + part[192 + tid];
 }
 
 template <bool WAIT>
-__device__ __forceinline__ void t2_tile(const PersistArgs& a, float* Ti, float* Tj, float* Tl, float* Tinv, int ta, int tb, int tid, long long* dbg = nullptr) {
+__device__ __forceinline__ void t2_tile(const PersistArgs& a, const GatherArgs& ga, float* Ti, float* Tj, float* Tl, float* Tinv, int ta, int tb, int tid,
+                                        long long* dbg = nullptr) {
     const int lane = tid & 63, wave = tid >> 6, wr = wave & 1, wc = wave >> 1;
     const int r = wr * 32 + (lane & 31);
     const int mb = a.mb, ldl = a.ldl;
@@ -481,6 +401,27 @@
         }
         if (dbg && tid == 0) dbg[kb] = (long long)__builtin_amdgcn_s_memrealtime();
     };
+    int qa[4], qb[4];
+    auto export_map = [&]() {
+        const int m = ga.m_dev ? *ga.m_dev : ga.m;
+#pragma unroll
+        for (int it = 0; it < 4; it++) {
+            const int sa = ta * PB + (tid >> 4) + 16 * it, sb = tb * PB + (tid >> 4) + 16 * it;
+            const int ua = ga.inv_idx[min(sa, a.nstate - 1)], ub = ga.inv_idx[min(sb, a.nstate - 1)];
+            qa[it] = (sa < a.nstate && ua < m) ? ua : -1;
+            qb[it] = (sb < a.nstate && ub < m) ? ub : -1;
+        }
+    };
+    auto export_rows = [&](const float* T, const int (&qs)[4], int cblk) {
+#pragma unroll
+        for (int it = 0; it < 4; it++) {
+            const int rr = (tid >> 4) + 16 * it, c4 = (tid & 15) * 4;
+            if (qs[it] >= 0)
+                *reinterpret_cast<float4*>(ga.T2m + (size_t)qs[it] * ga.ld + (size_t)(cblk * PB + c4)) =
+                    make_float4(T[c4 * PLD + rr], T[(c4 + 1) * PLD + rr], T[(c4 + 2) * PLD + rr], T[(c4 + 3) * PLD + rr]);
+        }
+    };
+    if constexpr (!WAIT) export_map();
     if constexpr (WAIT) {
         for (int kb = 0; kb < mb - 2; kb++) {
             __syncthreads();
@@ -505,6 +446,7 @@
         const int kl = mb - 1, k6 = mb - 2;
         const __amdgpu_buffer_rsrc_t bS = persist_rsrc(a.S, (unsigned)a.lds * (unsigned)(mb * PB));
         const __amdgpu_buffer_rsrc_t bI = persist_rsrc(a.Linv, (unsigned)(mb * PB * PB));
+        export_map();
         __syncthreads();
         persist_wait(a, a.ready + kl, a.pan + ia * mb + k6, diag ? nullptr : a.pan + ib * mb + k6, tid, 4, false);
         RegTile pi6, pj6, ql, qi, qj;
@@ -541,6 +483,8 @@
     __syncthreads();
     store_tile(Ti, a.T2 + (size_t)tb * PB * a.ldt + (size_t)ta * PB, a.ldt, tid);
     if (!diag) store_tile(Tj, a.T2 + (size_t)ta * PB * a.ldt + (size_t)tb * PB, a.ldt, tid);
+    export_rows(Ti, qa, tb);
+    if (!diag) export_rows(Tj, qb, ta);
     if (dbg && tid == 0) dbg[15] = (long long)__builtin_amdgcn_s_memrealtime();
 }
 
@@ -900,7 +844,7 @@
             const int tb = role.n;
             __syncthreads();
             if (role.a < a.idb0 - mb) {
-                if (a.t2) gain_tile2<true>(a, ga, Ti, Tj, Tl, Tinv, persist_dyn_lds, persist_dyn_lds + PB * PLD, role.a, role.b, tid);
+                if (a.t2) gain_tile2<true>(a, ga, Ti, Tj, Tl, Tinv, persist_dyn_lds, persist_dyn_lds + 256, role.a, role.b, tid);
                 else gain_tile(a, Ti, Tj, Tl, Tinv, role.a, role.b, tid);
                 if (a.dbg && tid == 0 && tb < 104) a.dbg[200 + tb] = (long long)__builtin_amdgcn_s_memrealtime();
             }
@@ -1049,7 +993,7 @@
                 td = a.dbg + 840 + 16 * (p == 0 ? 0 : p == np_ - 1 ? 2 : 1);
                 if (tid == 0) td[14] = (long long)__builtin_amdgcn_s_memrealtime();
             }
-            t2_tile<true>(a, Ti, Tj, Tl, Tinv, ta, tb, tid, td);
+            t2_tile<true>(a, ga, Ti, Tj, Tl, Tinv, ta, tb, tid, td);
             if (a.dbg && tid == 0 && p < 91) a.dbg[304 + p] = (long long)__builtin_amdgcn_s_memrealtime();
         }
         PEXIT();
@@ -1140,12 +1084,11 @@
     __shared__ __attribute__((aligned(16))) float Ti[PB * PLD];
     __shared__ __attribute__((aligned(16))) float Tj[PB * PLD];
     __shared__ __attribute__((aligned(16))) float Th[PB * PLD];
-    __shared__ float tab[192];
     if ((int)blockIdx.x < gain_wgs) {
-        gain_tile2<false>(a, ga, Ti, Tj, nullptr, nullptr, Th, tab, (int)blockIdx.x / a.mb, (int)blockIdx.x % a.mb, threadIdx.x);
+        gain_tile2<false>(a, ga, Ti, Tj, nullptr, nullptr, Th, Th + 256, (int)blockIdx.x / a.mb, (int)blockIdx.x % a.mb, threadIdx.x);
     } else {
         int ta, tb;
         t2_pair((int)blockIdx.x - gain_wgs, ta, tb);
-        t2_tile<false>(a, Ti, Tj, Th, nullptr, ta, tb, threadIdx.x);
-    }
-}
+        t2_tile<false>(a, ga, Ti, Tj, Th, nullptr, ta, tb, threadIdx.x);
+    }
+}
diff --git a/ekf_vio_amd/csrc/common.h b/ekf_vio_amd/csrc/common.h
--- a/ekf_vio_amd/csrc/common.h
+++ b/ekf_vio_amd/csrc/common.h
@@ -173,6 +173,7 @@
     float* Km = nullptr;
     float* Wt = nullptr;
     float* Gm = nullptr;
+    float* T2m = nullptr;
     int* info = nullptr;
     float gate_chi2 = 0.f;
     float* gate_d2 = nullptr;
@@ -321,6 +322,7 @@
     int mean_keep = 0;
     int sym_w = 1;
     int sym = 0;
+    const float* Bsub = nullptr;
     const int* abort = nullptr;
 };
 struct GemmCall {
diff --git a/ekf_vio_amd/csrc/ekf_kernels.hip b/ekf_vio_amd/csrc/ekf_kernels.hip
--- a/ekf_vio_amd/csrc/ekf_kernels.hip
+++ b/ekf_vio_amd/csrc/ekf_kernels.hip
@@ -773,6 +773,7 @@
     ProfScope ps(f, PC_GEMM_UPDATE, 2.0 * n * (double)n * m_pad, 1);
     e2.mode = EPI_MEAN_PARTIAL;
     e2.Kyp = f->Wt, e2.kyp_blocks = m_pad / 64, e2.kyp_ld = ld;
+    if (p.tail == TAIL_T2) e2.Bsub = f->T2m;
     if (p.lin_blocks) {
         e2.lin_blocks = p.lin_blocks, e2.lin_N = f->N, e2.lin_dt = in.next_dt;
         e2.lin_FA = f->FA, e2.lin_FB = f->FB, e2.lin_FD = f->FD, e2.lin_mu_next = f->mu_next;
diff --git a/ekf_vio_amd/csrc/gather_body.inc b/ekf_vio_amd/csrc/gather_body.inc
--- a/ekf_vio_amd/csrc/gather_body.inc
+++ b/ekf_vio_amd/csrc/gather_body.inc
@@ -11,6 +11,8 @@
     const float* zrow;
     const float* mu;
     float* G;
+    float* T2m;
+    const int* inv_idx;
     int gx, nb1;
     int* zero_words;
     int n_zero;
@@ -128,6 +130,8 @@
     a.zrow = f->yres;
     a.mu = f->mu;
     a.G = f->Gm;
+    a.T2m = f->T2m;
+    a.inv_idx = f->inv_idx;
     a.gx = gather_gx(f->ldp, m_pad);
     a.nb1 = gather_element_wgs(f->ldp, m_pad);
     a.zero_words = nullptr;
diff --git a/ekf_vio_amd/csrc/gemm.hip b/ekf_vio_amd/csrc/gemm.hip
--- a/ekf_vio_amd/csrc/gemm.hip
+++ b/ekf_vio_amd/csrc/gemm.hip
@@ -25,7 +25,7 @@
 #define LDS_BT (BN)
 #define LDS_BN (BN + 1)
 
-template <bool TRANSB, int GROUPS, int EPI>
+template <bool TRANSB, int GROUPS, int EPI, bool SUBB = false>
 __global__ __launch_bounds__(256 * GROUPS) void gemm_f32_mfma_kernel(int M, int N, int K, float alpha, const float* __restrict__ A,
                                                             int lda, const float* __restrict__ B, int ldb, float beta,
                                                             const float* Cin, int ldcin, float* C, int ldc, int flush,
@@ -101,6 +101,8 @@
     const int kbeg = kbeg0 + grp * KTm * BK;
     const float* Ap = A + (size_t)(kbeg + a_k) * lda + i0 + a_i;
     const float* Bp = TRANSB ? (B + (size_t)(kbeg + a_k) * ldb + j0 + a_i) : (B + (size_t)(j0 + b_j) * ldb + kbeg + b_k);
+    static_assert(!SUBB || TRANSB, "B - Bsub is formed for A * B^T only");
+    const float* Ep = SUBB ? (epi.Bsub + (size_t)(kbeg + a_k) * ldb + j0 + a_i) : Bp;
     const size_t a_step = (size_t)BK * lda, b_step = TRANSB ? (size_t)BK * ldb : (size_t)BK;
     const size_t a_half = (size_t)16 * lda, b_half = TRANSB ? (size_t)16 * ldb : (size_t)16;
 
@@ -114,6 +116,9 @@
 
     float4 xa0, xa1, xb0, xb1;
     xa0 = xa1 = xb0 = xb1 = make_float4(0.f, 0.f, 0.f, 0.f);
+    float4 xe0, xe1;
+    xe0 = xe1 = make_float4(0.f, 0.f, 0.f, 0.f);
+#define GEMM_BPIECE(b, e) (SUBB ? make_float4(b.x - e.x, b.y - e.y, b.z - e.z, b.w - e.w) : b)
     float Fa[BK / 2], Fb[BK / 2], Ga[BK / 2], Gb[BK / 2];
 #pragma unroll
     for (int kk = 0; kk < BK / 2; kk++) Fa[kk] = Fb[kk] = Ga[kk] = Gb[kk] = 0.f;
@@ -126,13 +131,18 @@
         xa1 = *reinterpret_cast<const float4*>(ap_ + a_half);              \
         xb0 = *reinterpret_cast<const float4*>(bp_);                       \
         xb1 = *reinterpret_cast<const float4*>(bp_ + b_half);              \
+        if (SUBB) {                                                        \
+            const float* ep_ = Ep + (size_t)(kt) * b_step;                 \
+            xe0 = *reinterpret_cast<const float4*>(ep_);                   \
+            xe1 = *reinterpret_cast<const float4*>(ep_ + b_half);          \
+        }                                                                  \
     } while (0)
 #define GEMM_STAGE_A0(buf) *reinterpret_cast<float4*>(&As[buf][a_k * LDS_A + a_i]) = xa0
 #define GEMM_STAGE_A1(buf) *reinterpret_cast<float4*>(&As[buf][(a_k + 16) * LDS_A + a_i]) = xa1
 #define GEMM_STAGE_B0(buf)                                                                          \
     do {                                                                                            \
         if (TRANSB) {                                                                               \
-            *reinterpret_cast<float4*>(&Bs[buf][a_k * LDS_BT + a_i]) = xb0;                         \
+            *reinterpret_cast<float4*>(&Bs[buf][a_k * LDS_BT + a_i]) = GEMM_BPIECE(xb0, xe0);       \
         } else {                                                                                    \
             float* b_ = &Bs[buf][b_k * LDS_BN + b_j];                                               \
             b_[0] = xb0.x; b_[LDS_BN] = xb0.y; b_[2 * LDS_BN] = xb0.z; b_[3 * LDS_BN] = xb0.w;      \
@@ -141,7 +151,7 @@
 #define GEMM_STAGE_B1(buf)                                                                          \
     do {                                                                                            \
         if (TRANSB) {                                                                               \
-            *reinterpret_cast<float4*>(&Bs[buf][(a_k + 16) * LDS_BT + a_i]) = xb1;                  \
+            *reinterpret_cast<float4*>(&Bs[buf][(a_k + 16) * LDS_BT + a_i]) = GEMM_BPIECE(xb1, xe1); \
         } else {                                                                                    \
             float* b_ = &Bs[buf][(b_k + 16) * LDS_BN + b_j];                                        \
             b_[0] = xb1.x; b_[LDS_BN] = xb1.y; b_[2 * LDS_BN] = xb1.z; b_[3 * LDS_BN] = xb1.w;      \
@@ -170,6 +180,7 @@
         const float* bs_ = &Bs[nb][lk * LDB_S + wc * 32 + li];                                 \
         const float* ap_ = Ap + (size_t)(lt) * a_step;                                         \
         const float* bp_ = Bp + (size_t)(lt) * b_step;                                         \
+        const float* ep_ = Ep + (size_t)(lt) * b_step;                                         \
         _Pragma("unroll") for (int sl = 0; sl < 16; sl++) {                                    \
             if (act) GEMM_MFMA1(C, sl);                                                        \
             if (sl < 8 && (fr)) {                                                              \
@@ -189,6 +200,8 @@
                 if (sl == 13) xa1 = *reinterpret_cast<const float4*>(ap_ + a_half);            \
                 if (sl == 14) xb0 = *reinterpret_cast<const float4*>(bp_);                     \
                 if (sl == 15) xb1 = *reinterpret_cast<const float4*>(bp_ + b_half);            \
+                if (SUBB && sl == 14) xe0 = *reinterpret_cast<const float4*>(ep_);             \
+                if (SUBB && sl == 15) xe1 = *reinterpret_cast<const float4*>(ep_ + b_half);    \
             }                                                                                  \
             __builtin_amdgcn_sched_barrier(0);                                                 \
         }                                                                                      \
@@ -202,8 +215,8 @@
         cpre[r] = (beta != 0.f && ci_ < M && j < N) ? Cin[(size_t)j * ldcin + ci_] : 0.f;
     }
     {
-        float4 ya0, ya1, yb0, yb1;
-        ya0 = ya1 = yb0 = yb1 = make_float4(0.f, 0.f, 0.f, 0.f);
+        float4 ya0, ya1, yb0, yb1, ye0, ye1;
+        ya0 = ya1 = yb0 = yb1 = ye0 = ye1 = make_float4(0.f, 0.f, 0.f, 0.f);
         if (KT > 0) GEMM_LOAD(0);
         if (KT > 1) {
             const float* ap_ = Ap + a_step;
@@ -212,11 +225,15 @@
             ya1 = *reinterpret_cast<const float4*>(ap_ + a_half);
             yb0 = *reinterpret_cast<const float4*>(bp_);
             yb1 = *reinterpret_cast<const float4*>(bp_ + b_half);
+            if (SUBB) {
+                ye0 = *reinterpret_cast<const float4*>(Ep + b_step);
+                ye1 = *reinterpret_cast<const float4*>(Ep + b_step + b_half);
+            }
         }
         if (KT > 0) GEMM_STAGE(0);
         __syncthreads();
         if (KT > 0) GEMM_FRAGS(F, 0);
-        xa0 = ya0; xa1 = ya1; xb0 = yb0; xb1 = yb1;
+        xa0 = ya0; xa1 = ya1; xb0 = yb0; xb1 = yb1; xe0 = ye0; xe1 = ye1;
         if (KT > 1) GEMM_STAGE(1);
         if (KT > 2) GEMM_LOAD(2);
         __syncthreads();
@@ -250,6 +267,7 @@
         for (int r = 0; r < 16; r++) acc[r] += red[r * 256 + tid];
     }
 #undef GEMM_LOAD
+#undef GEMM_BPIECE
 #undef GEMM_STAGE
 #undef GEMM_STAGE_A0
 #undef GEMM_STAGE_A1
@@ -409,7 +427,7 @@
     for (int e = threadIdx.x; e < epi.n_zero; e += 256) epi.zero_words[e] = 0;
 }
 
-template <int BMt, int WPS, int EPI>
+template <int BMt, int WPS, int EPI, bool SUBB = false>
 __global__ __launch_bounds__(256 * WPS) void gemm16_kernel(int M, int N, int K, float alpha, const float* __restrict__ A, int lda,
                                                      const float* __restrict__ B, int ldb, float beta, const float* Cin,
                                                      int ldcin, float* C, int ldc, int flush, int lowerB, GemmEpi epi,
@@ -494,6 +512,7 @@
 #undef G16_ACOORD
     const __amdgpu_buffer_rsrc_t rsA = __builtin_amdgcn_make_buffer_rsrc(const_cast<float*>(A), 0, K * lda * 4, 0x00020000);
     const __amdgpu_buffer_rsrc_t rsB = __builtin_amdgcn_make_buffer_rsrc(const_cast<float*>(B), 0, K * ldb * 4, 0x00020000);
+    const __amdgpu_buffer_rsrc_t rsE = __builtin_amdgcn_make_buffer_rsrc(const_cast<float*>(SUBB ? epi.Bsub : B), 0, K * ldb * 4, 0x00020000);
     const int bo = ((tid >> 4) * ldb + j0 + (tid & 15) * 4) * 4;
     const int bl = (tid >> 4) * SB + (tid & 15) * 4;
     const int a_step = BKK * lda * 4, b_step = BKK * ldb * 4, b_rows = BKS * ldb * 4;
@@ -534,6 +553,8 @@
     }
     float4 Xa0, Xa1, Xa2, Xa3, Xb0, Xb1, Xb2, Xb3, Ya0, Ya1, Ya2, Ya3, Yb0, Yb1, Yb2, Yb3;
     float4 Za0, Za1, Za2, Za3, Zb0, Zb1, Zb2, Zb3;
+    float4 Xe0, Xe1, Xe2, Xe3, Ye0, Ye1, Ye2, Ye3, Ze0, Ze1, Ze2, Ze3;
+    Xe0 = Xe1 = Xe2 = Xe3 = Ye0 = Ye1 = Ye2 = Ye3 = Ze0 = Ze1 = Ze2 = Ze3 = make_float4(0.f, 0.f, 0.f, 0.f);
     Xa0 = Xa1 = Xa2 = Xa3 = Xb0 = Xb1 = Xb2 = Xb3 = make_float4(0.f, 0.f, 0.f, 0.f);
     Ya0 = Ya1 = Ya2 = Ya3 = Yb0 = Yb1 = Yb2 = Yb3 = make_float4(0.f, 0.f, 0.f, 0.f);
     Za0 = Za1 = Za2 = Za3 = Zb0 = Zb1 = Zb2 = Zb3 = make_float4(0.f, 0.f, 0.f, 0.f);
@@ -548,6 +569,10 @@
         S##b1 = __builtin_bit_cast(float4, __builtin_amdgcn_raw_buffer_load_b128(rsB, bo + b_rows, sb_, 0));                                                       \
         if constexpr (BV > 2) S##b2 = __builtin_bit_cast(float4, __builtin_amdgcn_raw_buffer_load_b128(rsB, bo + 2 * b_rows, sb_, 0));                             \
         if constexpr (BV > 2) S##b3 = __builtin_bit_cast(float4, __builtin_amdgcn_raw_buffer_load_b128(rsB, bo + 3 * b_rows, sb_, 0));                             \
+        if constexpr (SUBB) S##e0 = __builtin_bit_cast(float4, __builtin_amdgcn_raw_buffer_load_b128(rsE, bo, sb_, 0));                                            \
+        if constexpr (SUBB) S##e1 = __builtin_bit_cast(float4, __builtin_amdgcn_raw_buffer_load_b128(rsE, bo + b_rows, sb_, 0));                                   \
+        if constexpr (SUBB && BV > 2) S##e2 = __builtin_bit_cast(float4, __builtin_amdgcn_raw_buffer_load_b128(rsE, bo + 2 * b_rows, sb_, 0));                     \
+        if constexpr (SUBB && BV > 2) S##e3 = __builtin_bit_cast(float4, __builtin_amdgcn_raw_buffer_load_b128(rsE, bo + 3 * b_rows, sb_, 0));                     \
     } while (0)
 #define G16_LOADI(S, j, kt)                                                                            \
     do {                                                                                               \
@@ -560,17 +585,22 @@
         if ((j) == AV + 1) S##b1 = __builtin_bit_cast(float4, __builtin_amdgcn_raw_buffer_load_b128(rsB, bo + b_rows, sb_, 0));                                    \
         if ((j) == AV + 2 && BV > 2) S##b2 = __builtin_bit_cast(float4, __builtin_amdgcn_raw_buffer_load_b128(rsB, bo + 2 * b_rows, sb_, 0));                      \
         if ((j) == AV + 3 && BV > 2) S##b3 = __builtin_bit_cast(float4, __builtin_amdgcn_raw_buffer_load_b128(rsB, bo + 3 * b_rows, sb_, 0));                      \
-    } while (0)
+        if (SUBB && (j) == AV + BV) S##e0 = __builtin_bit_cast(float4, __builtin_amdgcn_raw_buffer_load_b128(rsE, bo, sb_, 0));                                    \
+        if (SUBB && (j) == AV + BV + 1) S##e1 = __builtin_bit_cast(float4, __builtin_amdgcn_raw_buffer_load_b128(rsE, bo + b_rows, sb_, 0));                       \
+        if (SUBB && (j) == AV + BV + 2 && BV > 2) S##e2 = __builtin_bit_cast(float4, __builtin_amdgcn_raw_buffer_load_b128(rsE, bo + 2 * b_rows, sb_, 0));         \
+        if (SUBB && (j) == AV + BV + 3 && BV > 2) S##e3 = __builtin_bit_cast(float4, __builtin_amdgcn_raw_buffer_load_b128(rsE, bo + 3 * b_rows, sb_, 0));         \
+    } while (0)
+#define G16_BPIECE(S, i) (SUBB ? make_float4(S##b##i.x - S##e##i.x, S##b##i.y - S##e##i.y, S##b##i.z - S##e##i.z, S##b##i.w - S##e##i.w) : S##b##i)
 #define G16_STAGEI(S, j, buf)                                                                          \
     do {                                                                                               \
         if ((j) == 0) *reinterpret_cast<float4*>(&As[buf][al0]) = S##a0;                               \
         if ((j) == 1 && AV > 1) *reinterpret_cast<float4*>(&As[buf][al1]) = S##a1;                     \
         if ((j) == 2 && AV > 2) *reinterpret_cast<float4*>(&As[buf][al2]) = S##a2;                     \
         if ((j) == 3 && AV > 3) *reinterpret_cast<float4*>(&As[buf][al3]) = S##a3;                     \
-        if ((j) == AV) *reinterpret_cast<float4*>(&Bs[buf][bl]) = S##b0;                               \
-        if ((j) == AV + 1) *reinterpret_cast<float4*>(&Bs[buf][bl + BKS * SB]) = S##b1;                \
-        if ((j) == AV + 2 && BV > 2) *reinterpret_cast<float4*>(&Bs[buf][bl + 2 * BKS * SB]) = S##b2;  \
-        if ((j) == AV + 3 && BV > 2) *reinterpret_cast<float4*>(&Bs[buf][bl + 3 * BKS * SB]) = S##b3;  \
+        if ((j) == AV) *reinterpret_cast<float4*>(&Bs[buf][bl]) = G16_BPIECE(S, 0);                               \
+        if ((j) == AV + 1) *reinterpret_cast<float4*>(&Bs[buf][bl + BKS * SB]) = G16_BPIECE(S, 1);                \
+        if ((j) == AV + 2 && BV > 2) *reinterpret_cast<float4*>(&Bs[buf][bl + 2 * BKS * SB]) = G16_BPIECE(S, 2);  \
+        if ((j) == AV + 3 && BV > 2) *reinterpret_cast<float4*>(&Bs[buf][bl + 3 * BKS * SB]) = G16_BPIECE(S, 3);  \
     } while (0)
 #define G16_STAGE_A(S, buf)                                                                            \
     do {                                                                                               \
@@ -581,10 +611,10 @@
     } while (0)
 #define G16_STAGE_B(S, buf)                                                                            \
     do {                                                                                               \
-        *reinterpret_cast<float4*>(&Bs[buf][bl]) = S##b0;                                              \
-        *reinterpret_cast<float4*>(&Bs[buf][bl + BKS * SB]) = S##b1;                                   \
-        if constexpr (BV > 2) *reinterpret_cast<float4*>(&Bs[buf][bl + 2 * BKS * SB]) = S##b2;         \
-        if constexpr (BV > 2) *reinterpret_cast<float4*>(&Bs[buf][bl + 3 * BKS * SB]) = S##b3;         \
+        *reinterpret_cast<float4*>(&Bs[buf][bl]) = G16_BPIECE(S, 0);                                              \
+        *reinterpret_cast<float4*>(&Bs[buf][bl + BKS * SB]) = G16_BPIECE(S, 1);                                   \
+        if constexpr (BV > 2) *reinterpret_cast<float4*>(&Bs[buf][bl + 2 * BKS * SB]) = G16_BPIECE(S, 2);         \
+        if constexpr (BV > 2) *reinterpret_cast<float4*>(&Bs[buf][bl + 3 * BKS * SB]) = G16_BPIECE(S, 3);         \
     } while (0)
 #define G16_MFMA(c, b, a) c = __builtin_amdgcn_mfma_f32_16x16x4f32(b, a, c, 0, 0, 0)
 #ifndef G16X_NOLOAD
@@ -631,6 +661,7 @@
     if (KT > 0) {
         constexpr int BAR = AV + BV;
         static_assert(BAR <= NS - 3 && NS % 4 == 0, "step schedule");
+        static_assert(!SUBB || AV + 2 * BV <= NS, "step schedule: one load per step, Bsub's pieces behind B's");
         G16_LOAD(Z, 0);
         G16_LOAD(X, 1);
         G16_LOAD(Y, 2);
@@ -670,6 +701,7 @@
 #undef G16_STAGEI
 #undef G16_STAGE_A
 #undef G16_STAGE_B
+#undef G16_BPIECE
     if constexpr (WPS > 1) {
         float* red = &As[0][0];
         static_assert(3 * BKK * SA >= RB * 4 * 256, "reduction scratch");
@@ -742,32 +774,35 @@
     const dim3 grid(p.grid_x, p.grid_y), block(p.threads());
     const int flush = c.flush, lowerB = c.lowerB;
     if (p.k16) {
-#define GEMM16_GO(BMv, W, EP)                                                                                                     \
-    hipLaunchKernelGGL((gemm16_kernel<BMv, W, EP>), grid, block, 0, s, M, N, K, c.alpha, c.A, c.lda, c.B, c.ldb, c.beta, c.Cin, c.ldcin, \
+#define GEMM16_GO(BMv, W, EP, SB)                                                                                                 \
+    hipLaunchKernelGGL((gemm16_kernel<BMv, W, EP, SB>), grid, block, 0, s, M, N, K, c.alpha, c.A, c.lda, c.B, c.ldb, c.beta, c.Cin, c.ldcin, \
                        c.C, c.ldc, flush, lowerB, e, p.tiles_x, p.tiles_y)
-#define GEMM16_BM(W, EP)                            \
-    do {                                            \
-        if (p.bm == 32) GEMM16_GO(32, W, EP);       \
-        else if (p.bm == 48) GEMM16_GO(48, W, EP);  \
-        else GEMM16_GO(64, W, EP);                  \
-    } while (0)
-        if (e.mode == EPI_JOSEPH1) GEMM16_BM(2, 1);
-        else if (e.mode == EPI_MEAN) GEMM16_BM(2, 2);
-        else if (e.mode == EPI_MEAN_PARTIAL) GEMM16_BM(2, 3);
-        else if (p.wps == 2) GEMM16_BM(2, 0);
-        else GEMM16_BM(1, 0);
+#define GEMM16_BM(W, EP, SB)                            \
+    do {                                                \
+        if (p.bm == 32) GEMM16_GO(32, W, EP, SB);       \
+        else if (p.bm == 48) GEMM16_GO(48, W, EP, SB);  \
+        else GEMM16_GO(64, W, EP, SB);                  \
+    } while (0)
+        if (e.mode == EPI_JOSEPH1) GEMM16_BM(2, 1, false);
+        else if (e.mode == EPI_MEAN) GEMM16_BM(2, 2, false);
+        else if (e.mode == EPI_MEAN_PARTIAL && e.Bsub) GEMM16_BM(2, 3, true);
+        else if (e.mode == EPI_MEAN_PARTIAL) GEMM16_BM(2, 3, false);
+        else if (p.wps == 2) GEMM16_BM(2, 0, false);
+        else GEMM16_BM(1, 0, false);
 #undef GEMM16_BM
 #undef GEMM16_GO
         return;
     }
     e.sym = p.sym, e.sym_w = p.sym_w, e.order2d = p.order2d;
-#define GEMM_GO(TB, G, EP)                                                                                                        \
-    hipLaunchKernelGGL((gemm_f32_mfma_kernel<TB, G, EP>), grid, block, 0, s, M, N, K, c.alpha, c.A, c.lda, c.B, c.ldb, c.beta, c.Cin, \
+#define GEMM_GO(TB, G, EP, ...)                                                                                                   \
+    hipLaunchKernelGGL((gemm_f32_mfma_kernel<TB, G, EP, ##__VA_ARGS__>), grid, block, 0, s, M, N, K, c.alpha, c.A, c.lda, c.B, c.ldb, c.beta, c.Cin, \
                        c.ldcin, c.C, c.ldc, flush, lowerB, e)
     if (e.mode == EPI_JOSEPH1) {
         GEMM_GO(true, 1, 1);
     } else if (e.mode == EPI_MEAN) {
         GEMM_GO(true, 1, 2);
+    } else if (e.mode == EPI_MEAN_PARTIAL && e.Bsub) {
+        GEMM_GO(true, 1, 3, true);
     } else if (e.mode == EPI_MEAN_PARTIAL) {
         GEMM_GO(true, 1, 3);
     } else if (p.groups == 2) {
diff --git a/ekf_vio_amd/filter.py b/ekf_vio_amd/filter.py
--- a/ekf_vio_amd/filter.py
+++ b/ekf_vio_amd/filter.py
@@ -373,6 +373,13 @@
         self._need_hooks()
         self._chk(self.lib.ekfvio_test_fill_update_scratch(self.h, int(word) & 0xFFFFFFFF))
 
+    def update_buffer(self, which, cols):
+        self._need_hooks()
+        ldp = (22 + 3 * int(self.cfg.max_features) + 1 + 63) // 64 * 64
+        out = np.zeros((int(cols), ldp), np.float32)
+        self._chk(self.lib.ekfvio_test_update_buffer(self.h, ("Km", "Gm", "T2m", "T2").index(which), _fp(out), out.size))
+        return out
+
     def test_cholesky_solve(self, S, Crhs):
         self._need_hooks()
         S = np.asarray(S, np.float32)
diff --git a/include/ekfvio_test_hooks.h b/include/ekfvio_test_hooks.h
--- a/include/ekfvio_test_hooks.h
+++ b/include/ekfvio_test_hooks.h
@@ -32,6 +32,7 @@
 EKFVIO_API int ekfvio_test_mem(ekfvio_filter* f, int64_t out[8]);
 EKFVIO_API int ekfvio_test_mem_fail(ekfvio_filter* f, int32_t nth);
 EKFVIO_API int ekfvio_test_fill_update_scratch(ekfvio_filter* f, uint32_t word);
+EKFVIO_API int ekfvio_test_update_buffer(ekfvio_filter* f, int32_t which, float* out, int64_t count);
 EKFVIO_API int ekfvio_test_zupt_decide(ekfvio_filter* f, const float* prev_px, const float* cur_px, const uint8_t* pass, int32_t count,
                                        float max_flow_px, int32_t min_tracks, float min_ratio, float* flow2, int32_t* n_pass, int32_t* n_still,
                                        int32_t* stationary);
```

After: 11140 (median of 6 runs). +1.0%, better.
